# SYSTRAN/faster-whisper

Hardware: AMD Instinct MI355X
Metric: audio-sec/sec (RTF) large-v3 fp16 beam=5 batch=16 (higher is better)
Workload: dtype f16

## Files before the change

### faster_whisper_amd/_lib.py

```python
import ctypes as C
import os

import numpy as np

_HERE = os.path.dirname(os.path.abspath(__file__))
LIB_PATH = os.environ.get("FWAMD_LIB") or os.path.join(_HERE, "libfwamd.so")

FW_OK = 0
FW_EINVAL = -1
FW_ENODEV = -2
FW_ENOMEM = -3
FW_ERUNTIME = -4
FW_ENOSPC = -5

COMPUTE_FLOAT16 = 0
COMPUTE_INT8_FLOAT16 = 1
FW_DT_F32 = 0
FW_DT_F16 = 1
FW_MAX_ALIGN_HEADS = 64


class FwConfig(C.Structure):
    _fields_ = [
        ("n_mels", C.c_int32), ("n_audio_ctx", C.c_int32), ("d_model", C.c_int32), ("n_heads", C.c_int32),
        ("n_enc_layers", C.c_int32), ("n_dec_layers", C.c_int32), ("n_vocab", C.c_int32),
        ("n_text_ctx", C.c_int32), ("is_multilingual", C.c_int32),
        ("tok_eot", C.c_int32), ("tok_sot", C.c_int32), ("tok_lang_begin", C.c_int32), ("n_langs", C.c_int32),
        ("tok_translate", C.c_int32), ("tok_transcribe", C.c_int32), ("tok_sot_lm", C.c_int32),
        ("tok_sot_prev", C.c_int32), ("tok_no_speech", C.c_int32), ("tok_no_timestamps", C.c_int32),
        ("tok_timestamp_begin", C.c_int32),
        ("n_suppress_begin", C.c_int32), ("suppress_begin", C.c_int32 * 8),
        ("n_align_heads", C.c_int32), ("align_heads", C.c_int32 * (2 * FW_MAX_ALIGN_HEADS)),
    ]


class FwWeight(C.Structure):
    _fields_ = [("name", C.c_char_p), ("data", C.c_void_p), ("dtype", C.c_int32), ("ndim", C.c_int32),
                ("dims", C.c_int64 * 4)]


class FwGenOpts(C.Structure):
    _fields_ = [
        ("beam_size", C.c_int32), ("patience", C.c_float), ("num_hypotheses", C.c_int32),
        ("length_penalty", C.c_float), ("repetition_penalty", C.c_float), ("no_repeat_ngram_size", C.c_int32),
        ("max_length", C.c_int32), ("return_scores", C.c_int32), ("return_no_speech_prob", C.c_int32),
        ("max_initial_timestamp_index", C.c_int32), ("suppress_blank", C.c_int32),
        ("suppress_tokens", C.POINTER(C.c_int32)), ("n_suppress_tokens", C.c_int32),
        ("sampling_topk", C.c_int32), ("sampling_temperature", C.c_float), ("seed", C.c_uint64),
        ("min_new_tokens", C.c_int32),
    ]


class FwVadWeights(C.Structure):
    _fields_ = [
        ("stft_basis", C.c_void_p), ("conv_w", C.c_void_p * 4), ("conv_b", C.c_void_p * 4),
        ("lstm_w", C.c_void_p), ("lstm_r", C.c_void_p), ("lstm_b", C.c_void_p), ("dec_w", C.c_void_p),
        ("dec_b", C.c_float),
    ]


SYMBOLS = [
    "fw_last_error", "fw_abi_version", "fw_device_count",
    "fw_model_create", "fw_model_free", "fw_model_info", "fw_model_blob", "fw_model_create_from_blob_dev",
    "fw_model_set_decode_batch", "fw_model_decode_batch", "fw_model_join_decoder", "fw_model_decode_stats",
    "fw_model_set_merge_wait", "fw_model_set_decode_lanes", "fw_model_run_capacity", "fw_dec_big_min_rows", "fw_dec_big_min_rows_of", "fw_test_knob",
    "fw_test_idle_lead_chunks",
    "fw_pack_blob_size", "fw_pack_blob_copy", "fw_pack_blob_free",
    "fw_logmel", "fw_logmel_full",
    "fw_encode", "fw_encode_pcm", "fw_encode_pcm_dev", "fw_tensor_shape", "fw_tensor_to_host",
    "fw_tensor_from_host", "fw_tensor_free",
    "fw_generate", "fw_generate_lp", "fw_detect_language", "fw_align",
    "fw_prof_enable", "fw_prof_reset", "fw_prof_count", "fw_prof_name", "fw_prof_get", "fw_synchronize",
    "fw_dev_alloc", "fw_dev_free", "fw_dev_upload",
    "fw_test_gemm", "fw_test_layernorm", "fw_test_attention", "fw_test_dec_linear", "fw_test_dec_logits", "fw_test_logits_rules",
    "fw_test_dec_self_attn", "fw_test_dec_cross_attn", "fw_test_dec_cross_probs", "fw_test_dec_softmax_pick", "fw_bench_gemm", "fw_bench_dec_linear", "fw_bench_attention",
    "fw_bench_gemm_epi", "fw_bench_dec_linear_epi",
    "fw_test_gemm_ex", "fw_test_cross_kv_frag_index", "fw_test_quant_rows", "fw_test_layernorm_frag",
    "fw_test_dec_beam_update", "fw_test_dec_embed", "fw_test_align_post",
    "fw_test_logits_rules_lp", "fw_test_dec_beam_update_lp",
    "fw_test_logits_rules_smp_tab", "fw_test_graph_captures",
    "fw_vad_create", "fw_vad_forward", "fw_vad_free", "fw_vad_forward_dev", "fw_vad_forward_audio_dev",
    "fw_vad_forward_audio_batch_dev",
    "fw_flac_info", "fw_flac_decode",
    "fw_resample_filter", "fw_resample_dev", "fw_bench_resample",
]

_lib = None


class FwError(RuntimeError):
    pass


def load():
    global _lib
    if _lib is not None:
        return _lib
    if not os.path.exists(LIB_PATH):
        raise FwError(
            f"{LIB_PATH} not found: build it with `python -c 'import __graft_entry__ as g; g.build()'` "
            "(hipcc --offload-arch=gfx950). faster_whisper_amd has no CPU fallback.")
    lib = C.CDLL(LIB_PATH)
    vp, i32, i64, f32p = C.c_void_p, C.c_int32, C.c_int64, C.POINTER(C.c_float)
    i32p, i64p = C.POINTER(C.c_int32), C.POINTER(C.c_int64)
    lib.fw_last_error.restype = C.c_char_p
    lib.fw_abi_version.restype = i32
    lib.fw_device_count.restype = i32
    lib.fw_model_create.argtypes = [C.POINTER(FwConfig), C.POINTER(FwWeight), i32, i32, i32, i32, i32, C.POINTER(vp)]
    lib.fw_model_free.argtypes = [vp]
    lib.fw_model_free.restype = None
    lib.fw_model_info.argtypes = [vp, C.POINTER(FwConfig), i32p, i32p, i32p, i32p]
    lib.fw_model_blob.argtypes = [vp, C.POINTER(vp), i64p]
    lib.fw_model_create_from_blob_dev.argtypes = [C.POINTER(FwConfig), vp, i64, i32, i32, i32, i32, C.POINTER(vp)]
    lib.fw_model_set_decode_batch.argtypes = [vp, i32]
    lib.fw_model_decode_batch.argtypes = [vp]
    lib.fw_model_decode_batch.restype = i32
    lib.fw_model_run_capacity.argtypes = [vp]
    lib.fw_model_run_capacity.restype = i32
    lib.fw_dec_big_min_rows.restype = i32
    if hasattr(lib, "fw_dec_big_min_rows_of"):
        lib.fw_dec_big_min_rows_of.restype = i32
        lib.fw_dec_big_min_rows_of.argtypes = [i32, i32]
    if hasattr(lib, "fw_flac_info"):
        lib.fw_flac_info.argtypes = [vp, i64, i32p, i32p, i32p, i64p]
        lib.fw_flac_decode.argtypes = [vp, i64, vp, i64, i64p, i32p]
    if hasattr(lib, "fw_test_knob"):
        lib.fw_test_knob.argtypes = [i32, i32]
    if hasattr(lib, "fw_test_idle_lead_chunks"):
        lib.fw_test_idle_lead_chunks.argtypes = [i64, i32, i32, i64, i32]
        lib.fw_test_idle_lead_chunks.restype = i64
    lib.fw_model_join_decoder.argtypes = [vp, vp]
    lib.fw_model_set_merge_wait.argtypes = [vp, i32, i32]
    lib.fw_model_set_decode_lanes.argtypes = [vp, i32]
    lib.fw_model_decode_stats.argtypes = [vp, i64p, i64p, i64p, i32p]
    lib.fw_pack_blob_size.argtypes = [C.POINTER(FwConfig), C.POINTER(FwWeight), i32, i32, i64p, C.POINTER(vp)]
    lib.fw_pack_blob_copy.argtypes = [vp, vp, i64]
    lib.fw_pack_blob_free.argtypes = [vp]
    lib.fw_pack_blob_free.restype = None
    lib.fw_logmel.argtypes = [vp, vp, i64p, i32, vp, i32p]
    lib.fw_logmel_full.argtypes = [vp, vp, i64, vp, i64]
    lib.fw_encode.argtypes = [vp, vp, i32, C.POINTER(vp)]
    lib.fw_encode_pcm.argtypes = [vp, vp, i64p, i32, C.POINTER(vp)]
    lib.fw_encode_pcm_dev.argtypes = [vp, vp, i64p, i32, C.POINTER(vp)]
    lib.fw_tensor_shape.argtypes = [vp, i32p, i32p, i32p]
    lib.fw_tensor_to_host.argtypes = [vp, vp, vp]
    lib.fw_tensor_from_host.argtypes = [vp, vp, i32, C.POINTER(vp)]
    lib.fw_tensor_free.argtypes = [vp]
    lib.fw_tensor_free.restype = None
    lib.fw_generate.argtypes = [vp, vp, i32p, i32p, i32, C.POINTER(FwGenOpts), i32p, i32p, f32p, f32p]
    if hasattr(lib, "fw_generate_lp"):
        lib.fw_generate_lp.argtypes = [vp, vp, i32p, i32p, i32, C.POINTER(FwGenOpts), i32p, i32p, f32p, f32p, f32p, f32p]
    lib.fw_detect_language.argtypes = [vp, vp, i32, i32p, f32p]
    lib.fw_align.argtypes = [vp, vp, i32p, i32, i32p, i32p, i32p, i32, i32, i32, i32p, i32p, f32p]
    lib.fw_prof_enable.argtypes = [vp, i32]
    lib.fw_prof_enable.restype = None
    lib.fw_prof_reset.argtypes = [vp]
    lib.fw_prof_reset.restype = None
    lib.fw_prof_count.restype = i32
    lib.fw_prof_name.argtypes = [i32]
    lib.fw_prof_name.restype = C.c_char_p
    lib.fw_prof_get.argtypes = [vp, i32, C.POINTER(C.c_double), i64p, C.POINTER(C.c_double), C.POINTER(C.c_double)]
    lib.fw_synchronize.argtypes = [vp]
    lib.fw_dev_alloc.argtypes = [vp, i64, C.POINTER(vp)]
    lib.fw_dev_free.argtypes = [vp, vp]
    lib.fw_dev_upload.argtypes = [vp, vp, vp, i64]
    lib.fw_test_gemm.argtypes = [vp, vp, vp, vp, vp, i32, i32, i32, i32, i32, vp]
    lib.fw_test_dec_linear.argtypes = [vp, vp, vp, vp, vp, vp, vp, i32, i32, i32, i32, i32, vp, vp]
    lib.fw_test_dec_logits.argtypes = [vp, vp, i32, vp]
    lib.fw_test_logits_rules.argtypes = [vp, vp, i32, vp, i32, vp, C.POINTER(FwGenOpts), i32, vp, vp]
    if hasattr(lib, "fw_test_dec_self_attn"):
        lib.fw_test_dec_self_attn.argtypes = [vp, vp, vp, vp, vp, i32, i32, i32, i32, i32, i32, i32, i32, i32, i32, i32, vp]
        lib.fw_test_dec_cross_attn.argtypes = [vp, vp, vp, vp, i32, i32, i32, i32, i32, i32, vp, vp, i32, C.c_float, vp]
        lib.fw_test_dec_cross_probs.argtypes = [vp, vp, vp, i32, i32, i32, vp, i32, i32, i32, i32, vp]
        lib.fw_test_dec_softmax_pick.argtypes = [vp, vp, i32, i32, i32, vp, i32, vp]
    lib.fw_bench_attention.argtypes = [vp, i32, i32, i32, i32, i32, f32p]
    lib.fw_bench_gemm.argtypes = [vp, i32, i32, i32, i32, i32, i32, i32, i32, f32p]
    lib.fw_bench_dec_linear.argtypes = [vp, i32, i32, i32, i32, i32, i32, f32p]
    if hasattr(lib, "fw_bench_gemm_epi"):
        lib.fw_bench_gemm_epi.argtypes = [vp, i32, i32, i32, i32, i32, i32, i32, i32, i32, i32, i32, f32p]
        lib.fw_bench_dec_linear_epi.argtypes = [vp, i32, i32, i32, i32, i32, i32, i32, i32, i32, f32p]
    lib.fw_test_layernorm.argtypes = [vp, vp, vp, vp, i32, i32, vp]
    lib.fw_test_attention.argtypes = [vp, vp, vp, vp, i32, i32, i32, vp]
    if hasattr(lib, "fw_test_gemm_ex"):
        lib.fw_test_gemm_ex.argtypes = [vp, vp, i64, i64, i64, vp, vp, vp, i64, i64, i64, vp, i64, i64, i64, i64, i64,
                                        i32, i32, i32, i32, i32, i32, i32, i32, i32, vp, vp]
        lib.fw_test_cross_kv_frag_index.argtypes = [i32, i32, i32, vp]
        lib.fw_test_quant_rows.argtypes = [vp, vp, i32, i32, i64, vp, vp, i32, vp, vp]
        lib.fw_test_layernorm_frag.argtypes = [vp, vp, vp, vp, i32, i32, i32, vp]
    if hasattr(lib, "fw_test_dec_beam_update"):
        f32 = C.c_float
        lib.fw_test_dec_beam_update.argtypes = [vp, i32, i32, i32, i32, i32, i32, i32, i32, f32, i32, vp, vp, vp, vp, vp,
                                                i32, f32, vp, vp, vp, vp, vp, vp, vp, vp, vp, vp, vp]
        lib.fw_test_dec_embed.argtypes = [vp, vp, i32, vp, i32, vp, i32, i32, i32, i32, i32, i32, f32, vp, vp]
        lib.fw_test_align_post.argtypes = [vp, vp, i32, i32, i32, i32, vp, vp, i32, vp]
    if hasattr(lib, "fw_test_dec_beam_update_lp"):
        f32 = C.c_float
        lib.fw_test_logits_rules_lp.argtypes = [vp, vp, i32, vp, i32, vp, C.POINTER(FwGenOpts), i32, vp, vp, vp]
        lib.fw_test_dec_beam_update_lp.argtypes = [vp, i32, i32, i32, i32, i32, i32, i32, i32, f32, i32, vp, vp, vp, vp, vp,
                                                   vp, vp, i32, f32, vp, vp, vp, vp, vp, vp, vp, vp, vp, vp, vp, vp, vp]
    if hasattr(lib, "fw_test_graph_captures"):
        lib.fw_test_logits_rules_smp_tab.argtypes = [vp, vp, i32, vp, i32, vp, C.POINTER(FwGenOpts), i32, vp, vp, vp, vp, vp, vp]
        lib.fw_test_graph_captures.argtypes = [vp, i64p]
    lib.fw_vad_create.argtypes = [C.POINTER(FwVadWeights), C.POINTER(vp)]
    lib.fw_vad_forward.argtypes = [vp, vp, i64, i32, vp, vp, vp]
    lib.fw_vad_free.argtypes = [vp]
    lib.fw_vad_forward_dev.argtypes = [vp, i32, vp, i64, vp, vp, vp]
    if hasattr(lib, "fw_vad_forward_audio_dev"):
        lib.fw_vad_forward_audio_dev.argtypes = [vp, i32, vp, i64, vp, vp, vp]
    if hasattr(lib, "fw_vad_forward_audio_batch_dev"):
        lib.fw_vad_forward_audio_batch_dev.argtypes = [vp, i32, vp, vp, i32, vp, vp, vp]
    lib.fw_vad_free.restype = None
    if hasattr(lib, "fw_resample_dev"):
        f64 = C.c_double
        lib.fw_resample_filter.argtypes = [i32, i32, i32, f64, vp, i64p, i32p, i32p]
        lib.fw_resample_dev.argtypes = [i32, vp, i64, i32, i32, i32, f64, i32, vp, i64]
        lib.fw_bench_resample.argtypes = [i32, vp, i64, i32, i32, i32, f64, i32, i32, f32p]
    _lib = lib
    return lib


def check(rc: int):
    if rc == FW_OK:
        return
    msg = load().fw_last_error().decode("utf-8", "replace")
    if rc in (FW_EINVAL, FW_ENOSPC):
        raise ValueError(msg)
    raise RuntimeError(f"libfwamd error {rc}: {msg}")


def ptr(a: np.ndarray):
    return a.ctypes.data_as(C.c_void_p)


def as_i32p(a: np.ndarray):
    return a.ctypes.data_as(C.POINTER(C.c_int32))


def as_i64p(a: np.ndarray):
    return a.ctypes.data_as(C.POINTER(C.c_int64))


def as_f32p(a: np.ndarray):
    return a.ctypes.data_as(C.POINTER(C.c_float))
```

### faster_whisper_amd/csrc/engine.h

```cpp
#pragma once
#include <hip/hip_runtime.h>
#include <math.h>
#include <stdint.h>
#include <string.h>
#include <algorithm>
#include <atomic>
#include <chrono>
#include <condition_variable>
#include <deque>
#include <map>
#include <memory>
#include <mutex>
#include <string>
#include <vector>

#include "../../include/fwamd.h"
#include "common.h"

namespace fw {

void set_error(const char* fmt, ...);
#define FW_HIP(call)                                                                   \
  do {                                                                                 \
    hipError_t e_ = (call);                                                            \
    if (e_ != hipSuccess) {                                                            \
      fw::set_error("%s failed: %s (%s:%d)", #call, hipGetErrorString(e_), __FILE__, __LINE__); \
      return FW_ENODEV;                                                                \
    }                                                                                  \
  } while (0)
#define FW_CHECK_ARG(cond, ...)        \
  do {                                 \
    if (!(cond)) {                     \
      fw::set_error(__VA_ARGS__);      \
      return FW_EINVAL;                \
    }                                  \
  } while (0)

inline uint16_t f32_to_f16_bits(float f) {
  half_t h = (half_t)f;
  uint16_t u;
  memcpy(&u, &h, 2);
  return u;
}
inline float f16_bits_to_f32(uint16_t u) {
  half_t h;
  memcpy(&h, &u, 2);
  return (float)h;
}

template <typename At>
inline float quant_row_i8(const float* row, int K, int8_t* q, At&& at) {
  float amax = 0.f;
  for (int k = 0; k < K; ++k) amax = std::max(amax, fabsf(row[k]));
  const float sc = amax > 0.f ? 127.0f / amax : 0.f;
  for (int k = 0; k < K; ++k) q[at(k)] = (int8_t)lrintf(row[k] * sc);
  return amax > 0.f ? amax / 127.0f : 1.0f;
}

#define FW_BLOB_MAGIC "FWAMDBL1"
struct BlobHeader {
  char magic[8];
  int32_t version;
  int32_t n_tensors;
  int64_t total_bytes;
  int32_t compute_type;
  int32_t reserved;
  fw_config cfg;
};
struct BlobEntry {
  char name[64];
  int32_t dtype;
  int32_t ndim;
  int64_t dims[4];
  int64_t offset;
  int64_t nbytes;
};

struct DevTensor {
  void* ptr = nullptr;
  int dtype = 1;
  int ndim = 0;
  int64_t dims[4] = {0, 0, 0, 0};
};

struct LinearW {
  const half_t* w = nullptr;
  const half_t* b = nullptr;
  const int8_t* wq = nullptr;
  const float* wscale = nullptr;
  const float* s1 = nullptr;
  const float* cf = nullptr;
  int N = 0, K = 0;
};
struct LNW { const half_t* g = nullptr; const half_t* b = nullptr; };

struct EncLayerW { LNW ln1, ln2; LinearW qk, v, out, ffn1, ffn2; };
struct DecLayerW { LNW ln1, ln2, ln3; LinearW qkv, out, cq, ck, cv, cout, ffn1, ffn2; LinearW qkv_p, cq_p, ffn1_p; };

enum ProfFamily {
  PF_LOGMEL = 0, PF_ENC_GEMM, PF_ENC_ATTN, PF_ENC_LN, PF_CROSS_KV_GEMM,
  PF_DEC_GEMM_QKV, PF_DEC_GEMM_DXD, PF_DEC_GEMM_FFN1, PF_DEC_GEMM_FFN2,
  PF_DEC_SELF_ATTN, PF_DEC_CROSS_ATTN, PF_DEC_LOGITS, PF_DEC_SAMPLE, PF_DEC_MISC, PF_COUNT
};

struct ProfAcc {
  double ms = 0; int64_t launches = 0; double flops = 0; double bytes = 0;
};

struct Prof {
  std::mutex mu;
  bool on = false;
  ProfAcc acc[PF_COUNT];
  struct PendingEv { hipEvent_t a, b; int fam; };
  std::vector<PendingEv> pending;
  std::vector<hipEvent_t> ev_pool;
  ~Prof();
};

struct Model;
struct Tensor {
  Model* owner = nullptr;
  half_t* data = nullptr;
  int B = 0, T = 0, D = 0;
  uint64_t id = 0;
};

struct GenWorkspace;
struct GenRequest;
struct CrossPool;

constexpr int kMaxDecodeLanes = 4;
struct DecodeLane {
  GenWorkspace* gen = nullptr;
  hipStream_t stream = nullptr;
  hipStream_t spare = nullptr;
  std::mutex mu;
  Prof prof;
  bool busy = false;
  ~DecodeLane();
};

struct DecodeGroup {
  std::mutex mu;
  std::condition_variable cv;
  std::deque<GenRequest*> queue;
  bool gathering = false;
  bool resizing = false;
  int active_runs = 0;
  std::atomic<int> lanes_enabled{kMaxDecodeLanes};
  std::atomic<int> encoding{0};
  std::chrono::steady_clock::time_point last_arrival{};
  std::mutex enc_mu;
  std::atomic<int> enc_pass_us{0};
  std::atomic<int> merge_wait_ms{-1};
  std::atomic<int> merge_fill_pct{90};
  std::atomic<int64_t> n_runs{0}, n_requests{0}, n_chunks{0};
  std::atomic<int> max_run_chunks{0};
  std::atomic<int64_t> graph_captures{0};
};

struct Model {
  fw_config cfg{};
  int compute_type = 0;
  int device = 0;
  int max_batch = 0, max_beam = 0;
  hipStream_t stream = nullptr;
  std::mutex mu;

  void* blob = nullptr;
  bool blob_owned = true;
  int64_t blob_bytes = 0;
  std::map<std::string, DevTensor> tensors;
  int c_pad = 0;
  LinearW conv1, conv2;
  const half_t* enc_pos = nullptr;
  std::vector<EncLayerW> enc;
  LNW enc_ln_post;
  const half_t* tok_emb = nullptr;
  const half_t* dec_pos = nullptr;
  std::vector<DecLayerW> dec;
  LinearW logits;
  LinearW logits_p;
  LNW dec_ln;
  int ln_unfold = 0;
  bool has_plain = false;

  float* lm_consts = nullptr;
  float* lm_filtT = nullptr;
  int lm_mel_pad = 0;

  float* ws_pcm = nullptr; int64_t ws_pcm_cap = 0;
  int64_t* ws_offsets = nullptr;
  float* ws_raw = nullptr; int64_t ws_raw_cap = 0;
  int* ws_chunk_max = nullptr;
  int* ws_nframes = nullptr;
  float* ws_feat32 = nullptr;
  half_t* ws_mel_cl = nullptr;
  half_t* ws_conv1 = nullptr;
  half_t *ws_x = nullptr, *ws_x2 = nullptr, *ws_xn = nullptr;
  half_t* ws_qk = nullptr;
  half_t* ws_vt = nullptr;
  half_t* ws_att = nullptr;
  half_t* ws_ffn = nullptr;
  int8_t* ws_xq = nullptr;
  float* ws_xs = nullptr;
  int t_pad = 0;

  std::vector<std::unique_ptr<DecodeLane>> lanes;
  Model* decoder = nullptr;
  CrossPool* xpool = nullptr;
  int decode_batch = 0;
  int lane_batch = 0;
  int decode_self_ctx = 0;
  int dependents = 0;
  bool free_deferred = false;
  void* self = nullptr;
  Model* blob_owner = nullptr;
  DecodeGroup grp;

  std::mutex pool_mu;
  std::vector<half_t*> enc_pool;

  Prof prof;
};

struct ProfScope {
  Prof* p; int fam; hipStream_t st; hipEvent_t a = nullptr, b = nullptr;
  ProfScope(Prof& p_, int fam_, double flops, double bytes, hipStream_t st_);
  ProfScope(Model* m, int fam_, double flops, double bytes) : ProfScope(m->prof, fam_, flops, bytes, m->stream) {}
  ~ProfScope();
};
void prof_collect(Prof& p);

int dev_alloc(void** p, size_t bytes);
hipError_t create_stream(hipStream_t* st, const char* role);
int64_t idle_lead_chunks(int64_t queued, int n_queued, int encoding, int64_t want, int max_batch, int lanes = 2);
template <typename T>
inline int dev_alloc_t(T** p, size_t n) { return dev_alloc(reinterpret_cast<void**>(p), n * sizeof(T)); }

int run_linear(Model* m, const LinearW& L, const half_t* A, int64_t lda, int64_t a_bs, half_t* C, int64_t ldc,
               int64_t c_bs, const half_t* res, int64_t ldr, int64_t r_bs, int M, int batch, int act, bool trans,
               int head_rows = 0, hipStream_t st = nullptr);

int run_linear_i8(Model* m, const LinearW& L, const half_t* A, const LNW* ln, half_t* C, int64_t ldc, int64_t c_bs,
                  const half_t* res, int64_t ldr, int64_t r_bs, int M, int batch, int act, bool trans, int head_rows,
                  hipStream_t st = nullptr, int8_t* xq = nullptr, float* xs = nullptr);

int run_linear_layers(Model* m, const LinearW& L0, int n_layers, int64_t w_lstride, int64_t b_lstride, const half_t* A,
                      int64_t lda, int64_t a_bs, half_t* C, int64_t ldc, int64_t c_bs, int64_t c_lstride, int M, int batch,
                      bool trans, int head_rows, hipStream_t st);
void set_cross_kv_layered(int on);
int run_encoder(Model* m, int B, half_t* out);

void set_pos_blocks(int on);
uint64_t next_tensor_id();
int gen_workspace_ensure(Model* dm, DecodeLane* lane);
int cross_pool_ensure(Model* dm, int pool_chunks);
int gen_workspace_build(const Model* dm, DecodeLane* lane, int lane_chunks, int self_ctx);
void gen_workspace_free(DecodeLane* lane);
int64_t gen_workspace_bytes(const Model* m, int lane_chunks, int self_ctx);
int64_t cross_pool_bytes(const Model* m, int pool_chunks);
void cross_pool_free(Model* m);
void launch_align_post(hipStream_t st, const float* probs, float* stats, int n_sel, int n_tok_cap, int T, int B,
                       const int* n_tok, const int* nfr, int width, float* mat);
inline Model* decoder_of(Model* m) { return m->decoder ? m->decoder : m; }
inline int lane_chunks_of(const Model* m) {
  const int b = m->lane_batch > 0 ? m->lane_batch : m->decode_batch;
  return b > m->max_batch ? b : m->max_batch;
}

}

struct fw_model { fw::Model impl; };
struct fw_tensor { fw::Tensor impl; };
```

### faster_whisper_amd/csrc/engine.hip

```cpp
#include "engine.h"

#include <math.h>
#include <stdarg.h>
#include <stdio.h>
#include <stdlib.h>
#include <string.h>

#include <algorithm>

#include "dec_kernels.h"
#include "kernels.h"

namespace fw {

static thread_local char g_err[1024] = "";
void set_error(const char* fmt, ...) {
  va_list ap;
  va_start(ap, fmt);
  vsnprintf(g_err, sizeof(g_err), fmt, ap);
  va_end(ap);
}

int dev_alloc(void** p, size_t bytes) {
  if (bytes == 0) bytes = 256;
  hipError_t e = hipMalloc(p, bytes);
  if (e != hipSuccess) {
    set_error("hipMalloc(%zu bytes) failed: %s", bytes, hipGetErrorString(e));
    *p = nullptr;
    return FW_ENOMEM;
  }
  return FW_OK;
}

static const char* kProfNames[PF_COUNT] = {
    "logmel", "enc_gemm", "enc_attn", "enc_layernorm", "cross_kv_gemm", "dec_gemm_qkv", "dec_gemm_dxd",
    "dec_gemm_ffn1", "dec_gemm_ffn2", "dec_self_attn", "dec_cross_attn", "dec_logits", "dec_sample", "dec_misc"};

static hipEvent_t ev_get(Prof& p) {
  if (!p.ev_pool.empty()) {
    hipEvent_t e = p.ev_pool.back();
    p.ev_pool.pop_back();
    return e;
  }
  hipEvent_t e;
  (void)hipEventCreate(&e);
  return e;
}
ProfScope::ProfScope(Prof& p_, int fam_, double flops, double bytes, hipStream_t st_) : p(&p_), fam(fam_), st(st_) {
  if (!p->on) return;
  {
    std::lock_guard<std::mutex> lk(p->mu);
    a = ev_get(*p);
    b = ev_get(*p);
    p->acc[fam].flops += flops;
    p->acc[fam].bytes += bytes;
    p->acc[fam].launches += 1;
  }
  (void)hipEventRecord(a, st);
}
ProfScope::~ProfScope() {
  if (!a) return;
  (void)hipEventRecord(b, st);
  std::lock_guard<std::mutex> lk(p->mu);
  p->pending.push_back({a, b, fam});
}
void prof_collect(Prof& p) {
  std::vector<Prof::PendingEv> todo;
  {
    std::lock_guard<std::mutex> lk(p.mu);
    todo.swap(p.pending);
  }
  std::vector<std::pair<int, float>> got;
  for (auto& e : todo) {
    (void)hipEventSynchronize(e.b);
    float ms = 0.f;
    (void)hipEventElapsedTime(&ms, e.a, e.b);
    got.push_back({e.fam, ms});
  }
  std::lock_guard<std::mutex> lk(p.mu);
  for (auto& g : got) p.acc[g.first].ms += g.second;
  for (auto& e : todo) {
    p.ev_pool.push_back(e.a);
    p.ev_pool.push_back(e.b);
  }
}
Prof::~Prof() {
  for (auto& e : pending) { (void)hipEventDestroy(e.a); (void)hipEventDestroy(e.b); }
  for (auto e : ev_pool) (void)hipEventDestroy(e);
}
template <typename F>
static void for_each_prof(Model* m, F&& f) {
  f(m->prof);
  for (auto& l : m->lanes) f(l->prof);
}

struct PackItem {
  std::string name;
  int ndim;
  int64_t dims[4];
  std::vector<uint16_t> data;
  std::vector<float> fdata;
  std::vector<int8_t> qdata;
  int dtype = 1;
  const void* bytes() const {
    return dtype == 1 ? (const void*)data.data() : dtype == 2 ? (const void*)qdata.data() : (const void*)fdata.data();
  }
  int64_t nbytes() const {
    return dtype == 1 ? (int64_t)data.size() * 2 : dtype == 2 ? (int64_t)qdata.size() : (int64_t)fdata.size() * 4;
  }
};

static const fw_weight* find_w(const fw_weight* w, int n, const std::string& name) {
  for (int i = 0; i < n; ++i)
    if (name == w[i].name) return &w[i];
  return nullptr;
}
static int64_t numel(const fw_weight* w) {
  int64_t n = 1;
  for (int i = 0; i < w->ndim; ++i) n *= w->dims[i];
  return n;
}
static float w_at(const fw_weight* w, int64_t i) {
  if (w->dtype == FW_DT_F32) return reinterpret_cast<const float*>(w->data)[i];
  half_t h;
  memcpy(&h, reinterpret_cast<const uint16_t*>(w->data) + i, 2);
  return (float)h;
}
static void to_f16(const fw_weight* w, std::vector<uint16_t>& out) {
  const int64_t n = numel(w);
  out.resize(n);
  if (w->dtype == FW_DT_F16) {
    memcpy(out.data(), w->data, n * 2);
  } else {
    const float* s = reinterpret_cast<const float*>(w->data);
    for (int64_t i = 0; i < n; ++i) out[i] = f32_to_f16_bits(s[i]);
  }
}

static int expect_shape(const fw_weight* w, const std::string& name, std::initializer_list<int64_t> dims) {
  if (!w) {
    set_error("missing weight '%s'", name.c_str());
    return FW_EINVAL;
  }
  if ((size_t)w->ndim != dims.size()) {
    set_error("weight '%s': expected %zu dims, got %d", name.c_str(), dims.size(), w->ndim);
    return FW_EINVAL;
  }
  int i = 0;
  for (int64_t d : dims) {
    if (w->dims[i] != d) {
      set_error("weight '%s': dim %d is %lld, expected %lld", name.c_str(), i, (long long)w->dims[i], (long long)d);
      return FW_EINVAL;
    }
    ++i;
  }
  return FW_OK;
}

static int check_config(const fw_config* c) {
  FW_CHECK_ARG(c->n_mels > 0 && c->n_mels <= 128, "n_mels must be in (0,128], got %d", c->n_mels);
  FW_CHECK_ARG(c->d_model % 128 == 0 && c->d_model >= 128 && c->d_model <= 1280,
               "d_model must be a multiple of 128 in [128,1280], got %d", c->d_model);
  FW_CHECK_ARG(c->n_heads * 64 == c->d_model, "head dim must be 64 (n_heads=%d, d_model=%d)", c->n_heads, c->d_model);
  FW_CHECK_ARG(c->n_audio_ctx == 1500, "n_audio_ctx must be 1500, got %d", c->n_audio_ctx);
  FW_CHECK_ARG(c->n_text_ctx > 0 && c->n_text_ctx <= 448, "n_text_ctx must be in (0,448]");
  FW_CHECK_ARG(c->n_enc_layers > 0 && c->n_dec_layers > 0, "layer counts must be positive");
  FW_CHECK_ARG(c->n_vocab > c->tok_timestamp_begin && c->tok_timestamp_begin > 0, "bad vocabulary layout");
  FW_CHECK_ARG(c->n_align_heads >= 0 && c->n_align_heads <= FW_MAX_ALIGN_HEADS, "too many alignment heads");
  FW_CHECK_ARG(c->n_suppress_begin >= 0 && c->n_suppress_begin <= 8, "n_suppress_begin out of range");
  FW_CHECK_ARG(c->n_vocab <= 57344, "n_vocab %d exceeds the 57344 ids the logits kernel holds per row", c->n_vocab);
  const int toks[] = {c->tok_eot, c->tok_sot, c->tok_translate, c->tok_transcribe, c->tok_sot_lm, c->tok_sot_prev,
                      c->tok_no_speech, c->tok_no_timestamps, c->tok_timestamp_begin};
  for (int t : toks) FW_CHECK_ARG(t >= 0 && t < c->n_vocab, "special token id %d outside the vocabulary of %d", t, c->n_vocab);
  FW_CHECK_ARG(c->n_langs >= 0 && c->tok_lang_begin >= 0 && c->tok_lang_begin + c->n_langs <= c->n_vocab,
               "language ids [%d, %d) outside the vocabulary of %d", c->tok_lang_begin, c->tok_lang_begin + c->n_langs,
               c->n_vocab);
  for (int i = 0; i < c->n_suppress_begin; ++i)
    FW_CHECK_ARG(c->suppress_begin[i] >= 0 && c->suppress_begin[i] < c->n_vocab, "suppress_begin id out of range");
  return FW_OK;
}

static int pack_blob(const fw_config* cfg, const fw_weight* w, int nw, int compute_type,
                     std::vector<uint8_t>& blob) {
  const int d = cfg->d_model, nm = cfg->n_mels;
  const int c_pad = ((nm + 63) / 64) * 64;
  std::vector<PackItem> items;
  auto add_plain = [&](const std::string& name, std::initializer_list<int64_t> dims) -> int {
    const fw_weight* t = find_w(w, nw, name);
    int rc = expect_shape(t, name, dims);
    if (rc) return rc;
    PackItem it;
    it.name = name;
    it.ndim = (int)dims.size();
    int i = 0;
    for (int64_t x : dims) it.dims[i++] = x;
    for (; i < 4; ++i) it.dims[i] = 1;
    to_f16(t, it.data);
    items.push_back(std::move(it));
    return FW_OK;
  };
  auto add_conv = [&](const std::string& name, int cout, int cin, int cin_pad) -> int {
    const fw_weight* t = find_w(w, nw, name + ".w");
    int rc = expect_shape(t, name + ".w", {cout, cin, 3});
    if (rc) return rc;
    PackItem it;
    it.name = name + ".wg";
    it.ndim = 2;
    it.dims[0] = cout; it.dims[1] = 3 * cin_pad; it.dims[2] = it.dims[3] = 1;
    it.data.assign((size_t)cout * 3 * cin_pad, 0);
    for (int o = 0; o < cout; ++o)
      for (int c = 0; c < cin; ++c)
        for (int k = 0; k < 3; ++k)
          it.data[(size_t)o * 3 * cin_pad + (size_t)k * cin_pad + c] =
              f32_to_f16_bits(w_at(t, ((int64_t)o * cin + c) * 3 + k));
    items.push_back(std::move(it));
    return add_plain(name + ".b", {cout});
  };
  auto add_folded = [&](const std::string& out, const std::string& wname, const std::string& bname,
                        const std::string& gname, const std::string& lbname, int N, int K) -> int {
    const fw_weight* W = find_w(w, nw, wname);
    const fw_weight* G = find_w(w, nw, gname);
    const fw_weight* LB = find_w(w, nw, lbname);
    const fw_weight* Bi = bname.empty() ? nullptr : find_w(w, nw, bname);
    int rc = expect_shape(W, wname, {N, K});
    if (rc) return rc;
    if ((rc = expect_shape(G, gname, {K}))) return rc;
    if ((rc = expect_shape(LB, lbname, {K}))) return rc;
    if (!bname.empty() && (rc = expect_shape(Bi, bname, {N}))) return rc;
    std::vector<float> g(K), lb(K);
    for (int k = 0; k < K; ++k) {
      g[k] = f16_bits_to_f32(f32_to_f16_bits(w_at(G, k)));
      lb[k] = f16_bits_to_f32(f32_to_f16_bits(w_at(LB, k)));
    }
    PackItem wf, s1, cf;
    wf.name = out + ".wf"; wf.ndim = 2; wf.dims[0] = N; wf.dims[1] = K; wf.dims[2] = wf.dims[3] = 1;
    wf.data.resize((size_t)N * K);
    s1.name = out + ".s1"; s1.ndim = 1; s1.dims[0] = N; s1.dims[1] = s1.dims[2] = s1.dims[3] = 1; s1.dtype = 0;
    cf.name = out + ".cf"; cf.ndim = 1; cf.dims[0] = N; cf.dims[1] = cf.dims[2] = cf.dims[3] = 1; cf.dtype = 0;
    s1.fdata.resize(N); cf.fdata.resize(N);
    for (int n = 0; n < N; ++n) {
      double a1 = 0.0, ac = 0.0;
      for (int k = 0; k < K; ++k) {
        const float wv = f16_bits_to_f32(f32_to_f16_bits(w_at(W, (int64_t)n * K + k)));
        const uint16_t wg = f32_to_f16_bits(wv * g[k]);
        wf.data[(size_t)n * K + k] = wg;
        a1 += (double)f16_bits_to_f32(wg);
        ac += (double)wv * (double)lb[k];
      }
      if (Bi) ac += (double)f16_bits_to_f32(f32_to_f16_bits(w_at(Bi, n)));
      s1.fdata[n] = (float)a1;
      cf.fdata[n] = (float)ac;
    }
    items.push_back(std::move(wf)); items.push_back(std::move(s1)); items.push_back(std::move(cf));
    return FW_OK;
  };
  auto add_quant = [&](const std::string& out, const std::string& wname, int N, int K) -> int {
    const fw_weight* W = find_w(w, nw, wname);
    int rc = expect_shape(W, wname, {N, K});
    if (rc) return rc;
    PackItem wq, ws;
    wq.name = out + ".wq"; wq.ndim = 2; wq.dims[0] = N; wq.dims[1] = K; wq.dims[2] = wq.dims[3] = 1; wq.dtype = 2;
    ws.name = out + ".ws"; ws.ndim = 1; ws.dims[0] = N; ws.dims[1] = ws.dims[2] = ws.dims[3] = 1; ws.dtype = 0;
    wq.qdata.resize((size_t)N * K);
    ws.fdata.resize(N);
    std::vector<float> row(K);
    for (int n = 0; n < N; ++n) {
      for (int k = 0; k < K; ++k) row[k] = f16_bits_to_f32(f32_to_f16_bits(w_at(W, (int64_t)n * K + k)));
      ws.fdata[n] = quant_row_i8(row.data(), K, wq.qdata.data(), [&](int k) { return (size_t)n * K + k; });
    }
    items.push_back(std::move(wq)); items.push_back(std::move(ws));
    return FW_OK;
  };
  const bool i8 = compute_type == FW_COMPUTE_INT8_FLOAT16;
  auto add_linear = [&](const std::string& base, int N, int K) -> int {
    int rc = i8 ? add_quant(base, base + ".w", N, K) : add_plain(base + ".w", {N, K});
    if (rc) return rc;
    return add_plain(base + ".b", {N});
  };
  const char* lu_env = getenv("FWAMD_LN_UNFOLD");
  const char* pp_env = getenv("FWAMD_PACK_PLAIN");
  const bool with_plain = (lu_env && (lu_env[0] == '1' || lu_env[0] == '2') && !lu_env[1]) || (pp_env && pp_env[0] == '1');
  auto add_ln_linear = [&](const std::string& base, const std::string& ln, int N, int K) -> int {
    if (!i8) {
      int rc = add_folded(base, base + ".w", base + ".b", ln + ".g", ln + ".b", N, K);
      if (rc || !with_plain) return rc;
    }
    int rc = add_linear(base, N, K);
    if (rc) return rc;
    if ((rc = add_plain(ln + ".g", {K}))) return rc;
    return add_plain(ln + ".b", {K});
  };
  int rc;
#define TRY(x) do { rc = (x); if (rc) return rc; } while (0)
  TRY(add_conv("enc.conv1", d, nm, c_pad));
  TRY(add_conv("enc.conv2", d, d, d));
  TRY(add_plain("enc.pos", {cfg->n_audio_ctx, d}));
  char nb[96];
  for (int i = 0; i < cfg->n_enc_layers; ++i) {
    auto nmf = [&](const char* s) { snprintf(nb, sizeof(nb), "enc.%d.%s", i, s); return std::string(nb); };
    TRY(add_plain(nmf("ln1.g"), {d})); TRY(add_plain(nmf("ln1.b"), {d}));
    TRY(add_linear(nmf("attn.qkv"), 3 * d, d));
    TRY(add_linear(nmf("attn.out"), d, d));
    TRY(add_plain(nmf("ln2.g"), {d})); TRY(add_plain(nmf("ln2.b"), {d}));
    TRY(add_linear(nmf("ffn1"), 4 * d, d));
    TRY(add_linear(nmf("ffn2"), d, 4 * d));
  }
  TRY(add_plain("enc.ln_post.g", {d})); TRY(add_plain("enc.ln_post.b", {d}));
  TRY(add_plain("dec.tok_emb", {cfg->n_vocab, d}));
  if (i8) {
    PackItem& te = items.back();
    const int64_t K = d;
    for (int64_t n = 0; n < cfg->n_vocab; ++n) {
      float amax = 0.f;
      for (int64_t k = 0; k < K; ++k) amax = std::max(amax, fabsf(f16_bits_to_f32(te.data[n * K + k])));
      const float sc = amax > 0.f ? 127.0f / amax : 0.f, ds = amax > 0.f ? amax / 127.0f : 1.0f;
      for (int64_t k = 0; k < K; ++k)
        te.data[n * K + k] = f32_to_f16_bits((float)lrintf(f16_bits_to_f32(te.data[n * K + k]) * sc) * ds);
    }
  }
  TRY(add_plain("dec.pos", {cfg->n_text_ctx, d}));
  for (int i = 0; i < cfg->n_dec_layers; ++i) {
    auto nmf = [&](const char* s) { snprintf(nb, sizeof(nb), "dec.%d.%s", i, s); return std::string(nb); };
    TRY(add_ln_linear(nmf("self.qkv"), nmf("ln1"), 3 * d, d));
    TRY(add_linear(nmf("self.out"), d, d));
    TRY(add_ln_linear(nmf("cross.q"), nmf("ln2"), d, d));
    TRY(add_linear(nmf("cross.kv"), 2 * d, d));
    TRY(add_linear(nmf("cross.out"), d, d));
    TRY(add_ln_linear(nmf("ffn1"), nmf("ln3"), 4 * d, d));
    TRY(add_linear(nmf("ffn2"), d, 4 * d));
  }
  if (i8) {
    TRY(add_quant("dec.logits", "dec.tok_emb", cfg->n_vocab, d));
    TRY(add_plain("dec.ln.g", {d})); TRY(add_plain("dec.ln.b", {d}));
  } else {
    TRY(add_folded("dec.logits", "dec.tok_emb", "", "dec.ln.g", "dec.ln.b", cfg->n_vocab, d));
    if (with_plain) {
      TRY(add_plain("dec.tok_emb", {cfg->n_vocab, d}));
      items.back().name = "dec.logits.wp";
      TRY(add_plain("dec.ln.g", {d})); TRY(add_plain("dec.ln.b", {d}));
    }
  }
#undef TRY

  for (PackItem& it : items) {
    const std::string& nm = it.name;
    if (nm.compare(0, 4, "dec.") != 0 || it.ndim != 2 || it.dtype != (i8 ? 2 : 1)) continue;
    auto ends = [&](const char* suf) {
      const size_t n = strlen(suf);
      return nm.size() >= n && nm.compare(nm.size() - n, n, suf) == 0;
    };
    const bool hit = i8 ? (ends("self.qkv.wq") || ends("self.out.wq") || ends("cross.q.wq") || ends("cross.out.wq") ||
                           ends("ffn1.wq") || ends("ffn2.wq") || nm == "dec.logits.wq")
                        : (ends("self.qkv.wf") || ends("self.out.w") || ends("cross.q.wf") || ends("cross.out.w") ||
                           ends("ffn1.wf") || ends("ffn2.w") || nm == "dec.logits.wf" || ends("self.qkv.w") ||
                           ends("cross.q.w") || ends("ffn1.w") || nm == "dec.logits.wp");
    if (!hit) continue;
    const int64_t N = it.dims[0], K = it.dims[1], KE = i8 ? 64 : 32, OCT = KE / 4;
    const bool logits = nm.compare(0, 10, "dec.logits") == 0;
    if ((!logits && N % 32) || K % KE) {
      set_error("fragment-major packing needs N %% 32 == 0 and K %% %lld == 0 (%s is %lld x %lld)", (long long)KE,
                nm.c_str(), (long long)N, (long long)K);
      return FW_EINVAL;
    }
    const int64_t NP = (N + 15) / 16 * 16, KS = K / KE;
    it.dims[0] = NP;
    auto at = [&](int64_t n, int64_t k) {
      return (((n >> 4) * KS + k / KE) * 64 + ((k / OCT) & 3) * 16 + (n & 15)) * OCT + (k % OCT);
    };
    if (i8) {
      std::vector<int8_t> src;
      src.swap(it.qdata);
      it.qdata.assign((size_t)NP * K, 0);
      for (int64_t n = 0; n < N; ++n)
        for (int64_t k = 0; k < K; ++k) it.qdata[at(n, k)] = src[n * K + k];
    } else {
      std::vector<uint16_t> src;
      src.swap(it.data);
      it.data.assign((size_t)NP * K, 0);
      for (int64_t n = 0; n < N; ++n)
        for (int64_t k = 0; k < K; ++k) it.data[at(n, k)] = src[n * K + k];
    }
  }

  const int64_t hdr = (int64_t)sizeof(BlobHeader) + (int64_t)items.size() * sizeof(BlobEntry);
  int64_t off = (hdr + 255) / 256 * 256;
  std::vector<BlobEntry> entries(items.size());
  for (size_t i = 0; i < items.size(); ++i) {
    BlobEntry& e = entries[i];
    memset(&e, 0, sizeof(e));
    snprintf(e.name, sizeof(e.name), "%s", items[i].name.c_str());
    e.dtype = items[i].dtype;
    e.ndim = items[i].ndim;
    for (int k = 0; k < 4; ++k) e.dims[k] = items[i].dims[k];
    e.offset = off;
    e.nbytes = items[i].nbytes();
    off = (off + e.nbytes + 255) / 256 * 256;
  }
  blob.assign((size_t)off, 0);
  BlobHeader h;
  memset(&h, 0, sizeof(h));
  memcpy(h.magic, FW_BLOB_MAGIC, 8);
  h.version = 1;
  h.n_tensors = (int32_t)items.size();
  h.total_bytes = off;
  h.compute_type = compute_type;
  h.reserved = 6;
  h.cfg = *cfg;
  memcpy(blob.data(), &h, sizeof(h));
  memcpy(blob.data() + sizeof(h), entries.data(), entries.size() * sizeof(BlobEntry));
  for (size_t i = 0; i < items.size(); ++i)
    memcpy(blob.data() + entries[i].offset, items[i].bytes(), (size_t)entries[i].nbytes);
  return FW_OK;
}

static void compute_mel_filters(int n_mels, std::vector<float>& filt ) {
  const int n_fft = 400, nb = 201;
  const double sr = 16000.0;
  std::vector<double> fftfreqs(nb);
  const double val = 1.0 / (n_fft * (1.0 / sr));
  for (int k = 0; k < nb; ++k) fftfreqs[k] = k * val;
  const double max_mel = 45.245640471924965;
  const int n = n_mels + 2;
  std::vector<double> mels(n), freqs(n);
  const double step = (max_mel - 0.0) / (n - 1);
  for (int i = 0; i < n; ++i) mels[i] = i * step + 0.0;
  mels[n - 1] = max_mel;
  const double f_sp = 200.0 / 3;
  const double min_log_hz = 1000.0, min_log_mel = (min_log_hz - 0.0) / f_sp;
  const double logstep = log(6.4) / 27.0;
  for (int i = 0; i < n; ++i) {
    freqs[i] = 0.0 + f_sp * mels[i];
    if (mels[i] >= min_log_mel) freqs[i] = min_log_hz * exp(logstep * (mels[i] - min_log_mel));
  }
  filt.assign((size_t)n_mels * nb, 0.f);
  for (int i = 0; i < n_mels; ++i) {
    const double fd0 = freqs[i + 1] - freqs[i], fd1 = freqs[i + 2] - freqs[i + 1];
    const double enorm = 2.0 / (freqs[i + 2] - freqs[i]);
    for (int k = 0; k < nb; ++k) {
      const double lower = -(freqs[i] - fftfreqs[k]) / fd0;
      const double upper = (freqs[i + 2] - fftfreqs[k]) / fd1;
      double wv = std::max(0.0, std::min(lower, upper));
      wv *= enorm;
      filt[(size_t)i * nb + k] = (float)wv;
    }
  }
}

static int setup_logmel_consts(Model* m) {
  std::vector<float> consts(800);
  for (int j = 0; j < 400; ++j) consts[j] = (float)cos(2.0 * M_PI * (double)j / 400.0);
  for (int n = 0; n < 400; ++n) consts[400 + n] = (float)(0.5 - 0.5 * cos(2.0 * M_PI * (double)n / 400.0));
  std::vector<float> filt;
  compute_mel_filters(m->cfg.n_mels, filt);
  m->lm_mel_pad = ((m->cfg.n_mels + 31) / 32) * 32;
  std::vector<float> filtT((size_t)224 * m->lm_mel_pad, 0.f);
  for (int i = 0; i < m->cfg.n_mels; ++i)
    for (int k = 0; k < 201; ++k) filtT[(size_t)k * m->lm_mel_pad + i] = filt[(size_t)i * 201 + k];
  int rc;
  if ((rc = dev_alloc_t(&m->lm_consts, 800))) return rc;
  if ((rc = dev_alloc_t(&m->lm_filtT, filtT.size()))) return rc;
  FW_HIP(hipMemcpy(m->lm_consts, consts.data(), 800 * sizeof(float), hipMemcpyHostToDevice));
  FW_HIP(hipMemcpy(m->lm_filtT, filtT.data(), filtT.size() * sizeof(float), hipMemcpyHostToDevice));
  return FW_OK;
}

std::mutex& g_models_mu_ref();
std::vector<Model*>& g_live_models_ref();
static const half_t* tptr(Model* m, const std::string& name) {
  auto it = m->tensors.find(name);
  return it == m->tensors.end() ? nullptr : reinterpret_cast<const half_t*>(it->second.ptr);
}

static int bind_weights(Model* m) {
  const fw_config& c = m->cfg;
  const int d = c.d_model;
  const bool i8 = m->compute_type == FW_COMPUTE_INT8_FLOAT16;
  m->c_pad = ((c.n_mels + 63) / 64) * 64;
  auto need = [&](const std::string& n, const half_t** out) -> int {
    *out = tptr(m, n);
    if (!*out) {
      set_error("weight blob lacks tensor '%s'", n.c_str());
      return FW_EINVAL;
    }
    return FW_OK;
  };
  auto need_f = [&](const std::string& n, const float** out) -> int {
    const half_t* p = nullptr;
    int r = need(n, &p);
    *out = reinterpret_cast<const float*>(p);
    return r;
  };
  auto linear = [&](const std::string& base, LinearW* L, int N, int K, int r0) -> int {
    int r;
    *L = LinearW();
    L->N = N; L->K = K;
    if (i8) {
      const half_t* q = nullptr;
      if ((r = need(base + ".wq", &q))) return r;
      L->wq = reinterpret_cast<const int8_t*>(q) + (size_t)r0 * K;
      if ((r = need_f(base + ".ws", &L->wscale))) return r;
      L->wscale += r0;
    } else {
      if ((r = need(base + ".w", &L->w))) return r;
      L->w += (size_t)r0 * K;
    }
    if ((r = need(base + ".b", &L->b))) return r;
    L->b += r0;
    return FW_OK;
  };
  auto folded = [&](const std::string& base, LinearW* L, int N, int K) -> int {
    int r;
    *L = LinearW();
    if ((r = need(base + ".wf", &L->w))) return r;
    if ((r = need_f(base + ".s1", &L->s1))) return r;
    if ((r = need_f(base + ".cf", &L->cf))) return r;
    L->N = N; L->K = K;
    return FW_OK;
  };
  auto ln = [&](const std::string& base, LNW* L) -> int {
    int r;
    if ((r = need(base + ".g", &L->g))) return r;
    return need(base + ".b", &L->b);
  };
  int rc;
#define TRY(x) do { if ((rc = (x))) return rc; } while (0)
  TRY(need("enc.conv1.wg", &m->conv1.w)); TRY(need("enc.conv1.b", &m->conv1.b));
  m->conv1.N = d; m->conv1.K = 3 * m->c_pad;
  TRY(need("enc.conv2.wg", &m->conv2.w)); TRY(need("enc.conv2.b", &m->conv2.b));
  m->conv2.N = d; m->conv2.K = 3 * d;
  TRY(need("enc.pos", &m->enc_pos));
  m->enc.resize(c.n_enc_layers);
  char nb[96];
  for (int i = 0; i < c.n_enc_layers; ++i) {
    EncLayerW& L = m->enc[i];
    auto nm = [&](const char* s) { snprintf(nb, sizeof(nb), "enc.%d.%s", i, s); return std::string(nb); };
    TRY(ln(nm("ln1"), &L.ln1));
    TRY(linear(nm("attn.qkv"), &L.qk, 2 * d, d, 0));
    TRY(linear(nm("attn.qkv"), &L.v, d, d, 2 * d));
    TRY(linear(nm("attn.out"), &L.out, d, d, 0));
    TRY(ln(nm("ln2"), &L.ln2));
    TRY(linear(nm("ffn1"), &L.ffn1, 4 * d, d, 0));
    TRY(linear(nm("ffn2"), &L.ffn2, d, 4 * d, 0));
  }
  TRY(ln("enc.ln_post", &m->enc_ln_post));
  TRY(need("dec.tok_emb", &m->tok_emb)); TRY(need("dec.pos", &m->dec_pos));
  m->dec.resize(c.n_dec_layers);
  m->has_plain = !i8 && tptr(m, "dec.logits.wp") != nullptr;
  for (int i = 0; i < c.n_dec_layers; ++i) {
    DecLayerW& L = m->dec[i];
    auto nm = [&](const char* s) { snprintf(nb, sizeof(nb), "dec.%d.%s", i, s); return std::string(nb); };
    if (i8) {
      TRY(ln(nm("ln1"), &L.ln1)); TRY(ln(nm("ln2"), &L.ln2)); TRY(ln(nm("ln3"), &L.ln3));
      TRY(linear(nm("self.qkv"), &L.qkv, 3 * d, d, 0));
      TRY(linear(nm("cross.q"), &L.cq, d, d, 0));
      TRY(linear(nm("ffn1"), &L.ffn1, 4 * d, d, 0));
    } else {
      TRY(folded(nm("self.qkv"), &L.qkv, 3 * d, d));
      TRY(folded(nm("cross.q"), &L.cq, d, d));
      TRY(folded(nm("ffn1"), &L.ffn1, 4 * d, d));
      if (m->has_plain) {
        TRY(ln(nm("ln1"), &L.ln1)); TRY(ln(nm("ln2"), &L.ln2)); TRY(ln(nm("ln3"), &L.ln3));
        TRY(linear(nm("self.qkv"), &L.qkv_p, 3 * d, d, 0));
        TRY(linear(nm("cross.q"), &L.cq_p, d, d, 0));
        TRY(linear(nm("ffn1"), &L.ffn1_p, 4 * d, d, 0));
      }
    }
    TRY(linear(nm("self.out"), &L.out, d, d, 0));
    TRY(linear(nm("cross.kv"), &L.ck, d, d, 0));
    TRY(linear(nm("cross.kv"), &L.cv, d, d, d));
    TRY(linear(nm("cross.out"), &L.cout, d, d, 0));
    TRY(linear(nm("ffn2"), &L.ffn2, d, 4 * d, 0));
  }
  if (i8) {
    const half_t* q = nullptr;
    m->logits = LinearW();
    TRY(need("dec.logits.wq", &q));
    m->logits.wq = reinterpret_cast<const int8_t*>(q);
    TRY(need_f("dec.logits.ws", &m->logits.wscale));
    m->logits.N = c.n_vocab; m->logits.K = d;
    TRY(ln("dec.ln", &m->dec_ln));
  } else {
    TRY(folded("dec.logits", &m->logits, c.n_vocab, d));
    m->logits_p = LinearW();
    if (m->has_plain) {
      TRY(need("dec.logits.wp", &m->logits_p.w));
      m->logits_p.N = c.n_vocab; m->logits_p.K = d;
      TRY(ln("dec.ln", &m->dec_ln));
    }
  }
#undef TRY
  return FW_OK;
}

static int alloc_workspaces(Model* m) {
  const fw_config& c = m->cfg;
  const size_t B = m->max_batch, d = c.d_model, T = c.n_audio_ctx;
  m->t_pad = ((c.n_audio_ctx + 63) / 64) * 64;
  int rc;
#define A(p, n) do { if ((rc = dev_alloc_t(&(p), (n)))) return rc; } while (0)
  A(m->ws_offsets, B + 1);
  A(m->ws_chunk_max, B);
  A(m->ws_nframes, B);
  m->ws_raw_cap = (int64_t)B * c.n_mels * 3008;
  A(m->ws_raw, (size_t)m->ws_raw_cap);
  A(m->ws_feat32, B * c.n_mels * 3000);
  A(m->ws_mel_cl, B * 3002 * m->c_pad);
  A(m->ws_conv1, B * 3002 * d);
  A(m->ws_x, B * T * d);
  A(m->ws_x2, B * T * d);
  A(m->ws_xn, B * T * d);
  A(m->ws_qk, B * T * 2 * d);
  A(m->ws_vt, B * d * m->t_pad);
  A(m->ws_att, B * T * d);
  A(m->ws_ffn, B * T * 4 * d);
  if (m->compute_type == FW_COMPUTE_INT8_FLOAT16) {
    A(m->ws_xq, B * T * 4 * d);
    A(m->ws_xs, B * T);
  }
#undef A
  FW_HIP(hipMemset(m->ws_conv1, 0, B * 3002 * d * sizeof(half_t)));
  FW_HIP(hipMemset(m->ws_vt, 0, B * d * m->t_pad * sizeof(half_t)));
  FW_HIP(hipMemset(m->ws_mel_cl, 0, B * 3002 * m->c_pad * sizeof(half_t)));
  return FW_OK;
}

static int model_from_blob(const void* blob_dev, int64_t blob_bytes, bool owned, int device, int max_batch,
                           int max_beam, fw_model** out) {
  FW_CHECK_ARG(max_batch >= 1 && max_batch <= 256, "max_batch must be in [1,256], got %d", max_batch);
  FW_CHECK_ARG(max_beam >= 1 && max_beam <= 16, "max_beam must be in [1,16], got %d", max_beam);
  FW_CHECK_ARG(max_batch * max_beam <= 2048, "max_batch * max_beam must be <= 2048 decoder rows, got %d", max_batch * max_beam);
  FW_CHECK_ARG(blob_bytes >= (int64_t)sizeof(BlobHeader), "weight blob too small");
  BlobHeader h;
  FW_HIP(hipMemcpy(&h, blob_dev, sizeof(h), hipMemcpyDeviceToHost));
  FW_CHECK_ARG(memcmp(h.magic, FW_BLOB_MAGIC, 8) == 0 && h.version == 1, "bad weight blob magic/version");
  FW_CHECK_ARG(h.total_bytes <= blob_bytes, "weight blob truncated (%lld > %lld)", (long long)h.total_bytes,
               (long long)blob_bytes);
  int rc = check_config(&h.cfg);
  if (rc) return rc;
  FW_CHECK_ARG(h.compute_type == FW_COMPUTE_FLOAT16 || h.compute_type == FW_COMPUTE_INT8_FLOAT16,
               "unsupported compute type %d", h.compute_type);
  std::vector<BlobEntry> entries(h.n_tensors);
  FW_HIP(hipMemcpy(entries.data(), reinterpret_cast<const char*>(blob_dev) + sizeof(h),
                   entries.size() * sizeof(BlobEntry), hipMemcpyDeviceToHost));
  fw_model* fm = new fw_model();
  Model* m = &fm->impl;
  m->lanes.reserve(kMaxDecodeLanes);
  m->lanes.emplace_back(new DecodeLane());
  m->cfg = h.cfg;
  m->compute_type = h.compute_type;
  if (h.reserved != 6) {
    delete fm;
    set_error("weight blob was packed by an older libfwamd (layout generation %d, expected 6): repack it", h.reserved);
    return FW_EINVAL;
  }
  m->device = device;
  m->max_batch = max_batch;
  m->max_beam = max_beam;
  m->blob = const_cast<void*>(blob_dev);
  m->blob_owned = owned;
  m->blob_bytes = blob_bytes;
  for (auto& e : entries) {
    DevTensor t;
    t.ptr = reinterpret_cast<char*>(m->blob) + e.offset;
    t.dtype = e.dtype;
    t.ndim = e.ndim;
    for (int k = 0; k < 4; ++k) t.dims[k] = e.dims[k];
    m->tensors[e.name] = t;
  }
  auto fail = [&](int code) { fw_model_free(fm); return code; };
  hipError_t he = create_stream(&m->stream, "ENC");
  if (he != hipSuccess) {
    set_error("hipStreamCreate failed: %s", hipGetErrorString(he));
    return fail(FW_ENODEV);
  }
  if ((rc = bind_weights(m))) return fail(rc);
  {
    const char* lu = getenv("FWAMD_LN_UNFOLD");
    if (lu && lu[0] >= '0' && lu[0] <= '2' && !lu[1]) m->ln_unfold = lu[0] - '0';
    if (m->ln_unfold && m->compute_type != FW_COMPUTE_INT8_FLOAT16 && !m->has_plain) {
      set_error("FWAMD_LN_UNFOLD=%d needs a weight blob packed with FWAMD_LN_UNFOLD set (this one carries the folded forms only)",
                m->ln_unfold);
      return fail(FW_EINVAL);
    }
  }
  if ((rc = setup_logmel_consts(m))) return fail(rc);
  if ((rc = alloc_workspaces(m))) return fail(rc);
  m->decode_batch = max_batch;
  he = hipDeviceSynchronize();
  if (he != hipSuccess) {
    set_error("device sync after model setup failed: %s", hipGetErrorString(he));
    return fail(FW_ENODEV);
  }
  {
    std::lock_guard<std::mutex> lk(g_models_mu_ref());
    if (!owned)
      for (Model* o : g_live_models_ref())
        if (o->blob == m->blob && o->blob_owned) { m->blob_owner = o; o->dependents += 1; break; }
    g_live_models_ref().push_back(m);
  }
  m->self = fm;
  *out = fm;
  return FW_OK;
}

static void balanced_cu_mask(int n_cus, bool invert, uint32_t mask[8]) {
  const int k = n_cus / 32;
  for (int w = 0; w < 8; ++w) mask[w] = 0;
  for (int i = 0; i < 256; ++i) {
    const bool in = ((i % 8) + (i / 8)) % 8 < k;
    if (in != invert) mask[i >> 5] |= 1u << (i & 31);
  }
}

hipError_t create_stream(hipStream_t* st, const char* role) {
  char name[64];
  snprintf(name, sizeof(name), "FWAMD_%s_CUS", role);
  if (const char* c = getenv(name)) {
    const int v = atoi(c), n = v < 0 ? -v : v;
    if (n >= 32 && n <= 224 && n % 32 == 0) {
      uint32_t mask[8];
      balanced_cu_mask(n, v < 0, mask);
      return hipExtStreamCreateWithCUMask(st, 8, mask);
    }
  }
  snprintf(name, sizeof(name), "FWAMD_%s_STREAM_PRIO", role);
  const char* e = getenv(name);
  if (e && (!strcmp(e, "high") || !strcmp(e, "low"))) {
    int least = 0, greatest = 0;
    if (hipDeviceGetStreamPriorityRange(&least, &greatest) == hipSuccess && least != greatest)
      return hipStreamCreateWithPriority(st, hipStreamNonBlocking, e[0] == 'h' ? greatest : least);
  }
  return hipStreamCreateWithFlags(st, hipStreamNonBlocking);
}

int run_linear(Model* m, const LinearW& L, const half_t* A, int64_t lda, int64_t a_bs, half_t* C, int64_t ldc,
               int64_t c_bs, const half_t* res, int64_t ldr, int64_t r_bs, int M, int batch, int act, bool trans,
               int head_rows, hipStream_t st) {
  fwk::GemmParams p;
  memset(&p, 0, sizeof(p));
  p.A = A; p.lda = lda; p.a_bstride = a_bs;
  p.W = L.w; p.ldw = L.K;
  p.bias = L.b;
  p.res = res; p.ldr = ldr; p.r_bstride = r_bs;
  p.C = C; p.ldc = ldc; p.c_bstride = c_bs;
  p.M = M; p.N = L.N; p.K = L.K;
  p.act = act;
  p.head_rows = head_rows;
  if (fwk::launch_gemm(st ? st : m->stream, p, batch, trans) != 0) {
    set_error("gemm: unsupported shape M=%d N=%d K=%d lda=%lld", M, L.N, L.K, (long long)lda);
    return FW_ERUNTIME;
  }
  return FW_OK;
}

int run_linear_layers(Model* m, const LinearW& L0, int n_layers, int64_t w_lstride, int64_t b_lstride, const half_t* A,
                      int64_t lda, int64_t a_bs, half_t* C, int64_t ldc, int64_t c_bs, int64_t c_lstride, int M, int batch,
                      bool trans, int head_rows, hipStream_t st) {
  fwk::GemmParams p;
  memset(&p, 0, sizeof(p));
  p.A = A; p.lda = lda; p.a_bstride = a_bs;
  p.W = L0.w; p.ldw = L0.K;
  p.bias = L0.b;
  p.C = C; p.ldc = ldc; p.c_bstride = c_bs;
  p.M = M; p.N = L0.N; p.K = L0.K;
  p.head_rows = head_rows;
  p.n_layers = n_layers; p.w_lstride = w_lstride; p.bias_lstride = b_lstride; p.c_lstride = c_lstride;
  if (fwk::launch_gemm(st ? st : m->stream, p, batch, trans) != 0) {
    set_error("layered gemm: unsupported shape M=%d N=%d K=%d layers=%d", M, L0.N, L0.K, n_layers);
    return FW_ERUNTIME;
  }
  return FW_OK;
}

int run_linear_i8(Model* m, const LinearW& L, const half_t* A, const LNW* ln, half_t* C, int64_t ldc, int64_t c_bs,
                  const half_t* res, int64_t ldr, int64_t r_bs, int M, int batch, int act, bool trans,
                  int head_rows, hipStream_t st, int8_t* xq, float* xs) {
  if (!st) st = m->stream;
  if (!xq) { xq = m->ws_xq; xs = m->ws_xs; }
  if (A) fwk::launch_quant_rows(st, A, L.K, ln ? ln->g : nullptr, ln ? ln->b : nullptr, xq, xs, batch * M, L.K);
  fwk::GemmParams p;
  memset(&p, 0, sizeof(p));
  p.A = reinterpret_cast<const half_t*>(xq); p.lda = L.K; p.a_bstride = (int64_t)M * L.K;
  p.W = reinterpret_cast<const half_t*>(L.wq); p.ldw = L.K;
  p.bias = L.b;
  p.res = res; p.ldr = ldr; p.r_bstride = r_bs;
  p.C = C; p.ldc = ldc; p.c_bstride = c_bs;
  p.M = M; p.N = L.N; p.K = L.K;
  p.act = act;
  p.head_rows = head_rows;
  p.a_scale = xs; p.as_bstride = M; p.w_scale = L.wscale;
  if (fwk::launch_gemm(st, p, batch, trans) != 0) {
    set_error("int8 gemm: unsupported shape M=%d N=%d K=%d", M, L.N, L.K);
    return FW_ERUNTIME;
  }
  return FW_OK;
}

int run_encoder(Model* m, int B, half_t* out) {
  const fw_config& c = m->cfg;
  const int d = c.d_model, T = c.n_audio_ctx, H = c.n_heads;
  const int64_t xs = (int64_t)T * d;
  int rc;
  {
    ProfScope ps(m, PF_ENC_GEMM, 2.0 * B * 3000.0 * d * (3.0 * c.n_mels), 0);
    if ((rc = run_linear(m, m->conv1, m->ws_mel_cl, m->c_pad, (int64_t)3002 * m->c_pad, m->ws_conv1 + d, d,
                         (int64_t)3002 * d, nullptr, 0, 0, 3000, B, 1, false)))
      return rc;
  }
  {
    ProfScope ps(m, PF_ENC_GEMM, 2.0 * B * (double)T * d * (3.0 * d), 0);
    if ((rc = run_linear(m, m->conv2, m->ws_conv1, 2 * d, (int64_t)3002 * d, m->ws_x, d, xs, m->enc_pos, d, 0, T, B,
                         1, false)))
      return rc;
  }
  half_t* x = m->ws_x;
  half_t* x2 = m->ws_x2;
  const bool i8 = m->compute_type == FW_COMPUTE_INT8_FLOAT16;
  for (int l = 0; l < c.n_enc_layers; ++l) {
    const EncLayerW& L = m->enc[l];
    if (i8) {
      {
        ProfScope ps(m, PF_ENC_GEMM, 2.0 * B * (double)T * d * (3.0 * d), 0);
        if ((rc = run_linear_i8(m, L.qk, x, &L.ln1, m->ws_qk, 2 * d, (int64_t)T * 2 * d, nullptr, 0, 0, T, B, 0, false,
                                0)))
          return rc;
        if ((rc = run_linear_i8(m, L.v, nullptr, nullptr, m->ws_vt, m->t_pad, (int64_t)d * m->t_pad, nullptr, 0, 0, T,
                                B, 0, true, 0)))
          return rc;
      }
      {
        ProfScope ps(m, PF_ENC_ATTN, 4.0 * B * (double)T * T * d, 0);
        fwk::launch_attn_enc(m->stream, m->ws_qk, m->ws_qk + d, 2 * d, (int64_t)T * 2 * d, m->ws_vt, m->t_pad,
                             (int64_t)d * m->t_pad, m->ws_att, d, xs, B, H, T);
      }
      {
        ProfScope ps(m, PF_ENC_GEMM, 2.0 * B * (double)T * d * (9.0 * d), 0);
        if ((rc = run_linear_i8(m, L.out, m->ws_att, nullptr, x2, d, xs, x, d, xs, T, B, 0, false, 0))) return rc;
        if ((rc = run_linear_i8(m, L.ffn1, x2, &L.ln2, m->ws_ffn, 4 * d, (int64_t)T * 4 * d, nullptr, 0, 0, T, B, 1,
                                false, 0)))
          return rc;
        if ((rc = run_linear_i8(m, L.ffn2, m->ws_ffn, nullptr, x, d, xs, x2, d, xs, T, B, 0, false, 0))) return rc;
      }
      continue;
    }
    {
      ProfScope ps(m, PF_ENC_LN, 0, 4.0 * B * T * d);
      fwk::launch_layernorm(m->stream, x, L.ln1.g, L.ln1.b, m->ws_xn, B * T, d);
    }
    {
      ProfScope ps(m, PF_ENC_GEMM, 2.0 * B * (double)T * d * (3.0 * d), 0);
      if ((rc = run_linear(m, L.qk, m->ws_xn, d, xs, m->ws_qk, 2 * d, (int64_t)T * 2 * d, nullptr, 0, 0, T, B, 0,
                           false)))
        return rc;
      if ((rc = run_linear(m, L.v, m->ws_xn, d, xs, m->ws_vt, m->t_pad, (int64_t)d * m->t_pad, nullptr, 0, 0, T, B, 0,
                           true)))
        return rc;
    }
    {
      ProfScope ps(m, PF_ENC_ATTN, 4.0 * B * (double)T * T * d, 0);
      fwk::launch_attn_enc(m->stream, m->ws_qk, m->ws_qk + d, 2 * d, (int64_t)T * 2 * d, m->ws_vt, m->t_pad,
                           (int64_t)d * m->t_pad, m->ws_att, d, xs, B, H, T);
    }
    {
      ProfScope ps(m, PF_ENC_GEMM, 2.0 * B * (double)T * d * d, 0);
      if ((rc = run_linear(m, L.out, m->ws_att, d, xs, x2, d, xs, x, d, xs, T, B, 0, false))) return rc;
    }
    {
      ProfScope ps(m, PF_ENC_LN, 0, 4.0 * B * T * d);
      fwk::launch_layernorm(m->stream, x2, L.ln2.g, L.ln2.b, m->ws_xn, B * T, d);
    }
    {
      ProfScope ps(m, PF_ENC_GEMM, 2.0 * B * (double)T * d * (8.0 * d), 0);
      if ((rc = run_linear(m, L.ffn1, m->ws_xn, d, xs, m->ws_ffn, 4 * d, (int64_t)T * 4 * d, nullptr, 0, 0, T, B, 1,
                           false)))
        return rc;
      if ((rc = run_linear(m, L.ffn2, m->ws_ffn, 4 * d, (int64_t)T * 4 * d, x, d, xs, x2, d, xs, T, B, 0, false)))
        return rc;
    }
  }
  {
    ProfScope ps(m, PF_ENC_LN, 0, 4.0 * B * T * d);
    fwk::launch_layernorm(m->stream, x, m->enc_ln_post.g, m->enc_ln_post.b, out, B * T, d);
  }
  hipError_t he = hipGetLastError();
  if (he != hipSuccess) {
    set_error("encoder launch failed: %s", hipGetErrorString(he));
    return FW_ERUNTIME;
  }
  return FW_OK;
}

static int new_tensor(Model* m, int B, fw_tensor** out) {
  fw_tensor* t = new fw_tensor();
  t->impl.owner = m;
  t->impl.B = B;
  t->impl.T = m->cfg.n_audio_ctx;
  t->impl.D = m->cfg.d_model;
  t->impl.id = next_tensor_id();
  {
    std::lock_guard<std::mutex> lk(m->pool_mu);
    if (!m->enc_pool.empty()) {
      t->impl.data = m->enc_pool.back();
      m->enc_pool.pop_back();
    }
  }
  if (!t->impl.data) {
    int rc = dev_alloc_t(&t->impl.data, (size_t)m->max_batch * t->impl.T * t->impl.D);
    if (rc) {
      delete t;
      return rc;
    }
  }
  *out = t;
  return FW_OK;
}

static std::mutex g_models_mu;
static std::vector<Model*> g_live_models;
std::mutex& g_models_mu_ref() { return g_models_mu; }
std::vector<Model*>& g_live_models_ref() { return g_live_models; }

static int ensure_pcm(Model* m, int64_t n) {
  if (n <= m->ws_pcm_cap) return FW_OK;
  if (m->ws_pcm) (void)hipFree(m->ws_pcm);
  m->ws_pcm = nullptr;
  m->ws_pcm_cap = 0;
  int rc = dev_alloc_t(&m->ws_pcm, (size_t)n);
  if (rc) return rc;
  m->ws_pcm_cap = n;
  return FW_OK;
}

static int check_offsets(const int64_t* offsets, int B, int64_t* total, int* max_frames) {
  FW_CHECK_ARG(offsets && offsets[0] == 0, "offsets[0] must be 0");
  int mf = 0;
  for (int b = 0; b < B; ++b) {
    const int64_t n = offsets[b + 1] - offsets[b];
    FW_CHECK_ARG(n >= 0 && n < (int64_t)1 << 30, "chunk %d has invalid length %lld", b, (long long)n);
    mf = std::max(mf, (int)((n + 160) / 160));
  }
  *total = offsets[B];
  *max_frames = mf;
  return FW_OK;
}

static int ensure_raw(Model* m, int B, int stride) {
  const int64_t need = (int64_t)B * m->cfg.n_mels * stride;
  if (need <= m->ws_raw_cap) return FW_OK;
  (void)hipFree(m->ws_raw);
  m->ws_raw = nullptr;
  m->ws_raw_cap = 0;
  int rc = dev_alloc_t(&m->ws_raw, (size_t)need);
  if (rc) return rc;
  m->ws_raw_cap = need;
  return FW_OK;
}

static int logmel_batch(Model* m, const float* pcm_dev, const int64_t* offsets_host, int B, bool want_f32,
                        bool want_cl) {
  int64_t total;
  int max_frames;
  int rc = check_offsets(offsets_host, B, &total, &max_frames);
  if (rc) return rc;
  const int stride = std::max(3008, (max_frames + 7) / 8 * 8);
  if ((rc = ensure_raw(m, B, stride))) return rc;
  FW_HIP(hipMemcpyAsync(m->ws_offsets, offsets_host, (B + 1) * sizeof(int64_t), hipMemcpyHostToDevice, m->stream));
  {
    ProfScope ps(m, PF_LOGMEL, 0, (double)total * 4 + (double)B * m->cfg.n_mels * 3000 * (want_f32 ? 4 : 2));
    fwk::launch_logmel(m->stream, pcm_dev, m->ws_offsets, B, max_frames, m->lm_consts, m->lm_filtT, m->lm_mel_pad,
                       m->cfg.n_mels, m->ws_raw, (int64_t)m->cfg.n_mels * stride, stride, m->ws_chunk_max, 1, 3000,
                       want_f32 ? m->ws_feat32 : nullptr, want_cl ? m->ws_mel_cl : nullptr, m->c_pad, m->ws_nframes);
  }
  hipError_t he = hipGetLastError();
  if (he != hipSuccess) {
    set_error("logmel launch failed: %s", hipGetErrorString(he));
    return FW_ERUNTIME;
  }
  return FW_OK;
}

}

using namespace fw;

extern "C" {

const char* fw_last_error(void) { return g_err; }
int32_t fw_abi_version(void) { return FW_ABI_VERSION; }

int32_t fw_device_count(void) {
  int n = 0;
  if (hipGetDeviceCount(&n) != hipSuccess) return 0;
  return n;
}

int32_t fw_model_create(const fw_config* cfg, const fw_weight* weights, int32_t n_weights, int32_t compute_type,
                        int32_t device_index, int32_t max_batch, int32_t max_beam, fw_model** out) {
  FW_CHECK_ARG(cfg && weights && out, "null argument");
  FW_CHECK_ARG(compute_type == FW_COMPUTE_FLOAT16 || compute_type == FW_COMPUTE_INT8_FLOAT16,
               "unsupported compute_type %d", compute_type);
  int rc = check_config(cfg);
  if (rc) return rc;
  const int ndev = fw_device_count();
  if (ndev <= 0) {
    set_error("no HIP device visible: libfwamd has no CPU fallback");
    return FW_ENODEV;
  }
  FW_CHECK_ARG(device_index >= 0 && device_index < ndev, "device_index %d out of range (%d devices)", device_index,
               ndev);
  FW_HIP(hipSetDevice(device_index));
  std::vector<uint8_t> blob;
  if ((rc = pack_blob(cfg, weights, n_weights, compute_type, blob))) return rc;
  void* dblob = nullptr;
  if ((rc = dev_alloc(&dblob, blob.size()))) return rc;
  hipError_t he = hipMemcpy(dblob, blob.data(), blob.size(), hipMemcpyHostToDevice);
  if (he != hipSuccess) {
    (void)hipFree(dblob);
    set_error("weight upload failed: %s", hipGetErrorString(he));
    return FW_ENODEV;
  }
  rc = model_from_blob(dblob, (int64_t)blob.size(), true, device_index, max_batch, max_beam, out);
  return rc;
}

int32_t fw_pack_blob_size(const fw_config* cfg, const fw_weight* weights, int32_t n_weights, int32_t compute_type,
                          int64_t* size_out, void** handle_out) {
  FW_CHECK_ARG(cfg && weights && size_out && handle_out, "null argument");
  int rc = check_config(cfg);
  if (rc) return rc;
  auto* blob = new std::vector<uint8_t>();
  if ((rc = pack_blob(cfg, weights, n_weights, compute_type, *blob))) {
    delete blob;
    return rc;
  }
  *size_out = (int64_t)blob->size();
  *handle_out = blob;
  return FW_OK;
}
int32_t fw_pack_blob_copy(void* handle, void* dst, int64_t dst_bytes) {
  auto* blob = reinterpret_cast<std::vector<uint8_t>*>(handle);
  FW_CHECK_ARG(blob && dst && dst_bytes >= (int64_t)blob->size(), "bad blob copy arguments");
  memcpy(dst, blob->data(), blob->size());
  return FW_OK;
}
void fw_pack_blob_free(void* handle) { delete reinterpret_cast<std::vector<uint8_t>*>(handle); }

int32_t fw_model_create_from_blob_dev(const fw_config* cfg, const void* blob_dev, int64_t blob_bytes,
                                      int32_t compute_type, int32_t device_index, int32_t max_batch,
                                      int32_t max_beam, fw_model** out) {
  (void)cfg;
  (void)compute_type;
  FW_CHECK_ARG(blob_dev && out, "null argument");
  const int ndev = fw_device_count();
  if (ndev <= 0) {
    set_error("no HIP device visible: libfwamd has no CPU fallback");
    return FW_ENODEV;
  }
  FW_CHECK_ARG(device_index >= 0 && device_index < ndev, "device_index %d out of range", device_index);
  FW_HIP(hipSetDevice(device_index));
  return model_from_blob(blob_dev, blob_bytes, false, device_index, max_batch, max_beam, out);
}

void fw_model_free(fw_model* fm) {
  if (!fm) return;
  Model* m = &fm->impl;
  Model* release[2] = {nullptr, nullptr};
  {
    std::lock_guard<std::mutex> lk(g_models_mu);
    if (m->dependents > 0) {
      m->free_deferred = true;
      return;
    }
    g_live_models.erase(std::remove(g_live_models.begin(), g_live_models.end(), m), g_live_models.end());
    release[0] = m->blob_owner;
    release[1] = m->decoder;
  }
  (void)hipSetDevice(m->device);
  if (m->stream) (void)hipStreamSynchronize(m->stream);
  m->lanes.clear();
  cross_pool_free(m);
  for (half_t* p : m->enc_pool) (void)hipFree(p);
  m->enc_pool.clear();
  void* ptrs[] = {m->lm_consts, m->lm_filtT, m->ws_pcm, m->ws_offsets, m->ws_raw, m->ws_chunk_max, m->ws_nframes,
                  m->ws_feat32, m->ws_mel_cl, m->ws_conv1, m->ws_x, m->ws_x2, m->ws_xn, m->ws_qk, m->ws_vt,
                  m->ws_att, m->ws_ffn, m->ws_xq, m->ws_xs};
  for (void* p : ptrs)
    if (p) (void)hipFree(p);
  if (m->blob && m->blob_owned) (void)hipFree(m->blob);
  if (m->stream) (void)hipStreamDestroy(m->stream);
  delete fm;
  for (Model* t : release) {
    if (!t) continue;
    bool free_now = false;
    {
      std::lock_guard<std::mutex> lk(g_models_mu);
      t->dependents -= 1;
      free_now = t->free_deferred && t->dependents == 0;
    }
    if (free_now) fw_model_free(static_cast<fw_model*>(t->self));
  }
}

int32_t fw_model_blob(const fw_model* fm, void** blob_dev, int64_t* blob_bytes) {
  FW_CHECK_ARG(fm && blob_dev && blob_bytes, "null argument");
  *blob_dev = fm->impl.blob;
  *blob_bytes = fm->impl.blob_bytes;
  return FW_OK;
}

int32_t fw_model_info(const fw_model* fm, fw_config* cfg_out, int32_t* compute_type, int32_t* device_index,
                      int32_t* max_batch, int32_t* max_beam) {
  FW_CHECK_ARG(fm, "null model");
  const Model* m = &fm->impl;
  if (cfg_out) *cfg_out = m->cfg;
  if (compute_type) *compute_type = m->compute_type;
  if (device_index) *device_index = m->device;
  if (max_batch) *max_batch = m->max_batch;
  if (max_beam) *max_beam = m->max_beam;
  return FW_OK;
}

#define DEC_GROUP_RUN_ROWS 1600

int32_t fw_model_set_decode_batch(fw_model* fm, int32_t decode_batch) {
  FW_CHECK_ARG(fm, "null model");
  Model* m = &fm->impl;
  FW_CHECK_ARG(!m->decoder, "this model has joined another model's decoder");
  FW_CHECK_ARG(decode_batch >= 1, "decode_batch must be positive");
  {
    std::lock_guard<std::mutex> gl(m->grp.mu);
    FW_CHECK_ARG(m->grp.active_runs == 0 && !m->grp.gathering && m->grp.queue.empty() && !m->grp.resizing,
                 "decode runs are queued or in flight: set the decode batch before the first generate call or after the last one returned");
    m->grp.resizing = true;
  }
  struct Done {
    DecodeGroup& g;
    ~Done() {
      { std::lock_guard<std::mutex> gl(g.mu); g.resizing = false; }
      g.cv.notify_all();
    }
  } done{m->grp};
  DecodeLane* lane0 = m->lanes[0].get();
  std::lock_guard<std::mutex> lk(lane0->mu);
  FW_HIP(hipSetDevice(m->device));
  int want = std::max(decode_batch, m->max_batch) / m->max_batch * m->max_batch;
  int lanes_wanted = 2;
  if (const char* e = getenv("FWAMD_DECODE_LANES")) lanes_wanted = std::min(kMaxDecodeLanes, std::max(1, atoi(e)));
  const int n_lanes = want >= 4 * m->max_batch ? lanes_wanted : 1;
  const int max_rows = n_lanes >= 2 ? DEC_GROUP_RUN_ROWS : 2048;
  auto lane_of = [&](int pool_chunks) {
    int lc = pool_chunks;
    while (lc > m->max_batch && (int64_t)lc * m->max_beam > max_rows) lc -= m->max_batch;
    return lc;
  };
  size_t free_b = 0, total_b = 0;
  FW_HIP(hipMemGetInfo(&free_b, &total_b));
  for (const auto& l : m->lanes)
    if (l->gen) free_b += (size_t)gen_workspace_bytes(m, lane_chunks_of(m), m->decode_self_ctx);
  if (m->xpool) free_b += (size_t)cross_pool_bytes(m, std::max(m->decode_batch, m->max_batch));
  const int64_t budget = (int64_t)(0.7 * (double)free_b);
  const int NT = m->cfg.n_text_ctx;
  const int ctx_steps[] = {NT, 320, 224, 160};
  int self_ctx = NT;
  for (;;) {
    bool fits = false;
    for (int cs : ctx_steps) {
      if (cs > NT) continue;
      if (cross_pool_bytes(m, want) + n_lanes * gen_workspace_bytes(m, lane_of(want), cs) <= budget) { self_ctx = cs; fits = true; break; }
    }
    if (fits || want <= m->max_batch) break;
    want -= m->max_batch;
  }
  const int lane_batch = lane_of(want);
  const bool lanes_ok = n_lanes == (int)m->lanes.size();
  if (lane0->gen && m->xpool && lanes_ok && want == m->decode_batch && lane_batch == lane_chunks_of(m) &&
      self_ctx == m->decode_self_ctx)
    return FW_OK;
  if (lane0->stream) FW_HIP(hipStreamSynchronize(lane0->stream));
  auto reset = [&] {
    m->lanes.resize(1);
    gen_workspace_free(lane0);
    cross_pool_free(m);
    m->decode_batch = m->max_batch; m->lane_batch = 0; m->decode_self_ctx = 0;
  };
  reset();
  std::vector<std::unique_ptr<DecodeLane>> further;
  int rc = cross_pool_ensure(m, want);
  if (!rc) rc = gen_workspace_build(m, lane0, lane_batch, self_ctx);
  for (int k = 1; !rc && k < n_lanes; ++k) {
    further.emplace_back(new DecodeLane());
    further.back()->prof.on = m->prof.on;
    const hipError_t he = create_stream(&further.back()->spare, "DEC");
    if (he != hipSuccess) set_error("hipStreamCreate failed: %s", hipGetErrorString(he));
    rc = he != hipSuccess ? FW_ENODEV : gen_workspace_build(m, further.back().get(), lane_batch, self_ctx);
  }
  if (rc) { reset(); return rc; }
  m->decode_batch = want; m->lane_batch = lane_batch; m->decode_self_ctx = self_ctx;
  for (auto& l : further) m->lanes.push_back(std::move(l));
  return FW_OK;
}

int32_t fw_model_set_decode_lanes(fw_model* fm, int32_t lanes) {
  FW_CHECK_ARG(fm, "null model");
  Model* dm = decoder_of(&fm->impl);
  int have;
  {
    std::lock_guard<std::mutex> gl(dm->grp.mu);
    have = std::max(2, (int)dm->lanes.size());
    if (const char* e = getenv("FWAMD_DECODE_LANES")) have = std::max(have, std::min(kMaxDecodeLanes, atoi(e)));
  }
  FW_CHECK_ARG(lanes >= 1 && lanes <= have, "decode lanes: 1 .. %d", have);
  dm->grp.lanes_enabled.store(lanes);
  return FW_OK;
}

int32_t fw_model_set_merge_wait(fw_model* fm, int32_t wait_ms, int32_t fill_percent) {
  FW_CHECK_ARG(fm, "null model");
  FW_CHECK_ARG(wait_ms >= -1 && wait_ms <= 10000, "merge wait: -1 (one encoder pass), 0 (never) or milliseconds <= 10000");
  FW_CHECK_ARG(fill_percent >= 1 && fill_percent <= 100, "merge fill: 1 .. 100 percent of a run's chunk capacity");
  DecodeGroup& g = decoder_of(&fm->impl)->grp;
  g.merge_wait_ms.store(wait_ms);
  g.merge_fill_pct.store(fill_percent);
  return FW_OK;
}

int32_t fw_model_decode_batch(const fw_model* fm) {
  if (!fm) return 0;
  const Model* m = fm->impl.decoder ? fm->impl.decoder : &fm->impl;
  return std::max(m->decode_batch, m->max_batch);
}

int32_t fw_model_run_capacity(const fw_model* fm) {
  if (!fm) return 0;
  return lane_chunks_of(fm->impl.decoder ? fm->impl.decoder : &fm->impl);
}

int32_t fw_model_decode_stats(const fw_model* fm, int64_t* runs, int64_t* requests, int64_t* chunks,
                              int32_t* max_run_chunks) {
  FW_CHECK_ARG(fm, "null model");
  const Model* m = fm->impl.decoder ? fm->impl.decoder : &fm->impl;
  if (runs) *runs = m->grp.n_runs.load();
  if (requests) *requests = m->grp.n_requests.load();
  if (chunks) *chunks = m->grp.n_chunks.load();
  if (max_run_chunks) *max_run_chunks = m->grp.max_run_chunks.load();
  return FW_OK;
}

int32_t fw_model_join_decoder(fw_model* fm, fw_model* decoder) {
  FW_CHECK_ARG(fm && decoder && fm != decoder, "need two distinct models");
  Model* m = &fm->impl;
  Model* d = &decoder->impl;
  FW_CHECK_ARG(!d->decoder, "the decoder model has itself joined another decoder");
  FW_CHECK_ARG(m->device == d->device && m->blob == d->blob && m->max_batch == d->max_batch && m->max_beam == d->max_beam,
               "models that share a decoder must share device, weight blob, max_batch and max_beam");
  FW_CHECK_ARG(!m->decoder, "this model has already joined a decoder");
  DecodeLane* lane = m->lanes[0].get();
  std::lock_guard<std::mutex> lk(lane->mu);
  FW_HIP(hipSetDevice(m->device));
  if (lane->stream) FW_HIP(hipStreamSynchronize(lane->stream));
  gen_workspace_free(lane);
  cross_pool_free(m);
  {
    std::lock_guard<std::mutex> lk2(g_models_mu);
    d->dependents += 1;
  }
  m->decoder = d;
  return FW_OK;
}

int32_t fw_logmel(fw_model* fm, const float* pcm, const int64_t* offsets, int32_t B, float* out,
                  int32_t* n_frames_out) {
  FW_CHECK_ARG(fm && offsets && out, "null argument");
  Model* m = &fm->impl;
  FW_CHECK_ARG(B >= 1 && B <= m->max_batch, "batch %d exceeds max_batch %d", B, m->max_batch);
  std::lock_guard<std::mutex> lk(m->mu);
  FW_HIP(hipSetDevice(m->device));
  int64_t total; int mf;
  int rc = check_offsets(offsets, B, &total, &mf);
  if (rc) return rc;
  FW_CHECK_ARG(total == 0 || pcm, "null pcm");
  if ((rc = ensure_pcm(m, std::max<int64_t>(total, 1)))) return rc;
  if (total) FW_HIP(hipMemcpyAsync(m->ws_pcm, pcm, total * sizeof(float), hipMemcpyHostToDevice, m->stream));
  if ((rc = logmel_batch(m, m->ws_pcm, offsets, B, true, false))) return rc;
  FW_HIP(hipMemcpyAsync(out, m->ws_feat32, (size_t)B * m->cfg.n_mels * 3000 * sizeof(float), hipMemcpyDeviceToHost,
                        m->stream));
  if (n_frames_out)
    FW_HIP(hipMemcpyAsync(n_frames_out, m->ws_nframes, B * sizeof(int32_t), hipMemcpyDeviceToHost, m->stream));
  FW_HIP(hipStreamSynchronize(m->stream));
  return FW_OK;
}

int32_t fw_logmel_full(fw_model* fm, const float* pcm, int64_t n_samples, float* out, int64_t out_frames) {
  FW_CHECK_ARG(fm && out, "null argument");
  Model* m = &fm->impl;
  FW_CHECK_ARG(n_samples >= 0 && n_samples < (int64_t)1 << 30, "invalid n_samples");
  const int64_t nf = (n_samples + 160) / 160;
  FW_CHECK_ARG(out_frames == nf, "out_frames must be n_samples/160 + 1 = %lld, got %lld", (long long)nf,
               (long long)out_frames);
  std::lock_guard<std::mutex> lk(m->mu);
  FW_HIP(hipSetDevice(m->device));
  int rc;
  if ((rc = ensure_pcm(m, std::max<int64_t>(n_samples, 1)))) return rc;
  if (n_samples) FW_HIP(hipMemcpyAsync(m->ws_pcm, pcm, n_samples * sizeof(float), hipMemcpyHostToDevice, m->stream));
  const int stride = (int)((nf + 7) / 8 * 8);
  if ((rc = ensure_raw(m, 1, std::max(stride, 3008)))) return rc;
  const int rstride = std::max(stride, 3008);
  int64_t offs[2] = {0, n_samples};
  FW_HIP(hipMemcpyAsync(m->ws_offsets, offs, 2 * sizeof(int64_t), hipMemcpyHostToDevice, m->stream));
  float* dout = nullptr;
  if ((rc = dev_alloc_t(&dout, (size_t)m->cfg.n_mels * nf))) return rc;
  {
    ProfScope ps(m, PF_LOGMEL, 0, (double)n_samples * 4 + (double)m->cfg.n_mels * nf * 4);
    fwk::launch_logmel(m->stream, m->ws_pcm, m->ws_offsets, 1, (int)nf, m->lm_consts, m->lm_filtT, m->lm_mel_pad,
                       m->cfg.n_mels, m->ws_raw, (int64_t)m->cfg.n_mels * rstride, rstride, m->ws_chunk_max, 0,
                       (int)nf, dout, nullptr, m->c_pad, nullptr);
  }
  hipError_t he = hipMemcpyAsync(out, dout, (size_t)m->cfg.n_mels * nf * sizeof(float), hipMemcpyDeviceToHost,
                                 m->stream);
  if (he == hipSuccess) he = hipStreamSynchronize(m->stream);
  (void)hipFree(dout);
  if (he != hipSuccess) {
    set_error("logmel_full failed: %s", hipGetErrorString(he));
    return FW_ERUNTIME;
  }
  return FW_OK;
}

namespace {
struct EncodingMark {
  fw::DecodeGroup& g;
  std::chrono::steady_clock::time_point t0;
  explicit EncodingMark(fw::Model* m) : g(fw::decoder_of(m)->grp) {
    g.encoding.fetch_add(1);
    g.enc_mu.lock();
    t0 = std::chrono::steady_clock::now();
  }
  ~EncodingMark() {
    const int us = (int)std::chrono::duration_cast<std::chrono::microseconds>(std::chrono::steady_clock::now() - t0).count();
    const int old = g.enc_pass_us.load();
    g.enc_pass_us.store(old ? (3 * old + us) / 4 : us);
    g.enc_mu.unlock();
    g.encoding.fetch_sub(1);
    g.cv.notify_all();
  }
};
}

int32_t fw_encode(fw_model* fm, const float* features, int32_t B, fw_tensor** out) {
  FW_CHECK_ARG(fm && features && out, "null argument");
  Model* m = &fm->impl;
  FW_CHECK_ARG(B >= 1 && B <= m->max_batch, "batch %d exceeds max_batch %d", B, m->max_batch);
  EncodingMark mark(m);
  std::lock_guard<std::mutex> lk(m->mu);
  FW_HIP(hipSetDevice(m->device));
  FW_HIP(hipMemcpyAsync(m->ws_feat32, features, (size_t)B * m->cfg.n_mels * 3000 * sizeof(float),
                        hipMemcpyHostToDevice, m->stream));
  fwk::launch_features_to_cl(m->stream, m->ws_feat32, B, m->cfg.n_mels, 3000, m->ws_mel_cl, m->c_pad);
  fw_tensor* t = nullptr;
  int rc = new_tensor(m, B, &t);
  if (rc) return rc;
  if ((rc = run_encoder(m, B, t->impl.data))) {
    fw_tensor_free(t);
    return rc;
  }
  hipError_t he = hipStreamSynchronize(m->stream);
  if (he != hipSuccess) {
    fw_tensor_free(t);
    set_error("encode failed: %s", hipGetErrorString(he));
    return FW_ERUNTIME;
  }
  prof_collect(m->prof);
  *out = t;
  return FW_OK;
}

static int encode_pcm_common(Model* m, const float* pcm_dev, const int64_t* offsets, int B, fw_tensor** out) {
  int rc;
  if ((rc = logmel_batch(m, pcm_dev, offsets, B, false, true))) return rc;
  fw_tensor* t = nullptr;
  if ((rc = new_tensor(m, B, &t))) return rc;
  if ((rc = run_encoder(m, B, t->impl.data))) {
    fw_tensor_free(t);
    return rc;
  }
  hipError_t he = hipStreamSynchronize(m->stream);
  if (he != hipSuccess) {
    fw_tensor_free(t);
// ... 160 lines not shown
```

### faster_whisper_amd/csrc/gemm.hip

```cpp
#include "common.h"
#include "kernels.h"
#include <atomic>
#include <type_traits>

#define GB_M 256
#define GB_N 256
#define GB_UNIT_BYTES (128 * 128)
#define GB_SLOT_BYTES (4 * GB_UNIT_BYTES)
#define GB_LDS_BYTES (8 * 64 * 272)

typedef int intx16 __attribute__((ext_vector_type(16)));

#ifndef GB_TL
#define GB_TL(slot)
#endif

#define GB_BARRIER()                      \
  do {                                    \
    asm volatile("" ::: "memory");         \
    __builtin_amdgcn_s_barrier();         \
    asm volatile("" ::: "memory");         \
  } while (0)

template <bool TRANS, bool I8, bool LAYERED = false>
__global__ __launch_bounds__(512) void gemm_f16_kernel(fwk::GemmParams p) {
  extern __shared__ __attribute__((aligned(16))) char smem_raw[];
  constexpr int ES = I8 ? 1 : 2;

  const int tid = threadIdx.x;
  const int lane = tid & 63;
  const int wave = __builtin_amdgcn_readfirstlane(tid >> 6);
  const int hi = lane >> 5, l31 = lane & 31;
  const int wm = wave >> 2, wn = wave & 3;

  int bid = xcd_remap(blockIdx.x, gridDim.x);
  int mp, nt;
  if (p.blk_n > 0) {
    const int per_band = p.blk_m * p.nNt;
    const int band = bid / per_band, r = bid - band * per_band;
    int bm = p.n_mp - band * p.blk_m; if (bm > p.blk_m) bm = p.blk_m;
    const int per_blk = bm * p.blk_n;
    const int cb = r / per_blk, rr = r - cb * per_blk;
    const int mi = rr / p.blk_n;
    mp = band * p.blk_m + mi;
    nt = cb * p.blk_n + (rr - mi * p.blk_n);
  } else {
    mp = bid / p.nNt;
    nt = bid - mp * p.nNt;
  }
  const int z = mp / p.nMt;
  const int mt = mp - z * p.nMt;
  int layer = 0;
  if (LAYERED) { layer = nt / p.nNt_layer; nt -= layer * p.nNt_layer; }
  const int m0 = mt * GB_M, n0 = nt * GB_N;

  const char* Ab = reinterpret_cast<const char*>(p.A) + (size_t)z * p.a_bstride * ES;
  const char* Wb = reinterpret_cast<const char*>(p.W) + (LAYERED ? (size_t)layer * p.w_lstride * ES : 0);
  const half_t* const biasp = (LAYERED && p.bias) ? p.bias + (size_t)layer * p.bias_lstride : p.bias;
  half_t* const Cp = LAYERED ? p.C + (size_t)layer * p.c_lstride : p.C;

  unsigned goff[4][2];
#pragma unroll
  for (int i = 0; i < 2; ++i) {
    const int u = (i * 8 + wave) * 8 + (lane >> 3);
    const int c = (lane & 7) ^ ((u >> 1) & 7);
#pragma unroll
    for (int h = 0; h < 2; ++h) {
      int am = m0 + (u >> 6) * 128 + (u & 63) + h * 64; if (am > p.M - 1) am = p.M - 1;
      int wr = n0 + (u >> 5) * 64 + (u & 31) + h * 32; if (wr > p.N - 1) wr = p.N - 1;
      goff[h][i] = (unsigned)((size_t)am * p.lda * ES + c * 16);
      goff[2 + h][i] = (unsigned)((size_t)wr * p.ldw * ES + c * 16);
    }
  }
  const int nk = p.K * ES / 128;
  auto issue = [&](int unit, int kt) {
    char* dst = smem_raw + (kt & 1) * GB_SLOT_BYTES + unit * GB_UNIT_BYTES;
    const char* base = unit < 2 ? Ab : Wb;
    const unsigned koff = (unsigned)kt * 128u;
#pragma unroll
    for (int i = 0; i < 2; ++i)
      __builtin_amdgcn_global_load_lds((const __attribute__((address_space(1))) void*)(base + (size_t)(goff[unit][i] + koff)),
                                       (__attribute__((address_space(3))) void*)(dst + (i * 8 + wave) * 1024), 16, 0, 0);
  };

  floatx16 accf[4][2];
  intx16 acci[4][2];
#pragma unroll
  for (int i = 0; i < 4; ++i)
#pragma unroll
    for (int j = 0; j < 2; ++j) { accf[i][j] = floatx16{0}; acci[i][j] = intx16{0}; }

  int arow[2], akey[2];
#pragma unroll
  for (int i = 0; i < 2; ++i) {
    const int u = wm * 64 + i * 32 + l31;
    arow[i] = u * 128;
    akey[i] = (u >> 1) & 7;
  }
  const int bu = wn * 32 + l31;
  const int brow = bu * 128, bkey = (bu >> 1) & 7;

  intx4 fa[2][4], fb0[4], fb1[4];
  auto read_a = [&](const char* unit) {
#pragma unroll
    for (int i = 0; i < 2; ++i)
#pragma unroll
      for (int ks = 0; ks < 4; ++ks)
        fa[i][ks] = *reinterpret_cast<const intx4*>(unit + arow[i] + (((ks * 2 + hi) ^ akey[i]) << 4));
  };
  auto read_b = [&](const char* unit, intx4 (&fb)[4]) {
#pragma unroll
    for (int ks = 0; ks < 4; ++ks) fb[ks] = *reinterpret_cast<const intx4*>(unit + brow + (((ks * 2 + hi) ^ bkey) << 4));
  };
  auto mma = [&](int ah, int ni, const intx4 (&fb)[4]) {
    __builtin_amdgcn_s_setprio(1);
#pragma unroll
    for (int ks = 0; ks < 4; ++ks)
#pragma unroll
      for (int i = 0; i < 2; ++i) {
        const int mi = ah * 2 + i;
        const intx4 opa = TRANS ? fa[i][ks] : fb[ks];
        const intx4 opb = TRANS ? fb[ks] : fa[i][ks];
        if (I8) acci[mi][ni] = __builtin_amdgcn_mfma_i32_32x32x32_i8(opa, opb, acci[mi][ni], 0, 0, 0);
        else accf[mi][ni] = __builtin_amdgcn_mfma_f32_32x32x16_f16(__builtin_bit_cast(half8_t, opa),
                                                                 __builtin_bit_cast(half8_t, opb), accf[mi][ni], 0, 0, 0);
      }
    __builtin_amdgcn_s_setprio(0);
  };
  auto seg_wait = [&](bool issued) {
    if (issued) asm volatile("s_waitcnt vmcnt(8)" ::: "memory");
    else asm volatile("s_waitcnt vmcnt(0)" ::: "memory");
  };

  const int mw = m0 + wm * 128, nw = n0 + wn * 64;
  const bool rowmajor = !TRANS && p.head_rows == 0;
  const half_t* const Rb = (rowmajor && p.res) ? p.res + (size_t)z * p.r_bstride : nullptr;
  const int ep_rr = lane >> 3, ep_cc = (lane & 7) * 8;
  const bool vec_ok = (p.ldc % 8 == 0) && (p.c_bstride % 8 == 0) && (!Rb || ((p.ldr % 8 == 0) && (p.r_bstride % 8 == 0)));
  const half4_t hz4 = {(half_t)0.f, (half_t)0.f, (half_t)0.f, (half_t)0.f};
  half4_t bias4[2][4] = {{hz4, hz4, hz4, hz4}, {hz4, hz4, hz4, hz4}};
  half_t biasT[2] = {(half_t)0.f, (half_t)0.f};
  half8_t resv[8];
  auto load_bias = [&]() {
    if (!biasp) return;
#pragma unroll
    for (int ni = 0; ni < 2; ++ni) {
      if (TRANS) {
        int n = nw + ni * 32 + l31; if (n > p.N - 1) n = p.N - 1;
        biasT[ni] = biasp[n];
      } else {
#pragma unroll
        for (int g = 0; g < 4; ++g) {
          int n = nw + ni * 32 + 8 * g + 4 * hi; if (n > p.N - 4) n = p.N - 4;
          bias4[ni][g] = *reinterpret_cast<const half4_t*>(biasp + n);
        }
      }
    }
  };
  auto load_res = [&](int half) {
    if (!Rb || !vec_ok || p.N < 8) return;
#pragma unroll
    for (int j = 0; j < 8; ++j) {
      int m = mw + half * 64 + j * 8 + ep_rr; if (m > p.M - 1) m = p.M - 1;
      int n = nw + ep_cc; if (n + 8 > p.N) n = (p.N - 8) & ~7;
      resv[j] = *reinterpret_cast<const half8_t*>(Rb + (size_t)m * p.ldr + n);
    }
  };

  issue(2, 0); issue(0, 0); issue(3, 0); issue(1, 0);
  if (nk > 1) { issue(2, 1); issue(0, 1); }
  seg_wait(nk > 1);
  GB_BARRIER();
  if (wm == 1) GB_BARRIER();

  auto tile = [&](int kt, auto N1, auto N2) {
    constexpr bool n1 = decltype(N1)::value, n2 = decltype(N2)::value;
    const char* slot = smem_raw + (kt & 1) * GB_SLOT_BYTES;
    GB_TL(0);
    read_a(slot);
    read_b(slot + 2 * GB_UNIT_BYTES, fb0);
    if (n1) issue(3, kt + 1);
    seg_wait(n1);
    GB_TL(1);
    GB_BARRIER();
    GB_TL(2);
    mma(0, 0, fb0);
    GB_TL(3);
    GB_BARRIER();
    GB_TL(4);
    read_b(slot + 3 * GB_UNIT_BYTES, fb1);
    if (n1) issue(1, kt + 1);
    seg_wait(n1);
    GB_TL(5);
    GB_BARRIER();
    GB_TL(6);
    mma(0, 1, fb1);
    GB_TL(7);
    GB_BARRIER();
    GB_TL(8);
    read_a(slot + GB_UNIT_BYTES);
    if (n2) issue(2, kt + 2);
    seg_wait(n2);
    GB_TL(9);
    GB_BARRIER();
    GB_TL(10);
    mma(1, 0, fb0);
    GB_TL(11);
    GB_BARRIER();
    GB_TL(12);
    if (n2) issue(0, kt + 2);
    seg_wait(n2);
    if (!n1 && !n2) { load_bias(); if (!I8) load_res(0); }
    GB_TL(13);
    GB_BARRIER();
    GB_TL(14);
    mma(1, 1, fb1);
    GB_TL(15);
    GB_BARRIER();
  };
  using T_ = std::true_type;
  using F_ = std::false_type;
  int kt = 0;
  for (; kt + 2 < nk; ++kt) tile(kt, T_{}, T_{});
  if (kt + 1 < nk) { tile(kt, T_{}, F_{}); ++kt; }
  if (kt < nk) tile(kt, F_{}, F_{});
  if (wm == 0) GB_BARRIER();

  const float* sa = I8 ? p.a_scale + (size_t)z * p.as_bstride : nullptr;
  if (!TRANS && p.head_rows == 0) {
    constexpr int EP_STRIDE = 272;
    char* ep = smem_raw + wave * (64 * EP_STRIDE);
    half_t* Cb = Cp + (size_t)z * p.c_bstride;
    const int rr = ep_rr, cc = ep_cc;
#pragma unroll
    for (int half = 0; half < 2; ++half) {
      if (half == 1 || I8) load_res(half);
#pragma unroll
      for (int ni = 0; ni < 2; ++ni)
#pragma unroll
        for (int mh = 0; mh < 2; ++mh) {
          const int mi = half * 2 + mh;
          const int r = mh * 32 + l31;
          int mc = mw + half * 64 + r; if (mc > p.M - 1) mc = p.M - 1;
          const float sam = I8 ? sa[mc] : 1.f;
#pragma unroll
          for (int g = 0; g < 4; ++g) {
            const int c = ni * 32 + 8 * g + 4 * hi;
            int n = nw + c; if (n > p.N - 4) n = p.N - 4;
            floatx4 v;
#pragma unroll
            for (int e = 0; e < 4; ++e)
              v[e] = I8 ? (float)acci[mi][ni][g * 4 + e] * sam * p.w_scale[n + e] : accf[mi][ni][g * 4 + e];
            if (biasp) {
#pragma unroll
              for (int e = 0; e < 4; ++e) v[e] += (float)bias4[ni][g][e];
            }
            if (p.act == 1) {
#pragma unroll
              for (int e = 0; e < 4; ++e) v[e] = gelu_erf(v[e]);
            }
            *reinterpret_cast<floatx4*>(ep + r * EP_STRIDE + c * 4) = v;
          }
        }
#pragma unroll
      for (int j = 0; j < 8; ++j) {
        const int r = j * 8 + rr;
        const int m = mw + half * 64 + r, n = nw + cc;
        const floatx4 v0 = *reinterpret_cast<const floatx4*>(ep + r * EP_STRIDE + cc * 4);
        const floatx4 v1 = *reinterpret_cast<const floatx4*>(ep + r * EP_STRIDE + cc * 4 + 16);
        if (m >= p.M || n >= p.N) continue;
        float v[8] = {v0[0], v0[1], v0[2], v0[3], v1[0], v1[1], v1[2], v1[3]};
        if (vec_ok && n + 8 <= p.N) {
          if (Rb) {
            const half8_t rv = resv[j];
#pragma unroll
            for (int e = 0; e < 8; ++e) v[e] += (float)rv[e];
          }
          half8_t o;
#pragma unroll
          for (int e = 0; e < 8; ++e) o[e] = (half_t)v[e];
          *reinterpret_cast<half8_t*>(Cb + (size_t)m * p.ldc + n) = o;
        } else {
          for (int e = 0; e < 8 && n + e < p.N; ++e) {
            float t = v[e];
            if (Rb) t += (float)Rb[(size_t)m * p.ldr + n + e];
            Cb[(size_t)m * p.ldc + n + e] = (half_t)t;
          }
        }
      }
    }
  } else if (p.head_rows > 0) {
    constexpr int FS = 144;
    char* ep = smem_raw + wave * (64 * FS);
    half_t* Cb = Cp + (size_t)z * p.c_bstride;
    if (nw < p.N) {
      half_t* Hb = Cb + (size_t)(nw >> 6) * p.head_rows * 64;
      const int g4 = lane >> 4, j = lane & 15;
#pragma unroll
      for (int half = 0; half < 2; ++half) {
#pragma unroll
        for (int ni = 0; ni < 2; ++ni)
#pragma unroll
          for (int mh = 0; mh < 2; ++mh) {
            const int mi = half * 2 + mh;
            if (!TRANS) {
              const int r = mh * 32 + l31;
              int mc = mw + half * 64 + r; if (mc > p.M - 1) mc = p.M - 1;
              const float sam = I8 ? sa[mc] : 1.f;
#pragma unroll
              for (int g = 0; g < 4; ++g) {
                const int c = ni * 32 + 8 * g + 4 * hi;
                int n = nw + c; if (n > p.N - 4) n = p.N - 4;
                half4_t o;
#pragma unroll
                for (int e = 0; e < 4; ++e) {
                  float v = I8 ? (float)acci[mi][ni][g * 4 + e] * sam * p.w_scale[n + e] : accf[mi][ni][g * 4 + e];
                  if (biasp) v += (float)bias4[ni][g][e];
                  if (p.act == 1) v = gelu_erf(v);
                  o[e] = (half_t)v;
                }
                *reinterpret_cast<half4_t*>(ep + r * FS + c * 2) = o;
              }
            } else {
              const int c = ni * 32 + l31;
              int n = nw + c; if (n > p.N - 1) n = p.N - 1;
              const float bv = (float)biasT[ni];
              const float swn = I8 ? p.w_scale[n] : 1.f;
#pragma unroll
              for (int g = 0; g < 4; ++g) {
                const int r = mh * 32 + 8 * g + 4 * hi;
                half4_t o;
#pragma unroll
                for (int e = 0; e < 4; ++e) {
                  int mm = mw + half * 64 + r + e; if (mm > p.M - 1) mm = p.M - 1;
                  float v = (I8 ? (float)acci[mi][ni][g * 4 + e] * swn * sa[mm] : accf[mi][ni][g * 4 + e]) + bv;
                  if (p.act == 1) v = gelu_erf(v);
                  o[e] = (half_t)v;
                }
                *reinterpret_cast<half4_t*>(ep + c * FS + r * 2) = o;
              }
            }
          }
#pragma unroll
        for (int gl = 0; gl < 2; ++gl) {
          const int key0 = mw + half * 64 + gl * 32;
          if (key0 >= p.M) continue;
          half_t* Gb = Hb + (size_t)(key0 >> 5) * 4 * 512;
#pragma unroll
          for (int q = 0; q < 4; ++q) {
            intx4 v;
            if (!TRANS) {
              const int kl = gl * 32 + 8 * (j >> 2) + 4 * (q >> 1) + (j & 3);
              v = *reinterpret_cast<const intx4*>(ep + kl * FS + (32 * (q & 1) + 8 * g4) * 2);
              if (mw + half * 64 + kl < p.M) *reinterpret_cast<intx4*>(Gb + ((size_t)q * 64 + lane) * 8) = v;
            } else {
              const int kl = gl * 32 + 8 * g4;
              v = *reinterpret_cast<const intx4*>(ep + (16 * q + j) * FS + kl * 2);
              const int left = p.M - (mw + half * 64 + kl);
              if (left <= 0) continue;
              if (left < 8) {
                half8_t h = __builtin_bit_cast(half8_t, v);
#pragma unroll
                for (int e = 0; e < 8; ++e)
                  if (e >= left) h[e] = (half_t)0.f;
                v = __builtin_bit_cast(intx4, h);
              }
              *reinterpret_cast<intx4*>(Gb + ((size_t)q * 64 + lane) * 8) = v;
            }
          }
        }
      }
    }
  } else if (TRANS && !I8 && p.vt_stage) {
    constexpr int TS = 272;
    char* ep = smem_raw + wave * (64 * TS);
    half_t* Cb = Cp + (size_t)z * p.c_bstride;
#pragma unroll
    for (int ni = 0; ni < 2; ++ni) {
      const int c = ni * 32 + l31;
      const float bv = (float)biasT[ni];
#pragma unroll
      for (int mi = 0; mi < 4; ++mi)
#pragma unroll
        for (int g = 0; g < 4; ++g) {
          const int r = mi * 32 + 8 * g + 4 * hi;
          half4_t o;
#pragma unroll
          for (int e = 0; e < 4; ++e) {
            float v = accf[mi][ni][g * 4 + e] + bv;
            if (p.act == 1) v = gelu_erf(v);
            o[e] = (half_t)v;
          }
          *reinterpret_cast<half4_t*>(ep + c * TS + r * 2) = o;
        }
    }
    const int rr = lane >> 4, cc = (lane & 15) * 8;
#pragma unroll 4
    for (int j = 0; j < 16; ++j) {
      const int c = j * 4 + rr;
      const int n = nw + c, m = mw + cc;
      const intx4 v = *reinterpret_cast<const intx4*>(ep + c * TS + cc * 2);
      if (n >= p.N || m >= p.M) continue;
      half_t* dst = Cb + (size_t)n * p.ldc + m;
      if (m + 8 <= p.M) {
        *reinterpret_cast<intx4*>(dst) = v;
      } else {
        const half8_t h = __builtin_bit_cast(half8_t, v);
#pragma unroll
        for (int e = 0; e < 8; ++e)
          if (m + e < p.M) dst[e] = h[e];
      }
    }
  } else {
    half_t* Cb = Cp + (size_t)z * p.c_bstride;
#pragma unroll
    for (int mi = 0; mi < 4; ++mi)
#pragma unroll
      for (int ni = 0; ni < 2; ++ni) {
        const int n = n0 + wn * 64 + ni * 32 + l31;
        if (n >= p.N) continue;
        const float bv = (float)biasT[ni];
        const float swn = I8 ? p.w_scale[n] : 1.f;
#pragma unroll
        for (int g = 0; g < 4; ++g) {
          const int m = m0 + wm * 128 + mi * 32 + 8 * g + 4 * hi;
          half4_t o;
#pragma unroll
          for (int e = 0; e < 4; ++e) {
            int mm = m + e; if (mm > p.M - 1) mm = p.M - 1;
            float v = (I8 ? (float)acci[mi][ni][g * 4 + e] * swn * sa[mm] : accf[mi][ni][g * 4 + e]) + bv;
            if (p.act == 1) v = gelu_erf(v);
            o[e] = (half_t)v;
          }
          half_t* dst = Cb + (size_t)n * p.ldc + m;
          if (m + 3 < p.M) {
            *reinterpret_cast<half4_t*>(dst) = o;
          } else {
#pragma unroll
            for (int e = 0; e < 4; ++e)
              if (m + e < p.M) dst[e] = o[e];
          }
        }
      }
  }
}

namespace fwk {

std::atomic<int> g_gemm_order{1};
std::atomic<int> g_gemm_vt_stage{1};

int launch_gemm(hipStream_t st, const GemmParams& pin, int batch, bool trans) {
  GemmParams p = pin;
  const bool i8 = p.a_scale != nullptr;
  const int es = i8 ? 1 : 2;
  if (p.K <= 0 || (p.K * es) % 128 != 0) return -1;
  if (((p.lda * es) % 16) || ((p.ldw * es) % 16) || ((p.a_bstride * es) % 16)) return -1;
  if (!trans && ((p.N % 4) || (p.ldc % 4) || (p.c_bstride % 4))) return -1;
  if (i8 && !p.w_scale) return -1;
  p.nMt = (p.M + GB_M - 1) / GB_M;
  p.nNt_layer = (p.N + GB_N - 1) / GB_N;
  if (p.n_layers > 1 && (i8 || p.res)) return -1;
  p.nNt = p.nNt_layer * (p.n_layers > 1 ? p.n_layers : 1);
  p.n_mp = p.nMt * batch;
  p.blk_m = p.blk_n = 0;
  p.vt_stage = (trans && !i8 && p.head_rows == 0 && g_gemm_vt_stage.load(std::memory_order_relaxed) == 1 && p.ldc % 8 == 0 &&
                p.c_bstride % 8 == 0) ? 1 : 0;
  if (g_gemm_order.load(std::memory_order_relaxed) == 1 && p.nNt > 1 && p.n_mp > 1) {
    int bn = 1, best = 1 << 30;
    for (int c = 1; c <= p.nNt && c <= 16; ++c) {
      if (p.nNt % c) continue;
      const int cost = c + (32 + c - 1) / c;
      if (cost <= best) { best = cost; bn = c; }
    }
    p.blk_n = bn;
    p.blk_m = 32 / bn > 1 ? 32 / bn : 1;
  }
  const int lds = GB_LDS_BYTES;
  static std::atomic<unsigned long long> attr_done{0};
  int dev = 0;
  (void)hipGetDevice(&dev);
  if (!((attr_done.load(std::memory_order_acquire) >> (dev & 63)) & 1ull)) {
    (void)hipFuncSetAttribute(reinterpret_cast<const void*>(gemm_f16_kernel<false, false>),
                              hipFuncAttributeMaxDynamicSharedMemorySize, lds);
    (void)hipFuncSetAttribute(reinterpret_cast<const void*>(gemm_f16_kernel<true, false>),
                              hipFuncAttributeMaxDynamicSharedMemorySize, lds);
    (void)hipFuncSetAttribute(reinterpret_cast<const void*>(gemm_f16_kernel<false, true>),
                              hipFuncAttributeMaxDynamicSharedMemorySize, lds);
    (void)hipFuncSetAttribute(reinterpret_cast<const void*>(gemm_f16_kernel<true, true>),
                              hipFuncAttributeMaxDynamicSharedMemorySize, lds);
    attr_done.fetch_or(1ull << (dev & 63), std::memory_order_release);
  }
  const int grid = p.nMt * p.nNt * batch;
  if (p.n_layers > 1) {
    static std::atomic<unsigned long long> attr_l{0};
    if (!((attr_l.load(std::memory_order_acquire) >> (dev & 63)) & 1ull)) {
      (void)hipFuncSetAttribute(reinterpret_cast<const void*>(gemm_f16_kernel<false, false, true>),
                                hipFuncAttributeMaxDynamicSharedMemorySize, lds);
      (void)hipFuncSetAttribute(reinterpret_cast<const void*>(gemm_f16_kernel<true, false, true>),
                                hipFuncAttributeMaxDynamicSharedMemorySize, lds);
      attr_l.fetch_or(1ull << (dev & 63), std::memory_order_release);
    }
    if (trans) gemm_f16_kernel<true, false, true><<<grid, 512, lds, st>>>(p);
    else gemm_f16_kernel<false, false, true><<<grid, 512, lds, st>>>(p);
    return 0;
  }
  if (i8) {
    if (trans) gemm_f16_kernel<true, true><<<grid, 512, lds, st>>>(p);
    else gemm_f16_kernel<false, true><<<grid, 512, lds, st>>>(p);
  } else {
    if (trans) gemm_f16_kernel<true, false><<<grid, 512, lds, st>>>(p);
    else gemm_f16_kernel<false, false><<<grid, 512, lds, st>>>(p);
  }
  return 0;
}

}
```

### faster_whisper_amd/csrc/hooks.hip

```cpp
#include "engine.h"

#include <math.h>
#include <string.h>

#include <algorithm>

#include "dec_kernels.h"
#include "kernels.h"

using namespace fw;
using fwd::FIN_CAP;
using fwd::GenDev;

namespace {

struct HookBufs {
  std::vector<void*> p;
  HookBufs() = default;
  HookBufs(const HookBufs&) = delete;
  HookBufs& operator=(const HookBufs&) = delete;
  ~HookBufs() { for (void* q : p) (void)hipFree(q); }
  template <typename T>
  int alloc(T** dst, size_t n) {
    int rc = dev_alloc_t(dst, n);
// ... 280 lines not shown
  std::vector<half_t> xh((size_t)R16 * d, (half_t)0.f);
  for (int r = 0; r < R; ++r)
    for (int k = 0; k < d; ++k) xh[i8 ? (size_t)r * d + k : frag_pos(r, k, d, 32)] = (half_t)x[(size_t)r * d + k];
  HookBufs db;
  half_t* d_x;
  float* d_out;
  int rc, lr;
  if ((rc = db.upload(&d_x, xh.data(), xh.size())) || (rc = db.alloc(&d_out, (size_t)R * V))) return rc;
  if (i8) {
    int8_t* d_xq;
    float* d_xs;
    if ((rc = db.alloc(&d_xq, (size_t)R16 * d)) || (rc = db.alloc(&d_xs, (size_t)R16)) || (rc = db.zero(d_xq, (size_t)R16 * d, st)))
      return rc;
    fwk::launch_quant_rows(st, d_x, d, m->dec_ln.g, m->dec_ln.b, d_xq, d_xs, R, d, 1);
    lr = fwd::launch_dec_logits(st, true, d_xq, d_xs, m->logits.wq, m->logits.wscale, nullptr, nullptr, d_out, V, R, V, d);
  } else {
    lr = fwd::launch_dec_logits(st, false, d_x, nullptr, m->logits.w, nullptr, m->logits.s1, m->logits.cf, d_out, V, R, V,
                                d);
  }
  FW_HIP(hipStreamSynchronize(st));
  if (lr != 0) {
    set_error("logits projection test failed: unsupported shape");
    return FW_ERUNTIME;
  }
  return download(out, d_out, (size_t)R * V);
}

int32_t fw_bench_dec_linear(fw_model* fm, int32_t R, int32_t N, int32_t K, int32_t lnf, int32_t variant, int32_t iters,
                            float* us_out) {
  FW_CHECK_ARG(fm && us_out && R > 0 && N > 0 && K > 0 && iters > 0, "bad argument");
  Model* m = &fm->impl;
  std::lock_guard<std::mutex> lk(m->mu);
  FW_HIP(hipSetDevice(m->device));
  hipStream_t st = m->stream;
  const size_t wn = (size_t)N * K;
  const int copies = (int)std::max<size_t>(2, ((size_t)640 << 20) / (wn * 2));
  const size_t rp = ((size_t)R + 15) / 16 * 16;
  HookBufs db;
  half_t *dW, *dX, *dO, *dB;
  float *dS, *dC;
  std::vector<uint16_t> stage;
  int rc;
  if ((rc = db.alloc(&dW, wn * copies)) || (rc = db.alloc(&dX, rp * K)) || (rc = db.alloc(&dO, rp * N)) ||
      (rc = db.alloc(&dB, (size_t)N)) || (rc = db.alloc(&dS, (size_t)N)) || (rc = db.alloc(&dC, (size_t)N)) ||
      (rc = fill_lcg(dW, wn, stage, 2463534242u, 1e-3f)) || (rc = fill_lcg(dX, rp * K, stage, 2463534242u, 1e-3f)) ||
      (rc = db.zero(dB, (size_t)N * 2, st)) || (rc = db.zero(dS, (size_t)N * 4, st)) || (rc = db.zero(dC, (size_t)N * 4, st)))
    return rc;
  for (int c = 1; c < copies; ++c) FW_HIP(hipMemcpy(dW + (size_t)c * wn, dW, wn * 2, hipMemcpyDeviceToDevice));
  float ms = 0.f;
  rc = time_launches(st, 4, iters, [&](int i) {
    return fwd::launch_dec_gemm_frag_variant(st, variant, lnf != 0, dX, dW + (size_t)(i % copies) * wn, dB, dS, dC, dO, R, N, K);
  }, &ms);
  if (rc == LAUNCH_REFUSED) { set_error("fw_bench_dec_linear: unsupported shape / variant"); return FW_EINVAL; }
  if (rc) return rc;
  *us_out = ms * 1000.f / (float)iters;
  return FW_OK;
}

int32_t fw_bench_gemm(fw_model* fm, int32_t M, int32_t N, int32_t K, int32_t batch, int32_t a_pad, int32_t w_pad,
                      int32_t trans, int32_t iters, float* ms_out) {
  FW_CHECK_ARG(fm && ms_out && M > 0 && N > 0 && K > 0 && batch > 0 && iters > 0, "bad argument");
  Model* m = &fm->impl;
  std::lock_guard<std::mutex> lk(m->mu);
  FW_HIP(hipSetDevice(m->device));
  const bool i8 = m->compute_type == FW_COMPUTE_INT8_FLOAT16;
  const int64_t lda = K + a_pad, ldw = K + w_pad;
  const int64_t ldct = (M + 63) / 64 * 64;
  const size_t na = (size_t)batch * M * lda, nw = (size_t)N * ldw,
               nc = trans ? (size_t)batch * N * ldct : (size_t)batch * M * N;
  const size_t ha = i8 ? (na + 1) / 2 : na, hw = i8 ? (nw + 1) / 2 : nw;
  HookBufs db;
  half_t *dA, *dW, *dC;
  float *dsa = nullptr, *dsw = nullptr;
  std::vector<uint16_t> stage;
  int rc;
  if ((rc = db.alloc(&dA, ha)) || (rc = db.alloc(&dW, hw)) || (rc = db.alloc(&dC, nc)) ||
      (rc = fill_lcg(dA, ha, stage, 12345u, 1e-3f)) || (rc = fill_lcg(dW, hw, stage, 12345u, 1e-3f)))
    return rc;
  if (i8 && ((rc = db.alloc(&dsa, (size_t)batch * M)) || (rc = db.alloc(&dsw, (size_t)N)) ||
             (rc = db.zero(dsa, (size_t)batch * M * 4, m->stream)) || (rc = db.zero(dsw, (size_t)N * 4, m->stream))))
    return rc;
  fwk::GemmParams p;
  memset(&p, 0, sizeof(p));
  p.A = dA; p.lda = lda; p.a_bstride = (int64_t)M * lda;
  p.W = dW; p.ldw = ldw;
  p.C = dC; p.ldc = trans ? ldct : N; p.c_bstride = trans ? (int64_t)N * ldct : (int64_t)M * N;
  p.M = M; p.N = N; p.K = K;
  p.a_scale = dsa; p.as_bstride = M; p.w_scale = dsw;
  float ms = 0.f;
  rc = time_launches(m->stream, 1, iters, [&](int) { return fwk::launch_gemm(m->stream, p, batch, trans != 0); }, &ms);
  if (rc == LAUNCH_REFUSED) { set_error("gemm bench failed: unsupported shape"); return FW_ERUNTIME; }
  if (rc) return rc;
  *ms_out = ms / (float)iters;
  return FW_OK;
}

int32_t fw_bench_gemm_epi(fw_model* fm, int32_t M, int32_t N, int32_t K, int32_t batch, int32_t lda_in, int32_t trans,
                          int32_t bias, int32_t act, int32_t res, int32_t n_layers, int32_t iters, float* ms_out) {
  FW_CHECK_ARG(fm && ms_out && M > 0 && N > 0 && K > 0 && batch > 0 && iters > 0 && n_layers >= 1, "bad argument");
  FW_CHECK_ARG(res >= 0 && res <= 2 && !(res && (trans || n_layers > 1)), "residual: row-major single-layer output only");
  Model* m = &fm->impl;
  FW_CHECK_ARG(m->compute_type != FW_COMPUTE_INT8_FLOAT16, "float16 models only");
  std::lock_guard<std::mutex> lk(m->mu);
  FW_HIP(hipSetDevice(m->device));
  const int64_t lda = lda_in > 0 ? lda_in : K;
  const bool layered = n_layers > 1;
  const int64_t kvp = (M + 31) / 32 * 32;
  const int64_t ldct = layered ? kvp : (M + 63) / 64 * 64;
  const int64_t c_bs = layered ? (int64_t)N * kvp : (trans ? (int64_t)N * ldct : (int64_t)M * N);
  const int64_t c_ls = c_bs * batch;
  const size_t na = (size_t)batch * ((size_t)M * lda + K), nw = (size_t)N * K * n_layers, nc = (size_t)c_ls * n_layers;
  const size_t nr1 = res == 1 ? (size_t)batch * M * N : (size_t)M * N;
  const int copies = res == 1 ? (int)std::max<size_t>(2, ((size_t)640 << 20) / (nr1 * 2)) : 1;
  HookBufs db;
  half_t *dA, *dW, *dC, *dB, *dR = nullptr;
  std::vector<uint16_t> stage;
  int rc;
  if ((rc = db.alloc(&dA, na)) || (rc = db.alloc(&dW, nw)) || (rc = db.alloc(&dC, nc)) || (rc = db.alloc(&dB, (size_t)N * n_layers)) ||
      (res && (rc = db.alloc(&dR, nr1 * copies))) || (rc = fill_lcg(dA, na, stage, 12345u, 1e-3f)) ||
      (rc = fill_lcg(dW, nw, stage, 12345u, 1e-3f)) || (rc = fill_lcg(dB, (size_t)N * n_layers, stage, 777u, 1e-3f)) ||
      (res && (rc = fill_lcg(dR, nr1, stage, 4242u, 1e-3f))) || (rc = db.zero(dC, nc * 2, m->stream)))
    return rc;
  for (int c = 1; res && c < copies; ++c) FW_HIP(hipMemcpy(dR + (size_t)c * nr1, dR, nr1 * 2, hipMemcpyDeviceToDevice));
  fwk::GemmParams p;
  memset(&p, 0, sizeof(p));
  p.A = dA; p.lda = lda; p.a_bstride = (int64_t)M * lda;
  p.W = dW; p.ldw = K;
  p.bias = bias ? dB : nullptr;
  p.C = dC; p.ldc = layered ? (trans ? kvp : N) : (trans ? ldct : N); p.c_bstride = c_bs;
  p.M = M; p.N = N; p.K = K;
  p.act = act;
  if (layered) {
    p.head_rows = (int)kvp;
    p.n_layers = n_layers; p.w_lstride = (int64_t)N * K; p.bias_lstride = N; p.c_lstride = c_ls;
  }
  p.ldr = N; p.r_bstride = res == 1 ? (int64_t)M * N : 0;
  float ms = 0.f;
  rc = time_launches(m->stream, 1, iters, [&](int i) {
    p.res = res ? dR + (size_t)(i % copies) * nr1 : nullptr;
    return fwk::launch_gemm(m->stream, p, batch, trans != 0);
  }, &ms);
  if (rc == LAUNCH_REFUSED) { set_error("gemm epilogue bench failed: unsupported shape"); return FW_ERUNTIME; }
  if (rc) return rc;
  *ms_out = ms / (float)iters;
  return FW_OK;
}

int32_t fw_bench_dec_linear_epi(fw_model* fm, int32_t R, int32_t N, int32_t K, int32_t lnf, int32_t variant, int32_t act,
                                int32_t res, int32_t outs, int32_t iters, float* us_out) {
  FW_CHECK_ARG(fm && us_out && R > 0 && N > 0 && K > 0 && iters > 0, "bad argument");
  FW_CHECK_ARG((outs & 3) != 0 && (!res || (outs & 1)), "needs an output; the residual is the row-major output in place");
  FW_CHECK_ARG(variant == 0 || variant == 5 || (variant >= 10 && variant <= 12), "unknown variant %d", variant);
  Model* m = &fm->impl;
  std::lock_guard<std::mutex> lk(m->mu);
  FW_HIP(hipSetDevice(m->device));
  hipStream_t st = m->stream;
  const size_t wn = (size_t)N * K;
  const int copies = (int)std::max<size_t>(2, ((size_t)640 << 20) / (wn * 2));
  const size_t rp = ((size_t)R + 15) / 16 * 16, on = rp * N;
  const int ocopies = (int)std::max<size_t>(2, ((size_t)640 << 20) / (on * 2));
  HookBufs db;
  half_t *dW, *dX, *dO, *dF, *dB;
  float *dS, *dC;
  std::vector<uint16_t> stage;
  int rc;
  if ((rc = db.alloc(&dW, wn * copies)) || (rc = db.alloc(&dX, rp * K)) || (rc = db.alloc(&dO, on * ocopies)) ||
      (rc = db.alloc(&dF, on)) || (rc = db.alloc(&dB, (size_t)N)) || (rc = db.alloc(&dS, (size_t)N)) || (rc = db.alloc(&dC, (size_t)N)) ||
      (rc = fill_lcg(dW, wn, stage, 2463534242u, 1e-3f)) || (rc = fill_lcg(dX, rp * K, stage, 2463534242u, 1e-3f)) ||
      (rc = db.zero(dO, on * ocopies * 2, st)) || (rc = db.zero(dB, (size_t)N * 2, st)) || (rc = db.zero(dS, (size_t)N * 4, st)) ||
      (rc = db.zero(dC, (size_t)N * 4, st)))
    return rc;
  for (int c = 1; c < copies; ++c) FW_HIP(hipMemcpy(dW + (size_t)c * wn, dW, wn * 2, hipMemcpyDeviceToDevice));
  float ms = 0.f;
  rc = time_launches(st, 4, iters, [&](int i) {
    const half_t* w = dW + (size_t)(i % copies) * wn;
    half_t* o = dO + (size_t)(i % ocopies) * on;
    half_t* op = (outs & 1) ? o : nullptr;
    half_t* of = (outs & 2) ? dF : nullptr;
    const half_t* r = res ? o : nullptr;
    const half_t* b = lnf ? nullptr : dB;
    const float *s1 = lnf ? dS : nullptr, *cf = lnf ? dC : nullptr;
    if (variant >= 10) return fwd::launch_dec_gemm_big(st, variant - 10, dX, w, b, s1, cf, r, N, op, N, of, R, N, K, act);
    if (variant == 5) return fwd::launch_dec_gemm_skinny(st, dX, w, b, s1, cf, r, N, op, N, of, R, N, K, act);
    return fwd::launch_dec_gemm_frag(st, dX, w, b, s1, cf, r, N, op, N, of, R, N, K, act);
  }, &ms);
  if (rc == LAUNCH_REFUSED) { set_error("fw_bench_dec_linear_epi: unsupported shape / variant"); return FW_EINVAL; }
  if (rc) return rc;
  *us_out = ms * 1000.f / (float)iters;
  return FW_OK;
}

int32_t fw_test_layernorm(fw_model* fm, const float* x, const float* g, const float* b, int32_t rows, int32_t d,
                          float* out) {
  return test_layernorm_impl(fm, x, g, b, rows, d, 0, out);
}
int32_t fw_test_layernorm_frag(fw_model* fm, const float* x, const float* g, const float* b, int32_t rows, int32_t d,
                               int32_t frag, float* out) {
  return test_layernorm_impl(fm, x, g, b, rows, d, frag, out);
}

int32_t fw_test_quant_rows(fw_model* fm, const float* x, int32_t rows, int32_t d, int64_t ldx, const float* ln_g,
                           const float* ln_b, int32_t frag, int8_t* xq, float* scale) {
  FW_CHECK_ARG(fm && x && xq && scale && rows >= 1 && rows <= (1 << 20), "bad argument");
  FW_CHECK_ARG((ln_g == nullptr) == (ln_b == nullptr), "ln_g and ln_b go together");
  FW_CHECK_ARG(d >= 64 && d % 64 == 0 && d <= (ln_g ? 1536 : 5120), "d %% 64 == 0, d <= 1536 with LayerNorm, <= 5120 without");
  FW_CHECK_ARG(ldx >= d && ldx % 8 == 0 && ldx <= (1 << 20), "ldx >= d, ldx %% 8 == 0");
  Model* m = &fm->impl;
  std::lock_guard<std::mutex> lk(m->mu);
  FW_HIP(hipSetDevice(m->device));
  const int R16 = (rows + 15) / 16 * 16;
  std::vector<int8_t> hq((size_t)R16 * d);
  HookBufs db;
  half_t *dx, *dg = nullptr, *dlb = nullptr;
  int8_t* dq;
  float* ds;
  int rc;
  if ((rc = db.upload_f16(&dx, x, (size_t)(rows - 1) * ldx + d)) || (ln_g && (rc = db.upload_f16(&dg, ln_g, d))) ||
      (ln_b && (rc = db.upload_f16(&dlb, ln_b, d))) || (rc = db.alloc(&dq, hq.size())) || (rc = db.alloc(&ds, (size_t)R16)) ||
      (rc = db.zero(dq, hq.size(), m->stream)))
    return rc;
  fwk::launch_quant_rows(m->stream, dx, ldx, dg, dlb, dq, ds, rows, d, frag ? 1 : 0);
  FW_HIP(hipStreamSynchronize(m->stream));
  if ((rc = download(hq.data(), dq, hq.size())) || (rc = download(scale, ds, (size_t)rows))) return rc;
  for (int r = 0; r < rows; ++r)
    for (int k = 0; k < d; ++k) xq[(size_t)r * d + k] = hq[frag ? frag_pos(r, k, d, 64) : (size_t)r * d + k];
  return FW_OK;
}

int32_t fw_test_cross_kv_frag_index(int32_t vt, int32_t kvp, int32_t N, int64_t* idx) {
  FW_CHECK_ARG(idx && kvp >= 32 && kvp % 32 == 0 && N >= 64 && N % 64 == 0, "need kvp %% 32 == 0, N %% 64 == 0");
  for (int mm = 0; mm < kvp; ++mm)
    for (int n = 0; n < N; ++n) idx[(size_t)mm * N + n] = (int64_t)cross_kv_frag_pos(vt != 0, kvp, mm, n);
  return FW_OK;
}

int32_t fw_test_gemm_ex(fw_model* fm, const float* A, int64_t a_elems, int64_t lda, int64_t a_bstride, const float* W,
                        const float* bias, const float* res, int64_t r_elems, int64_t ldr, int64_t r_bstride, float* C,
                        int64_t c_elems, int64_t c_off, int64_t ldc, int64_t c_bstride, int64_t c_lstride, int32_t M,
                        int32_t N, int32_t K, int32_t batch, int32_t n_layers, int32_t act, int32_t trans,
                        int32_t head_rows, int32_t use_int8, const float* ln_g, const float* ln_b) {
  FW_CHECK_ARG(fm && A && W && C, "null argument");
  const int64_t dim_max = 1 << 20, cnt_max = 1 << 12, str_max = (int64_t)1 << 40;
  FW_CHECK_ARG(M >= 1 && N >= 1 && K >= 1 && M <= dim_max && N <= dim_max && K <= dim_max, "bad M / N / K");
  FW_CHECK_ARG(batch >= 1 && n_layers >= 1 && batch <= cnt_max && n_layers <= cnt_max, "bad batch / n_layers");
  for (int64_t v : {a_elems, lda, a_bstride, r_elems, ldr, r_bstride, c_elems, c_off, ldc, c_bstride, c_lstride})
    FW_CHECK_ARG(v >= 0 && v <= str_max, "negative or oversized count / stride");
  FW_CHECK_ARG(act == 0 || act == 1, "act is 0 or 1");
  FW_CHECK_ARG((ln_g == nullptr) == (ln_b == nullptr) && (!ln_g || use_int8), "ln_g / ln_b: both, and only with use_int8");
  const bool rowmajor = !trans && head_rows == 0;
  FW_CHECK_ARG(!res || (rowmajor && n_layers == 1), "a residual needs the row-major single-layer form");
  FW_CHECK_ARG(n_layers == 1 || (!use_int8 && act == 0), "the layered launch is fp16 without activation");
  FW_CHECK_ARG(head_rows == 0 || (head_rows > 0 && head_rows % 32 == 0 && head_rows >= M && N % 64 == 0),
               "fragment-major output: head_rows %% 32 == 0, head_rows >= M, N %% 64 == 0");
  FW_CHECK_ARG(c_off % 8 == 0 && c_lstride % 8 == 0, "c_off and c_lstride must be multiples of 8");
  if (use_int8) FW_CHECK_ARG(lda == K && a_bstride == (int64_t)M * K, "int8: A is contiguous [batch * M][K]");
  const int64_t a_last = (int64_t)(batch - 1) * a_bstride + (int64_t)(M - 1) * lda + (K - 1);
  FW_CHECK_ARG(a_last < a_elems, "the launch reads A[%lld], a_elems = %lld", (long long)a_last, (long long)a_elems);
  if (res) {
    const int64_t r_last = (int64_t)(batch - 1) * r_bstride + (int64_t)(M - 1) * ldr + (N - 1);
    FW_CHECK_ARG(r_last < r_elems, "the launch reads res[%lld], r_elems = %lld", (long long)r_last, (long long)r_elems);
  }
  const int64_t chunk_last = head_rows > 0 ? (int64_t)(N / 64 - 1) * head_rows * 64 + (int64_t)((M - 1) / 32 + 1) * 2048 - 1
                             : trans       ? (int64_t)(N - 1) * ldc + (M - 1)
                                           : (int64_t)(M - 1) * ldc + (N - 1);
  const int64_t c_last = c_off + (int64_t)(n_layers - 1) * c_lstride + (int64_t)(batch - 1) * c_bstride + chunk_last;
  FW_CHECK_ARG(c_last < c_elems, "the launch writes C[%lld], c_elems = %lld", (long long)c_last, (long long)c_elems);

  Model* m = &fm->impl;
  std::lock_guard<std::mutex> lk(m->mu);
  if (use_int8) {
    const int64_t T = m->cfg.n_audio_ctx;
    if (m->compute_type != FW_COMPUTE_INT8_FLOAT16 || (int64_t)batch * M * K > (int64_t)m->max_batch * T * 4 * m->cfg.d_model ||
        (int64_t)batch * M > (int64_t)m->max_batch * T || (ln_g && K > 1536)) {
      set_error("int8 gemm test needs an int8_float16 model, batch*M*K within its quantisation workspace, K <= 1536 with LayerNorm");
      return FW_EINVAL;
    }
  }
  FW_HIP(hipSetDevice(m->device));
  HookBufs db;
  half_t *dA, *dW, *dB = nullptr, *dR = nullptr, *dC, *dG = nullptr, *dLb = nullptr;
  int rc;
  if ((rc = db.upload_f16(&dA, A, (size_t)a_elems)) || (rc = db.upload_f16(&dW, W, (size_t)n_layers * N * K)) ||
      (bias && (rc = db.upload_f16(&dB, bias, (size_t)n_layers * N))) || (res && (rc = db.upload_f16(&dR, res, (size_t)r_elems))) ||
      (rc = db.upload_f16(&dC, C, (size_t)c_elems)) ||
      (ln_g && ((rc = db.upload_f16(&dG, ln_g, K)) || (rc = db.upload_f16(&dLb, ln_b, K)))))
    return rc;
  LinearW L{dW, dB, nullptr, nullptr, nullptr, nullptr, N, K};
  if (use_int8) {
    int8_t* dWq;
    float* dWs;
    if ((rc = upload_quant_w(db, W, N, K, [&](int n, int k) { return (size_t)n * K + k; }, &dWq, &dWs))) return rc;
    L.wq = dWq; L.wscale = dWs;
    LNW ln{dG, dLb};
    rc = run_linear_i8(m, L, dA, ln_g ? &ln : nullptr, dC + c_off, ldc, c_bstride, dR, ldr, r_bstride, M, batch, act,
                       trans != 0, head_rows);
  } else if (n_layers > 1) {
    rc = run_linear_layers(m, L, n_layers, (int64_t)N * K, bias ? N : 0, dA, lda, a_bstride, dC + c_off, ldc, c_bstride,
                           c_lstride, M, batch, trans != 0, head_rows, nullptr);
  } else {
    rc = run_linear(m, L, dA, lda, a_bstride, dC + c_off, ldc, c_bstride, dR, ldr, r_bstride, M, batch, act, trans != 0,
                    head_rows, nullptr);
  }
  return rc ? rc : download_f16(m->stream, C, dC, (size_t)c_elems);
}

int32_t fw_test_attention(fw_model* fm, const float* q, const float* k, const float* v, int32_t B, int32_t H,
                          int32_t T, float* out) {
  FW_CHECK_ARG(fm && q && k && v && out, "null argument");
  Model* m = &fm->impl;
  std::lock_guard<std::mutex> lk(m->mu);
  FW_HIP(hipSetDevice(m->device));
  const int d = H * 64, tp = (T + 63) / 64 * 64;
  const size_t n = (size_t)B * T * d;
  std::vector<float> vt((size_t)B * d * tp, 0.f);
  for (int b = 0; b < B; ++b)
    for (int t = 0; t < T; ++t)
      for (int c = 0; c < d; ++c) vt[((size_t)b * d + c) * tp + t] = v[((size_t)b * T + t) * d + c];
  HookBufs db;
  half_t *dq, *dk, *dvt, *dout;
  int rc;
  if ((rc = db.upload_f16(&dq, q, n)) || (rc = db.upload_f16(&dk, k, n)) || (rc = db.upload_f16(&dvt, vt.data(), vt.size())) ||
      (rc = db.alloc(&dout, n)))
    return rc;
  fwk::launch_attn_enc(m->stream, dq, dk, d, (int64_t)T * d, dvt, tp, (int64_t)d * tp, dout, d, (int64_t)T * d, B, H,
                       T);
  return download_f16(m->stream, out, dout, n);
}

int32_t fw_bench_attention(fw_model* fm, int32_t B, int32_t H, int32_t T, int32_t variant, int32_t iters, float* ms_out) {
  FW_CHECK_ARG(fm && ms_out && B > 0 && H > 0 && T > 0 && iters > 0, "bad argument");
  Model* m = &fm->impl;
  std::lock_guard<std::mutex> lk(m->mu);
  FW_HIP(hipSetDevice(m->device));
  const int d = H * 64, tp = (T + 63) / 64 * 64;
  const size_t nqk = (size_t)B * T * 2 * d, nvt = (size_t)B * d * tp, no = (size_t)B * T * d;
  HookBufs db;
  half_t *dqk, *dvt, *dout;
  std::vector<uint16_t> stage;
  int rc;
  if ((rc = db.alloc(&dqk, nqk)) || (rc = db.alloc(&dvt, nvt)) || (rc = db.alloc(&dout, no)) ||
      (rc = fill_lcg(dqk, nqk, stage, 777u, 2e-3f)) || (rc = fill_lcg(dvt, nvt, stage, 777u, 2e-3f)))
    return rc;
  float ms = 0.f;
  rc = time_launches(m->stream, 1, iters, [&](int) {
    fwk::launch_attn_enc(m->stream, dqk, dqk + d, 2 * d, (int64_t)T * 2 * d, dvt, tp, (int64_t)d * tp, dout, d, (int64_t)T * d, B,
                         H, T, variant);
    return 0;
  }, &ms);
  if (rc) return rc;
  *ms_out = ms / (float)iters;
  return FW_OK;
}

int32_t fw_test_dec_self_attn(fw_model* fm, const float* qkv, float* kcache, float* vcache, const uint8_t* kvidx,
                              int32_t n_chunks, int32_t kmul, int32_t Kbeam, int32_t H, int32_t n_ctx, int32_t cache_ctx,
                              int32_t pos_fixed, int32_t P, int32_t step, int32_t blk_n, int32_t frag, float* out) {
  FW_CHECK_ARG(fm && qkv && kcache && vcache && kvidx && out, "null argument");
  FW_CHECK_ARG(n_chunks >= 1 && H >= 1 && kmul >= 1 && kmul <= 16 && Kbeam >= 1 && Kbeam <= 255, "bad geometry");
  FW_CHECK_ARG(n_ctx >= 1 && n_ctx <= 448 && cache_ctx >= 1 && cache_ctx <= n_ctx, "need 1 <= cache_ctx <= n_ctx <= 448");
  FW_CHECK_ARG(blk_n >= 0 && (blk_n == 0 ? kmul <= Kbeam : (kmul == blk_n && pos_fixed >= 0)),
               "blk_n = 0: kmul <= Kbeam; blk_n > 0: kmul == blk_n and pos_fixed >= 0");
  const int pos0 = pos_fixed >= 0 ? pos_fixed : P - 1 + step;
  const int pos_last = pos0 + (blk_n > 0 ? blk_n - 1 : 0);
  FW_CHECK_ARG(pos0 >= 0 && pos_last < cache_ctx, "positions %d..%d outside the cache (%d)", pos0, pos_last, cache_ctx);
  const int d = H * 64, R = n_chunks * kmul, R16 = (R + 15) / 16 * 16, R_total = n_chunks * Kbeam;
  FW_CHECK_ARG(blk_n == 0 || fwd::self_attn_block_ok(n_ctx, cache_ctx, d, R_total), "position blocks need n_ctx %% 4 == 0");
  const size_t n_tab = (size_t)2 * R_total * n_ctx, n_cache = (size_t)R_total * H * cache_ctx * 64;
  for (size_t i = 0; i < n_tab; ++i)
    FW_CHECK_ARG(kvidx[i] < Kbeam, "kvidx[%zu] = %d is not a beam of %d", i, (int)kvidx[i], Kbeam);
  Model* m = &fm->impl;
  std::lock_guard<std::mutex> lk(m->mu);
  FW_HIP(hipSetDevice(m->device));
  hipStream_t st = m->stream;
  HookBufs db;
  half_t *d_qkv, *d_kc, *d_vc, *d_out;
  uint8_t* d_idx;
  int* d_step;
  int rc;
  if ((rc = db.upload_f16(&d_qkv, qkv, (size_t)R * 3 * d)) || (rc = db.upload_f16(&d_kc, kcache, n_cache)) ||
      (rc = db.upload_f16(&d_vc, vcache, n_cache)) || (rc = db.alloc(&d_out, (size_t)R16 * d)) ||
      (rc = db.upload(&d_idx, kvidx, n_tab)) || (rc = db.upload(&d_step, &step, 1)) ||
      (rc = db.zero(d_out, (size_t)R16 * d * 2, st)))
    return rc;
  fwd::launch_self_attn(st, d_qkv, d, d_kc, d_vc, n_ctx, cache_ctx, H, d_idx, Kbeam, kmul, d_out, R, d_step, pos_fixed, P,
                        R_total, frag ? 1 : 0, blk_n);
  FW_HIP(hipGetLastError());
  if ((rc = download_f16(st, kcache, d_kc, n_cache)) || (rc = download_f16(st, vcache, d_vc, n_cache))) return rc;
  return frag ? download_f16_frag(st, out, d_out, R, d) : download_f16(st, out, d_out, (size_t)R * d);
}

int32_t fw_test_dec_cross_attn(fw_model* fm, const float* q, const float* k, const float* v, int32_t n_enc, int32_t T,
                               int32_t H, int32_t B, int32_t kmul, int32_t kv_div, const int32_t* slot_map,
                               const int32_t* done, int32_t frag, float k_pad, float* out) {
  FW_CHECK_ARG(fm && q && k && v && slot_map && out, "null argument");
  FW_CHECK_ARG(n_enc >= 1 && T >= 1 && H >= 1 && B >= 1 && kmul >= 1 && kmul <= 16 && kv_div >= 1, "bad geometry");
  const int n_map = (B + kv_div - 1) / kv_div;
  for (int i = 0; i < n_map; ++i)
    FW_CHECK_ARG(slot_map[i] >= 0 && slot_map[i] < n_enc, "slot_map[%d] = %d outside [0, %d)", i, slot_map[i], n_enc);
  const int d = H * 64, kvp = (T + 31) / 32 * 32, R = B * kmul, R16 = (R + 15) / 16 * 16;
  const size_t blk = (size_t)d * kvp;
  std::vector<float> kf((size_t)n_enc * blk), vf((size_t)n_enc * blk, 0.f);
  for (int e = 0; e < n_enc; ++e)
    for (int t = 0; t < kvp; ++t)
      for (int n = 0; n < d; ++n) {
        const size_t src = ((size_t)e * T + t) * d + n;
        kf[e * blk + cross_kv_frag_pos(false, kvp, t, n)] = t < T ? k[src] : k_pad;
        if (t < T) vf[e * blk + cross_kv_frag_pos(true, kvp, t, n)] = v[src];
      }
  std::vector<float> of((size_t)R16 * d, 0.f);
  for (int r = 0; r < R; ++r)
    for (int n = 0; n < d; ++n) of[frag ? frag_pos(r, n, d, 32) : (size_t)r * d + n] = out[(size_t)r * d + n];
  Model* m = &fm->impl;
  std::lock_guard<std::mutex> lk(m->mu);
  FW_HIP(hipSetDevice(m->device));
  HookBufs db;
  half_t *d_q, *d_k, *d_vt, *d_out;
  int *d_map, *d_done = nullptr;
  int rc;
  if ((rc = db.upload_f16(&d_q, q, (size_t)R * d)) || (rc = db.upload_f16(&d_k, kf.data(), kf.size())) ||
      (rc = db.upload_f16(&d_vt, vf.data(), vf.size())) || (rc = db.upload_f16(&d_out, of.data(), of.size())) ||
      (rc = db.upload(&d_map, slot_map, (size_t)n_map)) || (done && (rc = db.upload(&d_done, done, (size_t)B))))
    return rc;
  fwd::launch_cross_attn(m->stream, d_q, d, d_k, d_vt, T, kvp, kmul, d_out, B, H, d_done, kv_div, frag ? 1 : 0, d_map);
  FW_HIP(hipGetLastError());
  return frag ? download_f16_frag(m->stream, out, d_out, R, d) : download_f16(m->stream, out, d_out, (size_t)R * d);
}

int32_t fw_test_dec_cross_probs(fw_model* fm, const float* q, const float* k, int32_t B, int32_t T, int32_t H,
                                const int32_t* heads, int32_t n_sel, int32_t n_tok, int32_t tok_idx, int32_t blk_n,
                                float* probs) {
  FW_CHECK_ARG(fm && q && k && heads && probs, "null argument");
  const int blk = blk_n > 0 ? blk_n : 1;
  FW_CHECK_ARG(B >= 1 && T >= 1 && H >= 1 && n_sel >= 1 && blk_n >= 0 && blk <= 16, "bad geometry");
  FW_CHECK_ARG(tok_idx >= 0 && tok_idx + blk <= n_tok, "tokens %d..%d outside [0, %d)", tok_idx, tok_idx + blk - 1, n_tok);
  for (int i = 0; i < n_sel; ++i) FW_CHECK_ARG(heads[i] >= 0 && heads[i] < H, "heads[%d] = %d outside [0, %d)", i, heads[i], H);
  const int d = H * 64, kvp = (T + 31) / 32 * 32;
  const size_t blkk = (size_t)d * kvp, n_probs = (size_t)B * n_sel * n_tok * T;
  std::vector<float> kf((size_t)B * blkk, 0.f);
  for (int b = 0; b < B; ++b)
    for (int t = 0; t < T; ++t)
      for (int n = 0; n < d; ++n) kf[b * blkk + cross_kv_frag_pos(false, kvp, t, n)] = k[((size_t)b * T + t) * d + n];
  Model* m = &fm->impl;
  std::lock_guard<std::mutex> lk(m->mu);
  FW_HIP(hipSetDevice(m->device));
  HookBufs db;
  half_t *d_q, *d_k;
  int* d_heads;
  float* d_p;
  int rc;
  if ((rc = db.upload_f16(&d_q, q, (size_t)B * blk * d)) || (rc = db.upload_f16(&d_k, kf.data(), kf.size())) ||
      (rc = db.upload(&d_heads, heads, (size_t)n_sel)) || (rc = db.upload(&d_p, probs, n_probs)))
    return rc;
  fwd::launch_cross_probs(m->stream, d_q, d, d_k, T, kvp, d_heads, n_sel, n_sel, d_p, n_tok, tok_idx, B, blk_n);
  FW_HIP(hipGetLastError());
  FW_HIP(hipStreamSynchronize(m->stream));
  return download(probs, d_p, n_probs);
}

int32_t fw_test_dec_softmax_pick(fw_model* fm, const float* logits, int32_t rows, int32_t V, int32_t row_mul,
                                 const int32_t* target, int32_t nospeech, float* out) {
  FW_CHECK_ARG(fm && logits && target && out, "null argument");
  FW_CHECK_ARG(rows >= 1 && V >= 1 && row_mul >= 1, "bad geometry");
  FW_CHECK_ARG(!nospeech || (target[0] >= 0 && target[0] < V), "no-speech id %d outside [0, %d)", target[0], V);
  Model* m = &fm->impl;
  std::lock_guard<std::mutex> lk(m->mu);
  FW_HIP(hipSetDevice(m->device));
  HookBufs db;
  const size_t n_lg = (size_t)rows * row_mul * V;
  float *d_lg, *d_out;
  int* d_t;
  int rc;
  if ((rc = db.upload(&d_lg, logits, n_lg)) || (rc = db.alloc(&d_out, (size_t)rows)) || (rc = db.alloc(&d_t, (size_t)rows))) return rc;
  FW_HIP(hipMemcpy(d_t, target, (size_t)(nospeech ? 1 : rows) * sizeof(int), hipMemcpyHostToDevice));
  if (nospeech) fwd::launch_nospeech(m->stream, d_lg, V, row_mul, target[0], d_out, rows);
  else fwd::launch_token_prob(m->stream, d_lg, V, d_t, d_out, 1, 0, rows, row_mul);
  FW_HIP(hipGetLastError());
  FW_HIP(hipStreamSynchronize(m->stream));
  return download(out, d_out, (size_t)rows);
}

static int32_t logits_rules_hook(fw_model* fm, const float* logits, int32_t R, const int32_t* hist, int32_t n,
                                 const float* cum, const fw_gen_opts* o, int32_t with_timestamps, float* cand_val,
                                 int32_t* cand_tok, float* cand_lp, const fwd::SmpRow* smp = nullptr) {
  FW_CHECK_ARG(fm && logits && cum && o && cand_val && cand_tok && R >= 1 && n >= 0, "bad arguments");
  Model* m = &fm->impl;
  const fw_config& c = m->cfg;
  const int K = o->beam_size;
  const bool sampling = K == 1 && o->sampling_topk != 1;
  FW_CHECK_ARG(K >= 1 && K <= 16 && R % K == 0 && n < c.n_text_ctx && (n == 0 || hist), "bad geometry");
  FW_CHECK_ARG(c.n_vocab <= LP_SUP_WORDS * 64, "vocabulary too large for the rules kernel");
  FW_HIP(hipSetDevice(m->device));
  GenDev gp;
  memset(&gp, 0, sizeof(gp));
  gp.B = R / K; gp.K = K; gp.R = R; gp.V = c.n_vocab; gp.n_text_ctx = c.n_text_ctx;
  gp.sample = sampling ? 1 : 0;
  gp.inv_temp = 1.0f;
  gp.with_ts = with_timestamps ? 1 : 0;
  gp.suppress_blank = o->suppress_blank ? 1 : 0;
  gp.min_new = o->min_new_tokens;
  gp.mits = o->max_initial_timestamp_index;
  gp.ngram = o->no_repeat_ngram_size;
  gp.rep_pen = o->repetition_penalty;
  gp.eot = c.tok_eot; gp.no_ts = c.tok_no_timestamps; gp.ts_begin = c.tok_timestamp_begin;
  gp.n_sup_begin = c.n_suppress_begin;
  for (int i = 0; i < c.n_suppress_begin; ++i) gp.sup_begin[i] = c.suppress_begin[i];
  std::vector<unsigned long long> mask(LP_SUP_WORDS, 0ull);
  for (int i = 0; i < o->n_suppress_tokens; ++i) {
    const int t = o->suppress_tokens[i];
    if (t >= 0 && t < c.n_vocab) mask[t >> 6] |= 1ull << (t & 63);
  }
  const size_t NT = (size_t)c.n_text_ctx;
  std::vector<int> h2(2 * (size_t)R * NT, 0);
  std::vector<float> c2(2 * (size_t)R, 0.f);
  const int cur = n & 1;
  for (int r = 0; r < R; ++r) {
    for (int i = 0; i < n; ++i) h2[((size_t)cur * R + r) * NT + i] = hist[(size_t)r * n + i];
    c2[(size_t)cur * R + r] = cum[r];
  }
  std::vector<float> hv((size_t)R * 32);
  std::vector<int> ht((size_t)R * 32);
  HookBufs db;
  std::vector<float> hl(cand_lp ? hv.size() : 0);
  float *d_lg, *d_cum, *d_cv, *d_cl = nullptr;
  int *d_hist, *d_step, *d_done, *d_ct;
  unsigned long long* d_bits;
  int rc;
  if ((rc = db.upload(&d_lg, logits, (size_t)R * c.n_vocab)) || (rc = db.upload(&d_cum, c2.data(), c2.size())) ||
      (rc = db.upload(&d_hist, h2.data(), h2.size())) || (rc = db.upload(&d_step, &n, 1)) ||
      (rc = db.upload(&d_bits, mask.data(), mask.size())) || (rc = db.alloc(&d_done, (size_t)R)) ||
      (rc = db.alloc(&d_cv, hv.size())) || (rc = db.alloc(&d_ct, ht.size())) || (rc = db.zero(d_done, (size_t)R * sizeof(int), nullptr)) ||
      (rc = db.zero(d_cv, hv.size() * sizeof(float), nullptr)) || (rc = db.zero(d_ct, ht.size() * sizeof(int), nullptr)))
    return rc;
  if (cand_lp && ((rc = db.alloc(&d_cl, hl.size())) || (rc = db.zero(d_cl, hl.size() * sizeof(float), nullptr)))) return rc;
  fwd::SmpRow* d_smp = nullptr;
  if (sampling) {
    std::vector<fwd::SmpRow> tab((size_t)R);
    for (int r = 0; r < R; ++r)
      tab[r] = smp ? smp[r]
                   : fwd::SmpRow{1.0f / o->sampling_temperature, (unsigned)(o->seed & 0xffffffffu), (unsigned)(o->seed >> 32), 0};
    if ((rc = db.upload(&d_smp, tab.data(), tab.size()))) return rc;
  }
  fwd::launch_logits_process(nullptr, gp, d_lg, d_bits, d_hist, d_cum, d_step, d_done, d_cv, d_ct, d_cl, d_smp);
  FW_HIP(hipGetLastError());
  FW_HIP(hipDeviceSynchronize());
  if ((rc = download(hv.data(), d_cv, hv.size())) || (rc = download(ht.data(), d_ct, ht.size()))) return rc;
  if (cand_lp && (rc = download(hl.data(), d_cl, hl.size()))) return rc;
  const int C = sampling ? 1 : 2 * K;
  for (int r = 0; r < R; ++r)
    for (int j = 0; j < C; ++j) {
      cand_val[(size_t)r * C + j] = hv[(size_t)r * 32 + j];
      cand_tok[(size_t)r * C + j] = ht[(size_t)r * 32 + j];
      if (cand_lp) cand_lp[(size_t)r * C + j] = hl[(size_t)r * 32 + j];
    }
  return FW_OK;
}

int32_t fw_test_logits_rules(fw_model* fm, const float* logits, int32_t R, const int32_t* hist, int32_t n,
                             const float* cum, const fw_gen_opts* o, int32_t with_timestamps, float* cand_val,
                             int32_t* cand_tok) {
  return logits_rules_hook(fm, logits, R, hist, n, cum, o, with_timestamps, cand_val, cand_tok, nullptr);
}

int32_t fw_test_logits_rules_lp(fw_model* fm, const float* logits, int32_t R, const int32_t* hist, int32_t n,
                                const float* cum, const fw_gen_opts* o, int32_t with_timestamps, float* cand_val,
                                int32_t* cand_tok, float* cand_lp) {
  FW_CHECK_ARG(cand_lp, "null argument");
  return logits_rules_hook(fm, logits, R, hist, n, cum, o, with_timestamps, cand_val, cand_tok, cand_lp);
}

int32_t fw_test_logits_rules_smp_tab(fw_model* fm, const float* logits, int32_t R, const int32_t* hist, int32_t n,
                                     const float* cum, const fw_gen_opts* o, int32_t with_timestamps,
                                     const float* inv_temp, const uint64_t* seed, const int32_t* row0, float* cand_val,
                                     int32_t* cand_tok, float* cand_lp) {
  FW_CHECK_ARG(o && inv_temp && seed && row0 && cand_lp && R >= 1, "null argument");
  FW_CHECK_ARG(o->beam_size == 1 && o->sampling_topk == 0, "the options must select sampling (beam_size 1, sampling_topk 0)");
  std::vector<fwd::SmpRow> tab((size_t)R);
  for (int r = 0; r < R; ++r) {
    FW_CHECK_ARG(row0[r] >= 0 && row0[r] <= r && inv_temp[r] > 0.f, "row %d: row0 must lie in [0, row], inv_temp must be positive", r);
    tab[r] = {inv_temp[r], (unsigned)(seed[r] & 0xffffffffu), (unsigned)(seed[r] >> 32), row0[r]};
  }
  return logits_rules_hook(fm, logits, R, hist, n, cum, o, with_timestamps, cand_val, cand_tok, cand_lp, tab.data());
}

int32_t fw_test_graph_captures(const fw_model* fm, int64_t* out) {
  FW_CHECK_ARG(fm && out, "null argument");
  const Model* m = fm->impl.decoder ? fm->impl.decoder : &fm->impl;
  *out = m->grp.graph_captures.load();
  return FW_OK;
}

struct BeamLpArgs { const float* cand_lp; const float* lphist; float* fin_lp; float* lphist2; };
static int32_t beam_update_hook(fw_model* fm, int32_t B, int32_t K, int32_t NT, int32_t V, int32_t P, int32_t step,
                                int32_t budget, int32_t max_fin, float lp_pow, int32_t eot, const float* cand_val,
                                const int32_t* cand_tok, const int32_t* hist, const uint8_t* kvidx, const float* cum,
                                int32_t sentinel_i, float sentinel_f, int32_t* done, int32_t* n_done, int32_t* n_fin,
                                int32_t* fin_tok, int32_t* fin_len, float* fin_score, float* fin_cum, int32_t* hist2,
                                uint8_t* kvidx2, float* cum2, int32_t* cur_tok, const BeamLpArgs* lp) {
  FW_CHECK_ARG(fm && cand_val && cand_tok && cum && done && n_done && n_fin && fin_tok && fin_len && fin_score &&
                   fin_cum && hist2 && kvidx2 && cum2 && cur_tok, "null argument");
  FW_CHECK_ARG(K >= 1 && K <= 16, "need 1 <= K <= 16 (K = %d)", K);
  FW_CHECK_ARG(B >= 1 && B <= 4096, "need 1 <= B <= 4096 (B = %d)", B);
  FW_CHECK_ARG(NT >= 1 && NT <= 4096 && V >= 1, "need 1 <= NT <= 4096 and V >= 1");
  FW_CHECK_ARG(P >= 1 && step >= 0 && step < NT && (int64_t)P - 1 + step < NT,
               "need P >= 1, 0 <= step < NT and P - 1 + step < NT (P = %d, step = %d, NT = %d)", P, step, NT);
  FW_CHECK_ARG(eot >= 0 && eot < V && max_fin >= 1 && budget >= 1 && lp_pow == lp_pow, "bad eot / max_fin / budget / lp_pow");
  const int R = B * K, C = 2 * K, pos = P - 1 + step;
// ... 161 lines not shown
```

### faster_whisper_amd/csrc/kernels.h

```cpp
#pragma once
#include <atomic>
#include "common.h"

namespace fwk {

size_t logmel_lds_bytes();
void launch_logmel(hipStream_t st, const float* pcm_dev, const int64_t* offsets_dev, int B, int max_frames_total,
                   const float* consts, const float* filtT, int mel_pad, int n_mels, float* raw,
                   int64_t raw_bstride, int raw_stride, int* chunk_max, int drop_last, int out_frames,
                   float* out_f32, half_t* out_cl, int c_pad, int* n_frames_out);
void launch_features_to_cl(hipStream_t st, const float* feats_dev, int B, int n_mels, int frames, half_t* out_cl,
                           int c_pad);

struct GemmParams {
  const half_t* A; int64_t lda; int64_t a_bstride;
  const half_t* W; int64_t ldw;
  const half_t* bias;
  const half_t* res; int64_t ldr; int64_t r_bstride;
  half_t* C; int64_t ldc; int64_t c_bstride;
  int M, N, K;
  int act;
  int head_rows;
  const float* a_scale; int64_t as_bstride; const float* w_scale;
  int nMt, nNt;
  int n_mp, blk_m, blk_n;
  int vt_stage;
  int n_layers; int64_t w_lstride, bias_lstride, c_lstride;
  int nNt_layer;
};
int launch_gemm(hipStream_t st, const GemmParams& p, int batch, bool trans);
extern std::atomic<int> g_gemm_order;
extern std::atomic<int> g_gemm_vt_stage;

void launch_layernorm(hipStream_t st, const half_t* x, const half_t* g, const half_t* b, half_t* y, int rows, int d,
                      int frag = 0);
void launch_quant_rows(hipStream_t st, const half_t* x, int64_t ldx, const half_t* g, const half_t* b, int8_t* xq,
                       float* scale, int rows, int d, int frag = 0);
void launch_f32_to_f16(hipStream_t st, const float* x, half_t* y, int64_t n);
void launch_f16_to_f32(hipStream_t st, const half_t* x, float* y, int64_t n);

void launch_attn_enc(hipStream_t st, const half_t* q, const half_t* k, int64_t ld, int64_t qk_bstride,
                     const half_t* vt, int64_t ldvt, int64_t vt_bstride, half_t* out, int64_t ldo,
                     int64_t o_bstride, int B, int H, int T, int order = 0);

}
```

Before: 3234.

## Fold encoder LayerNorms into GEMM epilogues via producer-side row statistics

Removes the standalone encoder LayerNorm kernels (ln1, ln2) for fp16 models. The producing GEMMs (conv2, attn.out, ffn2) now emit per-64-column mean/M2 partial statistics, and the consuming GEMMs (qk, v, ffn1) use pre-folded weights (gamma multiplied into W, plus column sums s1 and constant cf). They combine the partial stats per row and apply mean/rstd in the epilogue. This saves a full read and write of the activation per LayerNorm and drops the xn workspace. In exchange it adds extra LDS, register pressure and epilogue work to the GEMMs, and numerics change slightly because normalization happens after an fp16 matmul on unnormalized inputs.

```diff
diff --git a/faster_whisper_amd/_lib.py b/faster_whisper_amd/_lib.py
--- a/faster_whisper_amd/_lib.py
+++ b/faster_whisper_amd/_lib.py
@@ -78,7 +78,7 @@
     "fw_test_gemm_ex", "fw_test_cross_kv_frag_index", "fw_test_quant_rows", "fw_test_layernorm_frag",
     "fw_test_dec_beam_update", "fw_test_dec_embed", "fw_test_align_post",
     "fw_test_logits_rules_lp", "fw_test_dec_beam_update_lp",
-    "fw_test_logits_rules_smp_tab", "fw_test_graph_captures",
+    "fw_test_logits_rules_smp_tab", "fw_test_graph_captures", "fw_test_enc_ln_fold",
     "fw_vad_create", "fw_vad_forward", "fw_vad_free", "fw_vad_forward_dev", "fw_vad_forward_audio_dev",
     "fw_vad_forward_audio_batch_dev",
     "fw_flac_info", "fw_flac_decode",
@@ -201,6 +201,9 @@
     if hasattr(lib, "fw_test_graph_captures"):
         lib.fw_test_logits_rules_smp_tab.argtypes = [vp, vp, i32, vp, i32, vp, C.POINTER(FwGenOpts), i32, vp, vp, vp, vp, vp, vp]
         lib.fw_test_graph_captures.argtypes = [vp, i64p]
+    if hasattr(lib, "fw_test_enc_ln_fold"):
+        lib.fw_test_enc_ln_fold.argtypes = [vp, vp, vp, vp, vp, i32, vp, vp, vp, vp, i32, i32, i32, i32, i32, i64, i32, i32,
+                                            vp, vp, vp]
     lib.fw_vad_create.argtypes = [C.POINTER(FwVadWeights), C.POINTER(vp)]
     lib.fw_vad_forward.argtypes = [vp, vp, i64, i32, vp, vp, vp]
     lib.fw_vad_free.argtypes = [vp]
diff --git a/faster_whisper_amd/csrc/engine.h b/faster_whisper_amd/csrc/engine.h
--- a/faster_whisper_amd/csrc/engine.h
+++ b/faster_whisper_amd/csrc/engine.h
@@ -94,7 +94,7 @@
 };
 struct LNW { const half_t* g = nullptr; const half_t* b = nullptr; };
 
-struct EncLayerW { LNW ln1, ln2; LinearW qk, v, out, ffn1, ffn2; };
+struct EncLayerW { LNW ln1, ln2; LinearW qk, v, out, ffn1, ffn2; LinearW qk_p, v_p, ffn1_p; };
 struct DecLayerW { LNW ln1, ln2, ln3; LinearW qkv, out, cq, ck, cv, cout, ffn1, ffn2; LinearW qkv_p, cq_p, ffn1_p; };
 
 enum ProfFamily {
@@ -184,6 +184,7 @@
   LNW dec_ln;
   int ln_unfold = 0;
   bool has_plain = false;
+  int enc_ln_unfold = 0;
 
   float* lm_consts = nullptr;
   float* lm_filtT = nullptr;
@@ -197,7 +198,9 @@
   float* ws_feat32 = nullptr;
   half_t* ws_mel_cl = nullptr;
   half_t* ws_conv1 = nullptr;
-  half_t *ws_x = nullptr, *ws_x2 = nullptr, *ws_xn = nullptr;
+  half_t *ws_x = nullptr, *ws_x2 = nullptr;
+  half_t* ws_xn = nullptr;
+  float *ws_st1 = nullptr, *ws_st2 = nullptr;
   half_t* ws_qk = nullptr;
   half_t* ws_vt = nullptr;
   half_t* ws_att = nullptr;
@@ -240,7 +243,7 @@
 
 int run_linear(Model* m, const LinearW& L, const half_t* A, int64_t lda, int64_t a_bs, half_t* C, int64_t ldc,
                int64_t c_bs, const half_t* res, int64_t ldr, int64_t r_bs, int M, int batch, int act, bool trans,
-               int head_rows = 0, hipStream_t st = nullptr);
+               int head_rows = 0, hipStream_t st = nullptr, float* stats_out = nullptr, const float* stats_in = nullptr);
 
 int run_linear_i8(Model* m, const LinearW& L, const half_t* A, const LNW* ln, half_t* C, int64_t ldc, int64_t c_bs,
                   const half_t* res, int64_t ldr, int64_t r_bs, int M, int batch, int act, bool trans, int head_rows,
diff --git a/faster_whisper_amd/csrc/engine.hip b/faster_whisper_amd/csrc/engine.hip
--- a/faster_whisper_amd/csrc/engine.hip
+++ b/faster_whisper_amd/csrc/engine.hip
@@ -298,11 +298,9 @@
   char nb[96];
   for (int i = 0; i < cfg->n_enc_layers; ++i) {
     auto nmf = [&](const char* s) { snprintf(nb, sizeof(nb), "enc.%d.%s", i, s); return std::string(nb); };
-    TRY(add_plain(nmf("ln1.g"), {d})); TRY(add_plain(nmf("ln1.b"), {d}));
-    TRY(add_linear(nmf("attn.qkv"), 3 * d, d));
+    TRY(add_ln_linear(nmf("attn.qkv"), nmf("ln1"), 3 * d, d));
     TRY(add_linear(nmf("attn.out"), d, d));
-    TRY(add_plain(nmf("ln2.g"), {d})); TRY(add_plain(nmf("ln2.b"), {d}));
-    TRY(add_linear(nmf("ffn1"), 4 * d, d));
+    TRY(add_ln_linear(nmf("ffn1"), nmf("ln2"), 4 * d, d));
     TRY(add_linear(nmf("ffn2"), d, 4 * d));
   }
   TRY(add_plain("enc.ln_post.g", {d})); TRY(add_plain("enc.ln_post.b", {d}));
@@ -530,22 +528,32 @@
   m->conv2.N = d; m->conv2.K = 3 * d;
   TRY(need("enc.pos", &m->enc_pos));
   m->enc.resize(c.n_enc_layers);
+  m->has_plain = !i8 && tptr(m, "dec.logits.wp") != nullptr;
+  const bool enc_plain = m->has_plain;
   char nb[96];
   for (int i = 0; i < c.n_enc_layers; ++i) {
     EncLayerW& L = m->enc[i];
     auto nm = [&](const char* s) { snprintf(nb, sizeof(nb), "enc.%d.%s", i, s); return std::string(nb); };
-    TRY(ln(nm("ln1"), &L.ln1));
-    TRY(linear(nm("attn.qkv"), &L.qk, 2 * d, d, 0));
-    TRY(linear(nm("attn.qkv"), &L.v, d, d, 2 * d));
+    if (i8 || enc_plain) {
+      LinearW &qk = i8 ? L.qk : L.qk_p, &v = i8 ? L.v : L.v_p, &f1 = i8 ? L.ffn1 : L.ffn1_p;
+      TRY(ln(nm("ln1"), &L.ln1));
+      TRY(linear(nm("attn.qkv"), &qk, 2 * d, d, 0));
+      TRY(linear(nm("attn.qkv"), &v, d, d, 2 * d));
+      TRY(ln(nm("ln2"), &L.ln2));
+      TRY(linear(nm("ffn1"), &f1, 4 * d, d, 0));
+    }
+    if (!i8) {
+      TRY(folded(nm("attn.qkv"), &L.qk, 2 * d, d));
+      L.v = L.qk;
+      L.v.w += (size_t)2 * d * d; L.v.s1 += 2 * d; L.v.cf += 2 * d; L.v.N = d;
+      TRY(folded(nm("ffn1"), &L.ffn1, 4 * d, d));
+    }
     TRY(linear(nm("attn.out"), &L.out, d, d, 0));
-    TRY(ln(nm("ln2"), &L.ln2));
-    TRY(linear(nm("ffn1"), &L.ffn1, 4 * d, d, 0));
     TRY(linear(nm("ffn2"), &L.ffn2, d, 4 * d, 0));
   }
   TRY(ln("enc.ln_post", &m->enc_ln_post));
   TRY(need("dec.tok_emb", &m->tok_emb)); TRY(need("dec.pos", &m->dec_pos));
   m->dec.resize(c.n_dec_layers);
-  m->has_plain = !i8 && tptr(m, "dec.logits.wp") != nullptr;
   for (int i = 0; i < c.n_dec_layers; ++i) {
     DecLayerW& L = m->dec[i];
     auto nm = [&](const char* s) { snprintf(nb, sizeof(nb), "dec.%d.%s", i, s); return std::string(nb); };
@@ -608,7 +616,11 @@
   A(m->ws_conv1, B * 3002 * d);
   A(m->ws_x, B * T * d);
   A(m->ws_x2, B * T * d);
-  A(m->ws_xn, B * T * d);
+  if (m->compute_type == FW_COMPUTE_FLOAT16) {
+    A(m->ws_st1, B * T * (d / 64) * 2);
+    A(m->ws_st2, B * T * (d / 64) * 2);
+  }
+  if (m->enc_ln_unfold) A(m->ws_xn, B * T * d);
   A(m->ws_qk, B * T * 2 * d);
   A(m->ws_vt, B * d * m->t_pad);
   A(m->ws_att, B * T * d);
@@ -683,6 +695,16 @@
       return fail(FW_EINVAL);
     }
   }
+  {
+    const char* eu = getenv("FWAMD_ENC_LN_UNFOLD");
+    if (eu && eu[0] == '1' && !eu[1] && m->compute_type != FW_COMPUTE_INT8_FLOAT16) {
+      if (!m->has_plain) {
+        set_error("FWAMD_ENC_LN_UNFOLD=1 needs a weight blob packed with FWAMD_LN_UNFOLD set (this one carries the folded forms only)");
+        return fail(FW_EINVAL);
+      }
+      m->enc_ln_unfold = 1;
+    }
+  }
   if ((rc = setup_logmel_consts(m))) return fail(rc);
   if ((rc = alloc_workspaces(m))) return fail(rc);
   m->decode_batch = max_batch;
@@ -735,12 +757,14 @@
 
 int run_linear(Model* m, const LinearW& L, const half_t* A, int64_t lda, int64_t a_bs, half_t* C, int64_t ldc,
                int64_t c_bs, const half_t* res, int64_t ldr, int64_t r_bs, int M, int batch, int act, bool trans,
-               int head_rows, hipStream_t st) {
+               int head_rows, hipStream_t st, float* stats_out, const float* stats_in) {
   fwk::GemmParams p;
   memset(&p, 0, sizeof(p));
   p.A = A; p.lda = lda; p.a_bstride = a_bs;
   p.W = L.w; p.ldw = L.K;
   p.bias = L.b;
+  p.stats_out = stats_out;
+  if (L.s1) { p.s1 = L.s1; p.cf = L.cf; p.stats_in = stats_in; p.bias = nullptr; }
   p.res = res; p.ldr = ldr; p.r_bstride = r_bs;
   p.C = C; p.ldc = ldc; p.c_bstride = c_bs;
   p.M = M; p.N = L.N; p.K = L.K;
@@ -800,6 +824,10 @@
   const fw_config& c = m->cfg;
   const int d = c.d_model, T = c.n_audio_ctx, H = c.n_heads;
   const int64_t xs = (int64_t)T * d;
+  const bool i8 = m->compute_type == FW_COMPUTE_INT8_FLOAT16;
+  const bool fold = !i8 && !m->enc_ln_unfold;
+  float* const st1 = fold ? m->ws_st1 : nullptr;
+  float* const st2 = fold ? m->ws_st2 : nullptr;
   int rc;
   {
     ProfScope ps(m, PF_ENC_GEMM, 2.0 * B * 3000.0 * d * (3.0 * c.n_mels), 0);
@@ -810,12 +838,11 @@
   {
     ProfScope ps(m, PF_ENC_GEMM, 2.0 * B * (double)T * d * (3.0 * d), 0);
     if ((rc = run_linear(m, m->conv2, m->ws_conv1, 2 * d, (int64_t)3002 * d, m->ws_x, d, xs, m->enc_pos, d, 0, T, B,
-                         1, false)))
+                         1, false, 0, nullptr, fold ? m->ws_st1 : nullptr)))
       return rc;
   }
   half_t* x = m->ws_x;
   half_t* x2 = m->ws_x2;
-  const bool i8 = m->compute_type == FW_COMPUTE_INT8_FLOAT16;
   for (int l = 0; l < c.n_enc_layers; ++l) {
     const EncLayerW& L = m->enc[l];
     if (i8) {
@@ -843,17 +870,17 @@
       }
       continue;
     }
-    {
+    if (!fold) {
       ProfScope ps(m, PF_ENC_LN, 0, 4.0 * B * T * d);
       fwk::launch_layernorm(m->stream, x, L.ln1.g, L.ln1.b, m->ws_xn, B * T, d);
     }
     {
       ProfScope ps(m, PF_ENC_GEMM, 2.0 * B * (double)T * d * (3.0 * d), 0);
-      if ((rc = run_linear(m, L.qk, m->ws_xn, d, xs, m->ws_qk, 2 * d, (int64_t)T * 2 * d, nullptr, 0, 0, T, B, 0,
-                           false)))
+      if ((rc = run_linear(m, fold ? L.qk : L.qk_p, fold ? x : m->ws_xn, d, xs, m->ws_qk, 2 * d, (int64_t)T * 2 * d, nullptr,
+                           0, 0, T, B, 0, false, 0, nullptr, nullptr, st1)))
         return rc;
-      if ((rc = run_linear(m, L.v, m->ws_xn, d, xs, m->ws_vt, m->t_pad, (int64_t)d * m->t_pad, nullptr, 0, 0, T, B, 0,
-                           true)))
+      if ((rc = run_linear(m, fold ? L.v : L.v_p, fold ? x : m->ws_xn, d, xs, m->ws_vt, m->t_pad, (int64_t)d * m->t_pad,
+                           nullptr, 0, 0, T, B, 0, true, 0, nullptr, nullptr, st1)))
         return rc;
     }
     {
@@ -863,18 +890,19 @@
     }
     {
       ProfScope ps(m, PF_ENC_GEMM, 2.0 * B * (double)T * d * d, 0);
-      if ((rc = run_linear(m, L.out, m->ws_att, d, xs, x2, d, xs, x, d, xs, T, B, 0, false))) return rc;
-    }
-    {
+      if ((rc = run_linear(m, L.out, m->ws_att, d, xs, x2, d, xs, x, d, xs, T, B, 0, false, 0, nullptr, st2))) return rc;
+    }
+    if (!fold) {
       ProfScope ps(m, PF_ENC_LN, 0, 4.0 * B * T * d);
       fwk::launch_layernorm(m->stream, x2, L.ln2.g, L.ln2.b, m->ws_xn, B * T, d);
     }
     {
       ProfScope ps(m, PF_ENC_GEMM, 2.0 * B * (double)T * d * (8.0 * d), 0);
-      if ((rc = run_linear(m, L.ffn1, m->ws_xn, d, xs, m->ws_ffn, 4 * d, (int64_t)T * 4 * d, nullptr, 0, 0, T, B, 1,
-                           false)))
+      if ((rc = run_linear(m, fold ? L.ffn1 : L.ffn1_p, fold ? x2 : m->ws_xn, d, xs, m->ws_ffn, 4 * d, (int64_t)T * 4 * d,
+                           nullptr, 0, 0, T, B, 1, false, 0, nullptr, nullptr, st2)))
         return rc;
-      if ((rc = run_linear(m, L.ffn2, m->ws_ffn, 4 * d, (int64_t)T * 4 * d, x, d, xs, x2, d, xs, T, B, 0, false)))
+      if ((rc = run_linear(m, L.ffn2, m->ws_ffn, 4 * d, (int64_t)T * 4 * d, x, d, xs, x2, d, xs, T, B, 0, false, 0, nullptr,
+                           l + 1 < c.n_enc_layers ? st1 : nullptr)))
         return rc;
     }
   }
@@ -1082,7 +1110,7 @@
   for (half_t* p : m->enc_pool) (void)hipFree(p);
   m->enc_pool.clear();
   void* ptrs[] = {m->lm_consts, m->lm_filtT, m->ws_pcm, m->ws_offsets, m->ws_raw, m->ws_chunk_max, m->ws_nframes,
-                  m->ws_feat32, m->ws_mel_cl, m->ws_conv1, m->ws_x, m->ws_x2, m->ws_xn, m->ws_qk, m->ws_vt,
+                  m->ws_feat32, m->ws_mel_cl, m->ws_conv1, m->ws_x, m->ws_x2, m->ws_xn, m->ws_st1, m->ws_st2, m->ws_qk, m->ws_vt,
                   m->ws_att, m->ws_ffn, m->ws_xq, m->ws_xs};
   for (void* p : ptrs)
     if (p) (void)hipFree(p);
diff --git a/faster_whisper_amd/csrc/gemm.hip b/faster_whisper_amd/csrc/gemm.hip
--- a/faster_whisper_amd/csrc/gemm.hip
+++ b/faster_whisper_amd/csrc/gemm.hip
@@ -22,8 +22,20 @@
     asm volatile("" ::: "memory");         \
   } while (0)
 
-template <bool TRANS, bool I8, bool LAYERED = false>
-__global__ __launch_bounds__(512) void gemm_f16_kernel(fwk::GemmParams p) {
+#define GB_LNF_LDS_BYTES 4096
+#define GB_LNF_MAX_SEG 20
+
+static __device__ __forceinline__ float gb_sum8(float v) {
+  v += dpp_f<FW_DPP_XOR1>(v);
+  v += dpp_f<FW_DPP_XOR2>(v);
+  v += dpp_f<0x141>(v);
+  return v;
+}
+
+template <bool TRANS, bool I8, bool LAYERED, bool LNF, bool STATS>
+static __device__ __forceinline__ void gemm_body(const fwk::GemmParams p) {
+  static_assert(!(LNF || STATS) || (!I8 && !LAYERED), "LayerNorm fold: plain fp16 launches only");
+  static_assert(!(LNF && STATS) && !(STATS && TRANS), "a launch is a producer or a consumer; producers are row-major");
   extern __shared__ __attribute__((aligned(16))) char smem_raw[];
   constexpr int ES = I8 ? 1 : 2;
 
@@ -56,7 +68,8 @@
 
   const char* Ab = reinterpret_cast<const char*>(p.A) + (size_t)z * p.a_bstride * ES;
   const char* Wb = reinterpret_cast<const char*>(p.W) + (LAYERED ? (size_t)layer * p.w_lstride * ES : 0);
-  const half_t* const biasp = (LAYERED && p.bias) ? p.bias + (size_t)layer * p.bias_lstride : p.bias;
+  const half_t* const biasp = LNF ? nullptr : (LAYERED && p.bias) ? p.bias + (size_t)layer * p.bias_lstride : p.bias;
+  const int head_rows = (LNF || STATS) ? 0 : p.head_rows;
   half_t* const Cp = LAYERED ? p.C + (size_t)layer * p.c_lstride : p.C;
 
   unsigned goff[4][2];
@@ -133,7 +146,7 @@
   };
 
   const int mw = m0 + wm * 128, nw = n0 + wn * 64;
-  const bool rowmajor = !TRANS && p.head_rows == 0;
+  const bool rowmajor = !TRANS && head_rows == 0;
   const half_t* const Rb = (rowmajor && p.res) ? p.res + (size_t)z * p.r_bstride : nullptr;
   const int ep_rr = lane >> 3, ep_cc = (lane & 7) * 8;
   const bool vec_ok = (p.ldc % 8 == 0) && (p.c_bstride % 8 == 0) && (!Rb || ((p.ldr % 8 == 0) && (p.r_bstride % 8 == 0)));
@@ -167,8 +180,47 @@
     }
   };
 
+  float* const lnf_par = reinterpret_cast<float*>(smem_raw + GB_LDS_BYTES);
+  float2 lnf_st[LNF ? GB_LNF_MAX_SEG : 1];
+  float lnf_s1 = 0.f, lnf_cf = 0.f;
+  if (LNF) {
+#pragma unroll
+    for (int u = 0; u < 4; ++u)
+#pragma unroll
+      for (int i = 0; i < 2; ++i) asm volatile("" : "+v"(goff[u][i]));
+    if (tid < 256) {
+      int m = m0 + tid; if (m > p.M - 1) m = p.M - 1;
+      const float2* sp = reinterpret_cast<const float2*>(p.stats_in) + ((size_t)z * p.M + m) * nk;
+#pragma unroll
+      for (int i = 0; i < GB_LNF_MAX_SEG; ++i) lnf_st[i] = sp[i < nk ? i : nk - 1];
+    } else {
+      int n = n0 + tid - 256; if (n > p.N - 1) n = p.N - 1;
+      lnf_s1 = p.s1[n];
+      lnf_cf = p.cf[n];
+    }
+    asm volatile("" ::: "memory");
+  }
+
   issue(2, 0); issue(0, 0); issue(3, 0); issue(1, 0);
   if (nk > 1) { issue(2, 1); issue(0, 1); }
+  if (LNF) {
+    asm volatile("" ::: "memory");
+    if (tid < 256) {
+      float mean = lnf_st[0].x, m2 = lnf_st[0].y;
+#pragma unroll
+      for (int i = 1; i < GB_LNF_MAX_SEG; ++i)
+        if (i < nk) {
+          const float dl = lnf_st[i].x - mean;
+          mean += dl * (1.0f / (float)(i + 1));
+          m2 += lnf_st[i].y + dl * dl * (64.0f * (float)i / (float)(i + 1));
+        }
+      const float var = m2 / (float)p.K;
+      *reinterpret_cast<float2*>(lnf_par + 2 * tid) = float2{mean, rsqrtf(fmaxf(var, 0.f) + 1e-5f)};
+    } else {
+      lnf_par[512 + tid - 256] = lnf_s1;
+      lnf_par[768 + tid - 256] = lnf_cf;
+    }
+  }
   seg_wait(nk > 1);
   GB_BARRIER();
   if (wm == 1) GB_BARRIER();
@@ -227,7 +279,7 @@
   if (wm == 0) GB_BARRIER();
 
   const float* sa = I8 ? p.a_scale + (size_t)z * p.as_bstride : nullptr;
-  if (!TRANS && p.head_rows == 0) {
+  if (!TRANS && head_rows == 0) {
     constexpr int EP_STRIDE = 272;
     char* ep = smem_raw + wave * (64 * EP_STRIDE);
     half_t* Cb = Cp + (size_t)z * p.c_bstride;
@@ -243,6 +295,8 @@
           const int r = mh * 32 + l31;
           int mc = mw + half * 64 + r; if (mc > p.M - 1) mc = p.M - 1;
           const float sam = I8 ? sa[mc] : 1.f;
+          float2 mr = {0.f, 1.f};
+          if (LNF) mr = *reinterpret_cast<const float2*>(lnf_par + 2 * (wm * 128 + half * 64 + r));
 #pragma unroll
           for (int g = 0; g < 4; ++g) {
             const int c = ni * 32 + 8 * g + 4 * hi;
@@ -251,7 +305,12 @@
 #pragma unroll
             for (int e = 0; e < 4; ++e)
               v[e] = I8 ? (float)acci[mi][ni][g * 4 + e] * sam * p.w_scale[n + e] : accf[mi][ni][g * 4 + e];
-            if (biasp) {
+            if (LNF) {
+              const floatx4 s1q = *reinterpret_cast<const floatx4*>(lnf_par + 512 + wn * 64 + c);
+              const floatx4 cfq = *reinterpret_cast<const floatx4*>(lnf_par + 768 + wn * 64 + c);
+#pragma unroll
+              for (int e = 0; e < 4; ++e) v[e] = mr.y * (v[e] - mr.x * s1q[e]) + cfq[e];
+            } else if (biasp) {
 #pragma unroll
               for (int e = 0; e < 4; ++e) v[e] += (float)bias4[ni][g][e];
             }
@@ -280,6 +339,18 @@
 #pragma unroll
           for (int e = 0; e < 8; ++e) o[e] = (half_t)v[e];
           *reinterpret_cast<half8_t*>(Cb + (size_t)m * p.ldc + n) = o;
+          if (STATS) {
+            float s = 0.f;
+#pragma unroll
+            for (int e = 0; e < 8; ++e) s += (float)o[e];
+            const float mean = gb_sum8(s) * (1.0f / 64.0f);
+            float q = 0.f;
+#pragma unroll
+            for (int e = 0; e < 8; ++e) { const float dv = (float)o[e] - mean; q += dv * dv; }
+            q = gb_sum8(q);
+            if ((lane & 7) == 0)
+              *reinterpret_cast<float2*>(p.stats_out + (((size_t)z * p.M + m) * (p.N >> 6) + (n >> 6)) * 2) = float2{mean, q};
+          }
         } else {
           for (int e = 0; e < 8 && n + e < p.N; ++e) {
             float t = v[e];
@@ -289,12 +360,12 @@
         }
       }
     }
-  } else if (p.head_rows > 0) {
+  } else if (head_rows > 0) {
     constexpr int FS = 144;
     char* ep = smem_raw + wave * (64 * FS);
     half_t* Cb = Cp + (size_t)z * p.c_bstride;
     if (nw < p.N) {
-      half_t* Hb = Cb + (size_t)(nw >> 6) * p.head_rows * 64;
+      half_t* Hb = Cb + (size_t)(nw >> 6) * head_rows * 64;
       const int g4 = lane >> 4, j = lane & 15;
 #pragma unroll
       for (int half = 0; half < 2; ++half) {
@@ -378,16 +449,23 @@
 #pragma unroll
     for (int ni = 0; ni < 2; ++ni) {
       const int c = ni * 32 + l31;
-      const float bv = (float)biasT[ni];
+      const float bv = LNF ? lnf_par[768 + wn * 64 + c] : (float)biasT[ni];
+      const float s1n = LNF ? lnf_par[512 + wn * 64 + c] : 0.f;
 #pragma unroll
       for (int mi = 0; mi < 4; ++mi)
 #pragma unroll
         for (int g = 0; g < 4; ++g) {
           const int r = mi * 32 + 8 * g + 4 * hi;
+          floatx4 mr0 = {0.f, 1.f, 0.f, 1.f}, mr1 = mr0;
+          if (LNF) {
+            mr0 = *reinterpret_cast<const floatx4*>(lnf_par + 2 * (wm * 128 + r));
+            mr1 = *reinterpret_cast<const floatx4*>(lnf_par + 2 * (wm * 128 + r) + 4);
+          }
+          const float mu4[4] = {mr0[0], mr0[2], mr1[0], mr1[2]}, rs4[4] = {mr0[1], mr0[3], mr1[1], mr1[3]};
           half4_t o;
 #pragma unroll
           for (int e = 0; e < 4; ++e) {
-            float v = accf[mi][ni][g * 4 + e] + bv;
+            float v = LNF ? rs4[e] * (accf[mi][ni][g * 4 + e] - mu4[e] * s1n) + bv : accf[mi][ni][g * 4 + e] + bv;
             if (p.act == 1) v = gelu_erf(v);
             o[e] = (half_t)v;
           }
@@ -419,16 +497,24 @@
       for (int ni = 0; ni < 2; ++ni) {
         const int n = n0 + wn * 64 + ni * 32 + l31;
         if (n >= p.N) continue;
-        const float bv = (float)biasT[ni];
+        const float bv = LNF ? lnf_par[768 + wn * 64 + ni * 32 + l31] : (float)biasT[ni];
+        const float s1n = LNF ? lnf_par[512 + wn * 64 + ni * 32 + l31] : 0.f;
         const float swn = I8 ? p.w_scale[n] : 1.f;
 #pragma unroll
         for (int g = 0; g < 4; ++g) {
           const int m = m0 + wm * 128 + mi * 32 + 8 * g + 4 * hi;
+          floatx4 mr0 = {0.f, 1.f, 0.f, 1.f}, mr1 = mr0;
+          if (LNF) {
+            mr0 = *reinterpret_cast<const floatx4*>(lnf_par + 2 * (m - m0));
+            mr1 = *reinterpret_cast<const floatx4*>(lnf_par + 2 * (m - m0) + 4);
+          }
+          const float mu4[4] = {mr0[0], mr0[2], mr1[0], mr1[2]}, rs4[4] = {mr0[1], mr0[3], mr1[1], mr1[3]};
           half4_t o;
 #pragma unroll
           for (int e = 0; e < 4; ++e) {
             int mm = m + e; if (mm > p.M - 1) mm = p.M - 1;
-            float v = (I8 ? (float)acci[mi][ni][g * 4 + e] * swn * sa[mm] : accf[mi][ni][g * 4 + e]) + bv;
+            float v = LNF ? rs4[e] * (accf[mi][ni][g * 4 + e] - mu4[e] * s1n) + bv
+                          : (I8 ? (float)acci[mi][ni][g * 4 + e] * swn * sa[mm] : accf[mi][ni][g * 4 + e]) + bv;
             if (p.act == 1) v = gelu_erf(v);
             o[e] = (half_t)v;
           }
@@ -443,6 +529,18 @@
         }
       }
   }
+}
+
+template <bool TRANS, bool I8, bool LAYERED = false>
+__global__ __launch_bounds__(512) void gemm_f16_kernel(fwk::GemmParams p) {
+  gemm_body<TRANS, I8, LAYERED, false, false>(p);
+}
+template <bool TRANS>
+__global__ __launch_bounds__(512) void gemm_f16_lnf_kernel(fwk::GemmParams p) {
+  gemm_body<TRANS, false, false, true, false>(p);
+}
+__global__ __launch_bounds__(512) void gemm_f16_stats_kernel(fwk::GemmParams p) {
+  gemm_body<false, false, false, false, true>(p);
 }
 
 namespace fwk {
@@ -461,6 +559,13 @@
   p.nMt = (p.M + GB_M - 1) / GB_M;
   p.nNt_layer = (p.N + GB_N - 1) / GB_N;
   if (p.n_layers > 1 && (i8 || p.res)) return -1;
+  const bool lnf = p.s1 != nullptr, stats = p.stats_out != nullptr;
+  if (lnf && (i8 || stats || p.n_layers > 1 || p.head_rows || p.res || !p.cf || !p.stats_in || p.K / 64 > GB_LNF_MAX_SEG))
+    return -1;
+  if (!lnf && (p.cf || p.stats_in)) return -1;
+  if (stats && (trans || i8 || p.n_layers > 1 || p.head_rows || p.N % 64 || p.ldc % 8 || p.c_bstride % 8 ||
+                (p.res && (p.ldr % 8 || p.r_bstride % 8))))
+    return -1;
   p.nNt = p.nNt_layer * (p.n_layers > 1 ? p.n_layers : 1);
   p.n_mp = p.nMt * batch;
   p.blk_m = p.blk_n = 0;
@@ -492,6 +597,22 @@
     attr_done.fetch_or(1ull << (dev & 63), std::memory_order_release);
   }
   const int grid = p.nMt * p.nNt * batch;
+  if (lnf || stats) {
+    static std::atomic<unsigned long long> attr_f{0};
+    if (!((attr_f.load(std::memory_order_acquire) >> (dev & 63)) & 1ull)) {
+      (void)hipFuncSetAttribute(reinterpret_cast<const void*>(gemm_f16_lnf_kernel<false>),
+                                hipFuncAttributeMaxDynamicSharedMemorySize, lds + GB_LNF_LDS_BYTES);
+      (void)hipFuncSetAttribute(reinterpret_cast<const void*>(gemm_f16_lnf_kernel<true>),
+                                hipFuncAttributeMaxDynamicSharedMemorySize, lds + GB_LNF_LDS_BYTES);
+      (void)hipFuncSetAttribute(reinterpret_cast<const void*>(gemm_f16_stats_kernel),
+                                hipFuncAttributeMaxDynamicSharedMemorySize, lds);
+      attr_f.fetch_or(1ull << (dev & 63), std::memory_order_release);
+    }
+    if (stats) gemm_f16_stats_kernel<<<grid, 512, lds, st>>>(p);
+    else if (trans) gemm_f16_lnf_kernel<true><<<grid, 512, lds + GB_LNF_LDS_BYTES, st>>>(p);
+    else gemm_f16_lnf_kernel<false><<<grid, 512, lds + GB_LNF_LDS_BYTES, st>>>(p);
+    return 0;
+  }
   if (p.n_layers > 1) {
     static std::atomic<unsigned long long> attr_l{0};
     if (!((attr_l.load(std::memory_order_acquire) >> (dev & 63)) & 1ull)) {
diff --git a/faster_whisper_amd/csrc/hooks.hip b/faster_whisper_amd/csrc/hooks.hip
--- a/faster_whisper_amd/csrc/hooks.hip
+++ b/faster_whisper_amd/csrc/hooks.hip
@@ -606,6 +606,93 @@
                     head_rows, nullptr);
   }
   return rc ? rc : download_f16(m->stream, C, dC, (size_t)c_elems);
+}
+
+int32_t fw_test_enc_ln_fold(fw_model* fm, const float* A, const float* Wp, const float* bp, const float* res, int32_t act_p,
+                            const float* ln_g, const float* ln_b, const float* Wc, const float* bc, int32_t M, int32_t Kp,
+                            int32_t Np, int32_t Nc, int32_t batch, int64_t x_bstride, int32_t form, int32_t fold,
+                            float* x_out, float* stats_out, float* y_out) {
+  FW_CHECK_ARG(fm && A && Wp && ln_g && ln_b && Wc && x_out && y_out, "null argument");
+  FW_CHECK_ARG(M >= 1 && M <= 4096 && batch >= 1 && batch <= 8, "M in [1, 4096], batch in [1, 8]");
+  FW_CHECK_ARG(Kp >= 64 && Kp % 64 == 0 && Kp <= 8192, "Kp: a multiple of 64");
+  FW_CHECK_ARG(Np >= 128 && Np % 128 == 0 && Np <= 1280, "Np: a multiple of 128, at most 1280 (the LayerNorm kernel's and the fold's range)");
+  FW_CHECK_ARG(Nc >= 4 && Nc % 4 == 0 && Nc <= 8192, "Nc: a multiple of 4");
+  FW_CHECK_ARG(x_bstride >= (int64_t)M * Np && x_bstride % 8 == 0 && x_bstride <= (int64_t)1 << 26, "x_bstride >= M * Np, a multiple of 8");
+  FW_CHECK_ARG((act_p == 0 || act_p == 1) && form >= 0 && form <= 2 && (fold == 0 || fold == 1), "act_p, fold: 0 | 1; form: 0 | 1 | 2");
+  Model* m = &fm->impl;
+  FW_CHECK_ARG(m->compute_type != FW_COMPUTE_INT8_FLOAT16, "float16 models only");
+  std::lock_guard<std::mutex> lk(m->mu);
+  FW_HIP(hipSetDevice(m->device));
+  hipStream_t st = m->stream;
+  auto h = [](float v) { return f16_bits_to_f32(f32_to_f16_bits(v)); };
+  const bool trans = form == 2;
+  const int nseg = Np / 64;
+  const int64_t ldct = (M + 7) / 8 * 8;
+  const size_t nx = (size_t)batch * x_bstride, ny = trans ? (size_t)batch * Nc * ldct : (size_t)batch * M * Nc,
+               nst = (size_t)batch * M * nseg * 2;
+  HookBufs db;
+  half_t *dA, *dWp, *dBp = nullptr, *dR = nullptr, *dX, *dY, *dXn = nullptr, *dG = nullptr, *dLb = nullptr, *dBc = nullptr;
+  uint16_t* dWc;
+  float *dSt = nullptr, *dS1 = nullptr, *dCf = nullptr;
+  int rc;
+  if ((rc = db.upload_f16(&dA, A, (size_t)batch * M * Kp)) || (rc = db.upload_f16(&dWp, Wp, (size_t)Np * Kp)) ||
+      (bp && (rc = db.upload_f16(&dBp, bp, Np))) || (res && (rc = db.upload_f16(&dR, res, (size_t)batch * M * Np))) ||
+      (rc = db.alloc(&dX, nx)) || (rc = db.zero(dX, nx * 2, st)) || (rc = db.alloc(&dY, ny)) || (rc = db.zero(dY, ny * 2, st)))
+    return rc;
+  std::vector<uint16_t> wc((size_t)Nc * Np);
+  LinearW Lp{dWp, dBp, nullptr, nullptr, nullptr, nullptr, Np, Kp}, Lc;
+  Lc.N = Nc; Lc.K = Np;
+  if (fold) {
+    std::vector<float> s1(Nc), cf(Nc);
+    for (int n = 0; n < Nc; ++n) {
+      double a1 = 0.0, ac = 0.0;
+      for (int k = 0; k < Np; ++k) {
+        const float wv = h(Wc[(size_t)n * Np + k]);
+        const uint16_t wg = f32_to_f16_bits(wv * h(ln_g[k]));
+        wc[(size_t)n * Np + k] = wg;
+        a1 += (double)f16_bits_to_f32(wg);
+        ac += (double)wv * (double)h(ln_b[k]);
+      }
+      if (bc) ac += (double)h(bc[n]);
+      s1[n] = (float)a1;
+      cf[n] = (float)ac;
+    }
+    if ((rc = db.upload(&dS1, s1.data(), (size_t)Nc)) || (rc = db.upload(&dCf, cf.data(), (size_t)Nc)) ||
+        (rc = db.alloc(&dSt, nst)) || (rc = db.zero(dSt, nst * 4, st)))
+      return rc;
+    Lc.s1 = dS1; Lc.cf = dCf;
+  } else {
+    for (size_t i = 0; i < wc.size(); ++i) wc[i] = f32_to_f16_bits(Wc[i]);
+    if ((rc = db.upload_f16(&dG, ln_g, Np)) || (rc = db.upload_f16(&dLb, ln_b, Np)) || (bc && (rc = db.upload_f16(&dBc, bc, Nc))) ||
+        (rc = db.alloc(&dXn, nx)) || (rc = db.zero(dXn, nx * 2, st)))
+      return rc;
+    Lc.b = dBc;
+  }
+  if ((rc = db.upload(&dWc, wc.data(), wc.size()))) return rc;
+  Lc.w = reinterpret_cast<const half_t*>(dWc);
+  if ((rc = run_linear(m, Lp, dA, Kp, (int64_t)M * Kp, dX, Np, x_bstride, dR, Np, (int64_t)M * Np, M, batch, act_p, false, 0,
+                       nullptr, dSt)))
+    return rc;
+  const half_t* xin = dX;
+  if (!fold) {
+    for (int z = 0; z < batch; ++z)
+      fwk::launch_layernorm(st, dX + (size_t)z * x_bstride, dG, dLb, dXn + (size_t)z * x_bstride, M, Np);
+    xin = dXn;
+  }
+  if ((rc = run_linear(m, Lc, xin, Np, x_bstride, dY, trans ? ldct : Nc, trans ? (int64_t)Nc * ldct : (int64_t)M * Nc, nullptr,
+                       0, 0, M, batch, form == 1 ? 1 : 0, trans, 0, nullptr, nullptr, dSt)))
+    return rc;
+  std::vector<float> xb(nx), yb(ny);
+  if ((rc = download_f16(st, xb.data(), dX, nx)) || (rc = download_f16(st, yb.data(), dY, ny))) return rc;
+  for (int z = 0; z < batch; ++z) {
+    memcpy(x_out + (size_t)z * M * Np, xb.data() + (size_t)z * x_bstride, (size_t)M * Np * sizeof(float));
+    if (!trans) continue;
+    for (int n = 0; n < Nc; ++n)
+      memcpy(y_out + ((size_t)z * Nc + n) * M, yb.data() + ((size_t)z * Nc + n) * ldct, (size_t)M * sizeof(float));
+  }
+  if (!trans) memcpy(y_out, yb.data(), ny * sizeof(float));
+  if (fold && stats_out) return download(stats_out, dSt, nst);
+  return FW_OK;
 }
 
 int32_t fw_test_attention(fw_model* fm, const float* q, const float* k, const float* v, int32_t B, int32_t H,
diff --git a/faster_whisper_amd/csrc/kernels.h b/faster_whisper_amd/csrc/kernels.h
--- a/faster_whisper_amd/csrc/kernels.h
+++ b/faster_whisper_amd/csrc/kernels.h
@@ -27,6 +27,8 @@
   int vt_stage;
   int n_layers; int64_t w_lstride, bias_lstride, c_lstride;
   int nNt_layer;
+  float* stats_out;
+  const float* stats_in; const float* s1; const float* cf;
 };
 int launch_gemm(hipStream_t st, const GemmParams& p, int batch, bool trans);
 extern std::atomic<int> g_gemm_order;
```

After: 3239, median of 2. Within noise of the previous version (+0.2%).
